# kalj/dealii-cuda

Measured on AMD Instinct MI355X. Metric: DoFs/s on 1305x Laplace vmult (bmop), p=4 3D uniform, higher is better.
Workload: dtype f64; 1 GPU; bmop: DEGREE_FE=4, DIMENSION=3, MATRIX_FREE_UNIFORM_MESH, hyper_cube(-1,1), 54^3 cells, 10218313 DoFs, 1 z-slab(s); cells_per_dir=54, n_dofs=10218313, n_cells=157464, parallelism=slab1, dof_numbering=caller's (lexicographic), finite=True, clock_ramp_steps=2000

## Files before the change

### dealii-cuda_amd/csrc/mfgpu_api.hip

```cpp
#include <hip/hip_runtime.h>

#include <type_traits>

#include <algorithm>
#include <cmath>
#include <cstdlib>
#include <cstring>
#include <memory>
#include <string>
#include <vector>

#include "mfgpu_kernels.h"

using namespace mfgpu;

struct EventTimer {
  std::vector<Event> ev;
  size_t used = 0;
  double ms = 0.0;
  int begin(hipStream_t st) {
    if (used + 2 > ev.size()) {
      Event e0, e1;
      int rc;
      if ((rc = e0.create(hipEventDefault)) || (rc = e1.create(hipEventDefault))) return rc;
      ev.push_back(std::move(e0));
      ev.push_back(std::move(e1));
    }
    HIP_TRY(hipEventRecord(ev[used].get(), st));
    return 0;
  }
  int end(hipStream_t st) {
    HIP_TRY(hipEventRecord(ev[used + 1].get(), st));
    used += 2;
    return 0;
  }
  int drain(double *total) {
    for (size_t i = 0; i + 1 < used; i += 2) {
      float t = 0.f;
      HIP_TRY(hipEventElapsedTime(&t, ev[i].get(), ev[i + 1].get()));
      ms += t;
    }
    used = 0;
    *total = ms;
    return 0;
  }
  void reset() {
    used = 0;
    ms = 0.0;
  }
};

struct mfgpu_handle {
  Plan plan;
  int dim = 0, n = 0, nd = 0, number_type = MFGPU_F64;
  bool hn = false;
  std::vector<double> S, Dt;
  std::vector<double> sv, sg;
  DeviceArray<uint32_t> d_batch_cell_off, d_batch_dof_off, d_bdofs;
  DeviceArray<uint8_t> d_bflags;
  DeviceArray<uint16_t> d_lmap;
  DeviceArray<uint16_t> d_lmapx;
  DeviceArray<uint16_t> d_perm;
  DeviceArray<uint32_t> d_bdofsp, d_idxp;
  DeviceArray<uint32_t> d_shtab;
  bool shared_records = false;
  size_t record_bytes = 0;
  DeviceArray<uint32_t> d_hnrec;
  DeviceArray<uint32_t> d_hn_slot;
  DeviceArray<void> d_coefp;
  DeviceArray<void> d_coef;
  DeviceArray<void> d_mass, d_massp;
  bool updatable = false;
  FoldGeometry geo;
  DeviceArray<uint32_t> d_cell_batch, d_cell_pos;
  size_t n_plane_cells = 0;
  DeviceArray<uint32_t> d_cmask, d_orphans;
  DeviceArray<void> d_hnw;
  DeviceArray<uint32_t> d_constrained;
  uint32_t n_constrained = 0;
  DeviceArray<void> d_tabsd;
  DeviceArray<void> d_tab2;
  bool twopass = true;
  DeviceArray<uint32_t> d_batch_nint, d_halo_off;
  std::vector<uint32_t> seg_end;
  std::vector<DeviceArray<uint32_t>> d_p2arr, d_p2tiles;
  std::vector<uint32_t> n_p2tiles;
  DeviceArray<uint32_t> d_p2rec, d_p2tab;
  bool p2_shared = false, p2_reverse = false, no_shared_records = false;
  Stream side;
  std::vector<Event> ev_seg;
  Event ev_side;
  bool side_pending = false;
  DeviceArray<void> d_halo;
  DeviceArray<unsigned long long> d_stamps;
  size_t lds = 0, device_bytes = 0;
  PlaneKernel planes = PlaneKernel::none;
  BatchKernel batches = BatchKernel::none;
  enum { kPlain, kMasked, kBatch };
  CellKernel<double> kernels_f64[3];
  CellKernel<float> kernels_f32[3];
  template <typename T>
  CellKernel<T> &kernel(int which) {
    if constexpr (std::is_same<T, double>::value) return kernels_f64[which];
    else return kernels_f32[which];
  }
  MultiKernel<double> multi_f64[kMaxFusedWidth - 1];
  MultiKernel<float> multi_f32[kMaxFusedWidth - 1];
  template <typename T>
  MultiKernel<T> &multi(int width) {
    if constexpr (std::is_same<T, double>::value) return multi_f64[width - 2];
    else return multi_f32[width - 2];
  }
  int multi_width = 1;
  DeviceArray<void> d_halo_multi;
  size_t halo_bytes = 0;
  uint32_t n_cus = 0, max_workgroups = 0;
  bool prof = false;
  EventTimer t_cells;
  EventTimer t_pass2;
  uint64_t prof_vmults = 0;
};

namespace {

template <typename T>
hipError_t bind_kernel(const mfgpu_handle *h, PlaneKernel pk, BatchKernel bk, bool hn, bool sh, CellKernel<T> *k) {
  const Plan &P = h->plan;
  const auto bind = pk == PlaneKernel::planes3 ? p_bind<T> : pk == PlaneKernel::planes4 ? q_bind<T>
                    : bk == BatchKernel::batches ? apply_bind<T> : bk == BatchKernel::x ? x_bind<T>
                    : bk == BatchKernel::g ? g_bind<T> : bk == BatchKernel::g2 ? g2_bind<T> : nullptr;
  if (!bind) return hipErrorInvalidValue;
  return bind(P.dim, P.n, hn, h->twopass, sh, h->d_mass.get() != nullptr, P.max_batch_dofs, k);
}

template <typename T, typename Args>
int launch_bound(mfgpu_handle *h, const CellKernel<T, Args> &k, const Args &a, uint32_t nbat, hipStream_t st) {
  if (!k.launch[0]) {
    set_error("cell-loop kernel not bound");
    return MFGPU_EINVAL;
  }
  uint32_t grid = (uint32_t)(k.per_cu < 1 ? 1 : k.per_cu) * h->n_cus;
  if (h->max_workgroups && h->max_workgroups < grid) grid = h->max_workgroups;
  HIP_TRY(k.launch[a.add != 0](a, h->S.data(), h->Dt.data(), k.lds, nbat < grid ? nbat : grid, st));
  return 0;
}

int check_symmetrize(int n, std::vector<double> &S, std::vector<double> &Dt) {
  const int p = n - 1;
  double err = 0, mag = 0;
  for (int r = 0; r < n; ++r)
    for (int c = 0; c < n; ++c) {
      const double s1 = S[r * n + c], s2 = S[(p - r) * n + (p - c)];
      const double d1 = Dt[r * n + c], d2 = -Dt[(p - r) * n + (p - c)];
      err = std::fmax(err, std::fmax(std::fabs(s1 - s2), std::fabs(d1 - d2)));
      mag = std::fmax(mag, std::fmax(std::fabs(s1), std::fabs(d1)));
    }
  if (err > 1e-10 * mag) {
    set_error("shape tables are not symmetric about the cell midpoint (unsupported)");
    return MFGPU_EUNSUPPORTED;
  }
  for (int r = 0; r < n; ++r)
    for (int c = 0; c < n; ++c) {
      const int r2 = p - r, c2 = p - c;
      if (r * n + c < r2 * n + c2) {
        const double s = 0.5 * (S[r * n + c] + S[r2 * n + c2]);
        S[r * n + c] = S[r2 * n + c2] = s;
        const double d = 0.5 * (Dt[r * n + c] - Dt[r2 * n + c2]);
        Dt[r * n + c] = d;
        Dt[r2 * n + c2] = -d;
      } else if (r == r2 && c == c2) {
        Dt[r * n + c] = 0.0;
      }
    }
  return 0;
}

int upload_pass2(mfgpu_handle *h, const uint32_t *priority, uint32_t n_priority) {
  const Plan &P = h->plan;
  const size_t ng = 1 + h->seg_end.size();
  const bool shared = P.sh_p2_use && !h->no_shared_records && n_priority == 0 && ng == 2;
  std::vector<Pass2Group> groups;
  int rc;
  if ((rc = pass2_groups(P, h->seg_end, priority, n_priority, shared, groups))) return rc;
  std::vector<DeviceArray<uint32_t>> d_arr(ng), d_tiles(ng);
  std::vector<uint32_t> n_tiles(ng, 0u);
  const bool reverse = (size_t)P.halo_off.back() * esize(h->number_type) <= ((size_t)256 << 20);
  DeviceArray<uint32_t> d_rec, d_tab;
  if (shared) {
    if ((rc = d_rec.upload(P.sh_p2rec.data(), P.sh_p2rec.size()))) return rc;
    if ((rc = d_tab.upload(P.sh_p2tab.data(), P.sh_p2tab.size()))) return rc;
  }
  for (size_t g = 0; g < ng; ++g) {
    std::vector<uint32_t> arr, tiles;
    build_pass2_classes(groups[g].dofs, groups[g].offsets, groups[g].slots, arr, tiles);
    n_tiles[g] = (uint32_t)(tiles.size() / 4);
    if (reverse) {
      const size_t nt = tiles.size() / 4;
      for (size_t a = 0, b = nt ? nt - 1 : 0; a < b; ++a, --b)
        for (int w = 0; w < 4; ++w) std::swap(tiles[4 * a + w], tiles[4 * b + w]);
    }
    if ((rc = d_arr[g].upload(arr.data(), arr.size()))) return rc;
    if ((rc = d_tiles[g].upload(tiles.data(), tiles.size()))) return rc;
  }
  h->d_p2arr = std::move(d_arr);
  h->d_p2tiles = std::move(d_tiles);
  h->n_p2tiles = std::move(n_tiles);
  h->d_p2rec = std::move(d_rec);
  h->d_p2tab = std::move(d_tab);
  h->p2_shared = shared;
  h->p2_reverse = reverse;
  return 0;
}

template <typename T>
int relayout_planes(mfgpu_handle *h, const uint32_t *cell_batch, const uint32_t *cell_pos, bool coef, bool mass,
                    hipStream_t st) {
  const size_t total = h->n_plane_cells * (size_t)h->nd;
  if (coef)
    HIP_TRY(relayout_coef_launch<T>(h->d_coefp.as<T>(), h->d_coef.as<const T>(), cell_batch, cell_pos, total, h->n, st));
  if (mass)
    HIP_TRY(relayout_coef_launch<T>(h->d_massp.as<T>(), h->d_mass.as<const T>(), cell_batch, cell_pos, total, h->n, st));
  return 0;
}

template <typename T>
int update_typed(mfgpu_handle *h, const void *coef, const void *mass, hipStream_t st) {
  const FoldInputs<T> in = h->geo.inputs<T>();
  if (coef) HIP_TRY(fold_coefficient_launch<T>(h->d_coef.as<T>(), (const T *)coef, in, st));
  if (mass) HIP_TRY(fold_mass_launch<T>(h->d_mass.as<T>(), (const T *)mass, in, st));
  if (h->planes == PlaneKernel::none) return 0;
  return relayout_planes<T>(h, h->d_cell_batch.get(), h->d_cell_pos.get(), coef != nullptr, mass != nullptr, st);
}

template <typename T>
int create_arrays(mfgpu_handle *h, const mfgpu_desc &d) {
  const Plan &P = h->plan;
  const size_t ncell = P.n_cells, nd = (size_t)P.nd;
  size_t &acct = h->device_bytes;
  auto up = [&](auto &arr, const void *src, size_t n) {
    const int rc = arr.upload(src, n);
    acct += arr.bytes();
    return rc;
  };
  int rc;
  if ((rc = up(h->d_batch_cell_off, P.batch_cell_off.data(), P.batch_cell_off.size()))) return rc;
  if ((rc = up(h->d_batch_dof_off, P.batch_dof_off.data(), P.batch_dof_off.size()))) return rc;
  if ((rc = up(h->d_bdofs, P.bdofs.data(), P.bdofs.size()))) return rc;
  if ((rc = up(h->d_bflags, P.bflags.data(), P.bflags.size()))) return rc;
  if ((rc = up(h->d_lmap, P.lmap.data(), P.lmap.size()))) return rc;
  const bool general = h->batches == BatchKernel::g || h->batches == BatchKernel::g2;
  if (h->batches == BatchKernel::x && !h->hn) {
    const std::vector<uint16_t> perm = x_lane_permutation(P.n);
    if ((rc = up(h->d_perm, perm.data(), perm.size()))) return rc;
  }
  if (h->batches == BatchKernel::x || general) {
    const std::vector<uint16_t> lx = x_pencil_runs(P.lmap, P.n);
    if ((rc = up(h->d_lmapx, lx.data(), lx.size()))) return rc;
  }
  if (h->batches == BatchKernel::g2) {
    std::vector<T> sd(2 * (size_t)P.n * P.n);
    for (int i = 0; i < P.n * P.n; ++i) {
      sd[i] = (T)h->S[i];
      sd[P.n * P.n + i] = (T)h->Dt[i];
    }
    if ((rc = up(h->d_tabsd, sd.data(), sd.size() * sizeof(T)))) return rc;
  }
  if (h->planes != PlaneKernel::none) {
    if ((rc = build_plane_records(h->plan, d.constraint_mask))) return rc;
    if (!P.pr_hn.empty()) {
      if ((rc = up(h->d_hnrec, P.pr_hn.data(), P.pr_hn.size()))) return rc;
      if ((rc = up(h->d_hn_slot, P.pr_hn_slot.data(), P.pr_hn_slot.size()))) return rc;
    }
    h->shared_records = P.sh_use && !(d.flags & MFGPU_NO_SHARED_RECORDS) &&
                        kernel_exists(h->planes, P.n, d.number_type, false, true, d.mass_coefficient != nullptr);
    const std::vector<uint32_t> &rd = h->shared_records ? P.sh_dofs : P.pr_dofs;
    const std::vector<uint32_t> &rx = h->shared_records ? P.sh_idx : P.pr_idx;
    if ((rc = up(h->d_bdofsp, rd.data(), rd.size()))) return rc;
    if ((rc = up(h->d_idxp, rx.data(), rx.size()))) return rc;
    if (h->shared_records && (rc = up(h->d_shtab, P.sh_batch.data(), P.sh_batch.size()))) return rc;
    h->record_bytes = h->d_bdofsp.bytes() + h->d_idxp.bytes() + h->d_shtab.bytes();
  }
  if ((rc = up(h->d_orphans, P.orphans.data(), P.orphans.size()))) return rc;
  if (h->twopass) {
    if ((rc = up(h->d_batch_nint, P.batch_nint.data(), P.batch_nint.size()))) return rc;
    if ((rc = up(h->d_halo_off, P.halo_off.data(), P.halo_off.size()))) return rc;
    if (h->planes != PlaneKernel::none && (uint64_t)P.halo_off.back() >= (1ull << 29)) {
      set_error("halo buffer too large for 32-bit byte offsets");
      return MFGPU_EUNSUPPORTED;
    }
    const size_t hb = ((size_t)P.halo_off.back() + 1) * sizeof(T);
    if ((rc = h->d_halo.alloc(hb, true))) return rc;
    acct += hb;
    h->halo_bytes = hb;
  }
  if (h->hn) {
    std::vector<uint32_t> cm(ncell);
    for (size_t i = 0; i < ncell; ++i) cm[i] = d.constraint_mask[P.cell_order[i]];
    if ((rc = up(h->d_cmask, cm.data(), ncell))) return rc;
    std::vector<T> w((size_t)h->n * h->n);
    for (size_t i = 0; i < w.size(); ++i) w[i] = (T)d.constraint_weights[i];
    if ((rc = up(h->d_hnw, w.data(), w.size() * sizeof(T)))) return rc;
  }
  FoldGeometry geo;
  if ((rc = geo.upload(d.JxW, d.inv_jac, P.cell_order.data(), P.dim, (uint32_t)ncell, (uint32_t)nd, general,
                       d.number_type)))
    return rc;
  DeviceArray<T> metric;
  if ((rc = fold_coefficient<T>(metric, d.coefficient, d.quadrature_points, geo.inputs<T>()))) return rc;
  h->d_coef = std::move(metric);
  acct += h->d_coef.bytes();
  if (d.mass_coefficient) {
    DeviceArray<T> mass;
    if ((rc = fold_mass<T>(mass, d.mass_coefficient, geo.inputs<T>()))) return rc;
    h->d_mass = std::move(mass);
    acct += h->d_mass.bytes();
  }
  if (h->updatable) {
    acct += geo.bytes();
    h->geo = std::move(geo);
  }
  if (h->planes != PlaneKernel::none) {
    const int n = P.n, NT = p_cells_per_wave(n) * n;
    const size_t nbat = P.n_plane_batches, total = nbat * (size_t)(n * n) * NT;
    const size_t ncell_p = P.batch_cell_off[nbat];
    std::vector<uint32_t> cb(ncell_p), cp(ncell_p);
    for (size_t b = 0; b < nbat; ++b)
      for (uint32_t c = P.batch_cell_off[b]; c < P.batch_cell_off[b + 1]; ++c) {
        cb[c] = (uint32_t)b;
        cp[c] = c - P.batch_cell_off[b];
      }
    DeviceArray<uint32_t> t_cb, t_cp;
    if ((rc = t_cb.upload(cb.data(), ncell_p))) return rc;
    if ((rc = t_cp.upload(cp.data(), ncell_p))) return rc;
    if ((rc = h->d_coefp.alloc(total * sizeof(T), true))) return rc;
    acct += h->d_coefp.bytes();
    h->n_plane_cells = ncell_p;
    if (d.mass_coefficient) {
      if ((rc = h->d_massp.alloc(total * sizeof(T), true))) return rc;
      acct += h->d_massp.bytes();
    }
    if ((rc = relayout_planes<T>(h, t_cb.get(), t_cp.get(), true, d.mass_coefficient != nullptr, nullptr))) return rc;
    HIP_TRY(hipDeviceSynchronize());
    if (h->updatable) {
      acct += t_cb.bytes() + t_cp.bytes();
      h->d_cell_batch = std::move(t_cb);
      h->d_cell_pos = std::move(t_cp);
    }
  }
  int dev = 0;
  hipDeviceProp_t prop;
  HIP_TRY(hipGetDevice(&dev));
  HIP_TRY(hipGetDeviceProperties(&prop, dev));
  h->n_cus = (uint32_t)prop.multiProcessorCount;
  h->max_workgroups = d.max_workgroups;
  if (h->planes != PlaneKernel::none) {
    CellKernel<T> &plain = h->kernel<T>(mfgpu_handle::kPlain), &masked = h->kernel<T>(mfgpu_handle::kMasked);
    HIP_TRY(bind_kernel<T>(h, h->planes, BatchKernel::none, false, h->shared_records, &plain));
    h->lds = plain.lds;
    if (P.n_plain_plane_batches < P.n_plane_batches) {
      HIP_TRY(bind_kernel<T>(h, h->planes, BatchKernel::none, true, false, &masked));
      h->lds = std::max(h->lds, masked.lds);
    }
  }
  if (h->batches == BatchKernel::none) return 0;
  CellKernel<T> &batch = h->kernel<T>(mfgpu_handle::kBatch);
  const hipError_t bind_batch_family = bind_kernel<T>(h, PlaneKernel::none, h->batches, h->hn, false, &batch);
  h->lds = batch.lds;
  if (h->lds > 160 * 1024) {
    set_error("batch needs more than 160 KiB of LDS; lower max_dofs_per_batch");
    return MFGPU_EINVAL;
  }
  HIP_TRY(bind_batch_family);
  if (h->twopass && h->planes == PlaneKernel::none)
    for (const int w : kFusedWidths) {
      if (!fused_kernel_exists(h->batches, P.n, d.number_type, h->hn, h->d_mass.get() != nullptr, w)) continue;
      MultiKernel<T> &mk = h->multi<T>(w);
      if (g_bind_width<T>(P.n, h->hn, false, h->d_mass.get() != nullptr, w, P.max_batch_dofs, &mk) != hipSuccess) {
        (void)hipGetLastError();
        mk = MultiKernel<T>();
      } else
        h->multi_width = std::max(h->multi_width, w);
    }
  return 0;
}

void choose_segments(mfgpu_handle *h, uint32_t request) {
  const Plan &P = h->plan;
  const uint32_t nb = (uint32_t)(P.batch_cell_off.size() - 1);
  h->seg_end.assign(1, nb);
  if (!h->twopass || nb < 2 || request == 1) return;
  const uint32_t npl = P.n_plane_batches, nplain = P.n_plain_plane_batches;
  std::vector<uint32_t> cuts;
  if (npl > 0 && npl < nb) cuts.push_back(npl);
  if (nplain > 0 && nplain < npl) cuts.push_back(nplain);
  if (request > 1) {
    for (uint32_t i = 1; i < request; ++i) cuts.push_back((uint32_t)((uint64_t)nb * i / request));
  }
  if (request == 0 && !P.pr_hn.empty() && nplain == 0 && P.n == 5) cuts.push_back(nb / 2);
  std::sort(cuts.begin(), cuts.end());
  h->seg_end.clear();
  for (uint32_t c : cuts)
    if (c > 0 && c < nb && (h->seg_end.empty() || h->seg_end.back() != c)) h->seg_end.push_back(c);
  h->seg_end.push_back(nb);
}

template <typename T>
int create_typed(mfgpu_handle *h, const mfgpu_desc &d) {
  int rc = create_arrays<T>(h, d);
  if (rc) return rc;
  choose_segments(h, d.cell_loop_segments);
  if (!h->twopass) return 0;
  if (h->seg_end.size() > 1) {
    int prio_least = 0, prio_greatest = 0;
    HIP_TRY(hipDeviceGetStreamPriorityRange(&prio_least, &prio_greatest));
    if ((rc = h->side.create(hipStreamNonBlocking, prio_least))) return rc;
    if ((rc = h->ev_side.create(hipEventDisableTiming))) return rc;
    h->ev_seg.resize(h->seg_end.size() - 1);
    for (Event &e : h->ev_seg)
      if ((rc = e.create(hipEventDisableTiming))) return rc;
  }
  return upload_pass2(h, nullptr, 0);
}

template <typename T>
int launch_pass2_group(mfgpu_handle *h, size_t group, void *dst, const void *src, hipStream_t st, int add) {
  if (h->p2_shared && group == 1)
    HIP_TRY(reduce_owner_batches_launch<T>((T *)dst, (const T *)src, h->d_halo.as<const T>(), h->d_p2rec.get(),
                                           h->d_p2tab.get(), (uint32_t)(h->plan.batch_cell_off.size() - 1),
                                           (uint32_t)p_hs(h->plan.n) * 64u, h->p2_reverse ? 1 : 0, add, st));
  HIP_TRY(reduce_classes_launch<T>((T *)dst, (const T *)src, h->d_halo.as<const T>(), h->d_p2arr[group].get(),
                                   h->d_p2tiles[group].get(), h->n_p2tiles[group], add, st));
  return 0;
}

template <typename T>
int vmult_pass2(mfgpu_handle *h, int phase, void *dst, const void *src, hipStream_t st, int add) {
  if (!h->twopass) return 0;
  if (phase == 0) return launch_pass2_group<T>(h, 0, dst, src, st, add);
  int rc = launch_pass2_group<T>(h, h->seg_end.size(), dst, src, st, add);
  if (!rc && h->side_pending) {
    HIP_TRY(hipStreamWaitEvent(st, h->ev_side.get(), 0));
    h->side_pending = false;
  }
  return rc;
}

template <typename T>
int launch_cells(mfgpu_handle *h, ApplyArgs<T> a, uint32_t b0, uint32_t b1, hipStream_t st) {
  const Plan &P = h->plan;
// ... 395 lines not shown
    set_error("null argument");
    return MFGPU_EINVAL;
  }
  const size_t nd = h->plan.n_dofs;
  if (n_vectors == 0 || (n_vectors > 1 && stride < nd)) {
    set_error("mfgpu_vmult_multi: n_vectors must be >= 1 and stride >= n_dofs");
    return MFGPU_EINVAL;
  }
  if ((flags & ~(MFGPU_MULTI_ADD | MFGPU_MULTI_LOOP | MFGPU_MULTI_FUSED)) ||
      ((flags & MFGPU_MULTI_LOOP) && (flags & MFGPU_MULTI_FUSED))) {
    set_error("mfgpu_vmult_multi: bad flags (MFGPU_MULTI_LOOP and MFGPU_MULTI_FUSED exclude each other)");
    return MFGPU_EINVAL;
  }
  const size_t bytes = ((size_t)(n_vectors - 1) * stride + nd) * esize(h->number_type);
  const char *d0 = (const char *)dst, *s0 = (const char *)src;
  if (d0 < s0 + bytes && s0 < d0 + bytes) {
    set_error("mfgpu_vmult_multi: the dst range overlaps the src range");
    return MFGPU_EINVAL;
  }
  return h->number_type == MFGPU_F64 ? vmult_multi_typed<double>(h, dst, src, n_vectors, stride, flags, (hipStream_t)stream)
                                     : vmult_multi_typed<float>(h, dst, src, n_vectors, stride, flags, (hipStream_t)stream);
}

int mfgpu_multi_width(const mfgpu_handle *h) { return h ? h->multi_width : 0; }

int mfgpu_update_coefficients(mfgpu_handle *h, const void *coefficient_dev, const void *mass_coefficient_dev,
                              void *stream) {
  if (!h) {
    set_error("null argument");
    return MFGPU_EINVAL;
  }
  if (!h->updatable) {
    set_error("mfgpu_update_coefficients: the handle was created without MFGPU_UPDATABLE_COEFFICIENTS");
    return MFGPU_EINVAL;
  }
  if (!coefficient_dev && !mass_coefficient_dev) {
    set_error("mfgpu_update_coefficients: coefficient_dev and mass_coefficient_dev are both NULL");
    return MFGPU_EINVAL;
  }
  if (mass_coefficient_dev && !h->d_mass.get()) {
    set_error("mfgpu_update_coefficients: the handle was created without a mass term (its kernels have no mass "
              "instantiation bound); create it with mass_coefficient");
    return MFGPU_EINVAL;
  }
  return h->number_type == MFGPU_F64 ? update_typed<double>(h, coefficient_dev, mass_coefficient_dev, (hipStream_t)stream)
                                     : update_typed<float>(h, coefficient_dev, mass_coefficient_dev, (hipStream_t)stream);
}

uint32_t mfgpu_n_dofs(const mfgpu_handle *h) { return h ? h->plan.n_dofs : 0; }

size_t mfgpu_memory_consumption(const mfgpu_handle *h) { return h ? h->device_bytes : 0; }

int mfgpu_plan_stats(const mfgpu_handle *h, uint64_t s[8]) {
  if (!h || !s) return MFGPU_EINVAL;
  const Plan &P = h->plan;
  s[0] = P.batch_cell_off.size() - 1;
  s[1] = P.color_batch_off.size() - 1;
  s[2] = P.bdofs.size();
  s[3] = P.max_batch_dofs;
  s[4] = P.max_batch_cells;
  s[5] = P.orphans.size();
  s[6] = P.n_first;
  s[7] = P.n_add;
  if (h->twopass) {
    const uint32_t nb = (uint32_t)s[0], npl = P.n_plane_batches, nplain = P.n_plain_plane_batches;
    const uint32_t edge[4] = {0u, nplain, npl, nb};
    s[1] = 0;
    for (size_t g = 0; g < h->seg_end.size(); ++g) {
      const uint32_t s0 = g ? h->seg_end[g - 1] : 0u, s1 = h->seg_end[g];
      for (int f = 0; f < 3; ++f)
        if (std::max(s0, edge[f]) < std::min(s1, edge[f + 1])) ++s[1];
    }
    s[6] = P.sdofs.size();
    s[7] = P.halo_off.back();
  }
  return 0;
}

int mfgpu_record_stats(const mfgpu_handle *h, uint64_t s[4]) {
  if (!h || !s) return MFGPU_EINVAL;
  const Plan &P = h->plan;
  const size_t n = (size_t)P.n, nb = (size_t)p_kgu((int)n) * 64, nx = ((n * n + 1) / 2) * (p_cells_per_wave((int)n) * n);
  const bool planes = h->planes != PlaneKernel::none;
  s[0] = (h->shared_records ? 1 : 0) | (h->p2_shared ? 2 : 0);
  s[1] = planes ? P.sh_dofs.size() / nb : 0;
  s[2] = planes ? P.sh_idx.size() / nx : 0;
  s[3] = h->record_bytes;
  return 0;
}

const char *mfgpu_kernel_name(const mfgpu_handle *h) {
  if (!h) return "";
  const bool x = h->batches == BatchKernel::x;
  switch (h->planes) {
    case PlaneKernel::planes3: return x ? "apply_planes3+apply_batches_x" : "apply_planes3";
    case PlaneKernel::planes4: return x ? "apply_planes4+apply_batches_x" : "apply_planes4";
    default: break;
  }
  switch (h->batches) {
    case BatchKernel::x: return "apply_batches_x";
    case BatchKernel::g: return "apply_batches_g";
    case BatchKernel::g2: return "apply_batches_g2";
    default: return "apply_batches";
  }
}

int mfgpu_profile_enable(mfgpu_handle *h, int on) {
  if (!h) return MFGPU_EINVAL;
  h->prof = on != 0;
  h->t_cells.reset();
  h->t_pass2.reset();
  h->prof_vmults = 0;
  return 0;
}

int mfgpu_profile_read_pass2(mfgpu_handle *h, double *ms) {
  if (!h || !ms) return MFGPU_EINVAL;
  HIP_TRY(hipDeviceSynchronize());
  return h->t_pass2.drain(ms);
}

int mfgpu_profile_read(mfgpu_handle *h, double *ms, uint64_t *nv) {
  if (!h || !ms || !nv) return MFGPU_EINVAL;
  HIP_TRY(hipDeviceSynchronize());
  if (const int rc = h->t_cells.drain(ms)) return rc;
  *nv = h->prof_vmults;
  return 0;
}

#ifdef MFGPU_STAMPS
int mfgpu_debug_stamps(mfgpu_handle *h, unsigned long long *out, size_t n_batches) {
  if (!h) return MFGPU_EINVAL;
  const size_t nbt = h->plan.batch_cell_off.size() - 1;
  if (!h->d_stamps.get()) return h->d_stamps.alloc(2 * nbt * 16, true);
  if (out && n_batches == nbt) {
    HIP_TRY(hipDeviceSynchronize());
    HIP_TRY(hipMemcpy(out, h->d_stamps.get(), 2 * nbt * 16 * sizeof(unsigned long long), hipMemcpyDeviceToHost));
  }
  return 0;
}
#endif


int mfgpu_compute_inverse_diagonal(mfgpu_handle *h, void *inv_diag, void *stream) {
  if (!h || !inv_diag) {
    set_error("null argument");
    return MFGPU_EINVAL;
  }
  return h->number_type == MFGPU_F64 ? inverse_diagonal_typed<double>(h, inv_diag, (hipStream_t)stream)
                                     : inverse_diagonal_typed<float>(h, inv_diag, (hipStream_t)stream);
}

int mfgpu_set_constrained_values(mfgpu_handle *h, void *vec, double value, void *stream) {
  if (!h || !vec) {
    set_error("null argument");
    return MFGPU_EINVAL;
  }
  if (h->number_type == MFGPU_F64)
    HIP_TRY(set_values_launch<double>((double *)vec, h->d_constrained.get(), h->n_constrained, value, (hipStream_t)stream));
  else
    HIP_TRY(set_values_launch<float>((float *)vec, h->d_constrained.get(), h->n_constrained, (float)value,
                                     (hipStream_t)stream));
  return 0;
}

int mfgpu_vec_sadd(void *v, double s, double a, const void *w, size_t n, int nt, void *stream) {
  return vec_map(0, v, w, s, a, n, nt, stream);
// ... 75 lines not shown
```

### dealii-cuda_amd/csrc/mfgpu_internal.h

```cpp
#ifndef MFGPU_INTERNAL_H
#define MFGPU_INTERNAL_H

#include <cstdint>
#include <string>
#include <vector>

#include "../../include/mfgpu.h"

namespace mfgpu {

void set_error(const std::string &msg);

inline int ipow(int a, int e) {
  int r = 1;
  for (int i = 0; i < e; ++i) r *= a;
  return r;
}

constexpr int p_cells_per_wave(int n) { return 64 / n; }
constexpr int p_ji(int n) { return n == 3 ? 2 : n == 4 ? 5 : n == 5 ? 9 : n == 6 ? 14 : 23; }
constexpr int p_hs(int n) { return n == 3 ? 3 : n == 4 ? 6 : n == 5 ? 9 : n == 6 ? 14 : 18; }
constexpr int p_kgu(int n) { return p_ji(n) + p_hs(n); }
constexpr int p_cell_stride(int n) {
  int s = n * n * n;
  while ((s & 31) != (n & 31)) ++s;
  return s;
}

constexpr int q_plane_stride(int n) { return n >= 6 ? 65 : n == 5 ? 33 : n == 4 ? 17 : 33; }
constexpr int q_cell_stride(int n) { return n * q_plane_stride(n); }
constexpr int p_priv_max(int n) { return n >= 5 ? 384 : n == 4 ? 256 : 192; }
constexpr int kHnOpRounds = 2;
constexpr int p_hn_rows(int n) { return p_priv_max(n) / 64 + 3 * kHnOpRounds * 3 + 2; }

template <typename T>
constexpr size_t q_region_doubles(int n) {
  const size_t t = ((size_t)(p_cells_per_wave(n) + 1) * q_cell_stride(n) * sizeof(T) + 7) / 8;
  const size_t u = (size_t)p_kgu(n) * 64 + p_priv_max(n);
  return t > u ? t : u;
}
template <typename T>
constexpr size_t q_lds_bytes(int n, bool hn) {
  return (q_region_doubles<T>(n) + (hn ? (size_t)n * n : 0)) * 8;
}

constexpr uint8_t kFlagConstrained = 1;
constexpr uint8_t kFlagAdd = 2;

struct Plan {
  int dim = 0, degree = 0, n = 0, nd = 0;
  uint32_t n_dofs = 0, n_cells = 0;
  std::vector<uint32_t> cell_order;
  std::vector<uint32_t> batch_cell_off;
  std::vector<uint32_t> batch_dof_off;
  std::vector<uint32_t> color_batch_off;
  std::vector<uint32_t> bdofs;
  std::vector<uint8_t> bflags;
  std::vector<uint16_t> lmap;
  std::vector<uint32_t> orphans;
  std::vector<uint32_t> batch_nint;
  std::vector<uint32_t> halo_off;
  std::vector<uint32_t> sdofs;
  std::vector<uint32_t> s_off;
  std::vector<uint32_t> s_idx;
  std::vector<uint32_t> chunks;
  std::vector<uint32_t> gstarts;
  uint32_t max_batch_dofs = 0, max_batch_cells = 0;
  uint32_t n_plane_batches = 0;
  uint32_t n_plain_plane_batches = 0;
  std::vector<uint32_t> pr_dofs, pr_idx, pr_hn, pr_hn_slot;
  std::vector<uint32_t> sh_dofs, sh_idx, sh_batch;
  bool sh_use = false;
  std::vector<uint32_t> sh_p2rec, sh_p2tab;
  bool sh_p2_use = false;
  uint64_t n_first = 0, n_add = 0;
};

struct PlanLimits {
  uint32_t max_cells = 0, max_dofs = 0;
  uint32_t interior_max = 0, shared_max = 0, halo_stride = 0;
  bool segregate_masked = false;
  bool masked_planes = false;
  uint32_t private_max = 0;
};

int build_plan(const mfgpu_desc &d, Plan &plan, uint32_t max_chunks = 3, const PlanLimits *limits = nullptr);

struct HnLine {
  uint16_t node[8];
};
void hn_cell_lines(unsigned mask, int n, std::vector<HnLine> (&lines)[3], std::vector<uint16_t> &nodes);

enum class PlaneKernel : uint8_t { none, planes3, planes4 };
enum class BatchKernel : uint8_t { none, batches, x, g, g2 };
int choose_kernel_and_plan(const mfgpu_desc &d, PlaneKernel &pk, BatchKernel &bk, Plan &plan);

constexpr bool planes4_wide(int n) { return n >= 6; }
constexpr bool kernel_exists(PlaneKernel k, int n, int number_type, bool hn, bool sh, bool mass) {
  switch (k) {
    case PlaneKernel::planes3: return n >= 3 && n <= 5 && !(sh && hn);
    case PlaneKernel::planes4:
      return planes4_wide(n) ? n <= 7 && !hn && !sh && !mass
                             : n >= 3 && !sh && !(mass && n == 5 && number_type == MFGPU_F64);
    default: return false;
  }
}
constexpr bool kernel_exists(BatchKernel k, int n, int , bool , bool sh, bool ) {
  return k != BatchKernel::none && n >= 2 && n <= 7 && !sh;
}
constexpr int kFusedWidths[] = {3, 2};
constexpr bool fused_kernel_exists(BatchKernel k, int n, int number_type, bool hn, bool , int nv) {
  return k == BatchKernel::g && n >= 2 && n <= 7 && (nv == 2 || nv == 3) &&
         !(hn && number_type == MFGPU_F64 && n >= (nv == 3 ? 6 : 7));
}
std::vector<uint32_t> multi_groups(uint32_t n_vectors, const std::vector<uint32_t> &widths);
int build_plane_records(Plan &plan, const uint32_t *constraint_mask);
constexpr int kShBatchWords = 4;
constexpr double kShareMaxFraction = 0.5;
void share_plane_records(Plan &plan);
constexpr int kP2Header = 16, kP2MaxK = 12, kP2SlotBits = 12;
void share_pass2_records(Plan &plan);

std::vector<uint16_t> x_lane_permutation(int n);
std::vector<uint16_t> x_pencil_runs(const std::vector<uint16_t> &lmap, int n);
struct Pass2Group {
  std::vector<uint32_t> dofs, offsets = std::vector<uint32_t>(1, 0u), slots;
};
int pass2_groups(const Plan &plan, const std::vector<uint32_t> &seg_end, const uint32_t *priority, uint32_t n_priority,
                 bool shared, std::vector<Pass2Group> &groups);

int derive_tables(int n, const double *shape_values, const double *shape_gradients,
                  std::vector<double> &S, std::vector<double> &Dt);

int handle_number_type(const mfgpu_handle *h);
int handle_set_priority_dofs(mfgpu_handle *h, const uint32_t *ids, uint32_t n);
int handle_vmult_phase(mfgpu_handle *h, int phase, void *dst, const void *src, void *stream, int add);
int handle_n_batches(const mfgpu_handle *h);
bool handle_ranged_ok(const mfgpu_handle *h);
int handle_batches_touching(const mfgpu_handle *h, const uint32_t *ids, uint32_t n, std::vector<uint8_t> &flags);
int handle_cells_range(mfgpu_handle *h, uint32_t b0, uint32_t b1, void *dst, const void *src, void *stream, int add);
int handle_cells_two_ranges(mfgpu_handle *h, uint32_t b0, uint32_t b1, uint32_t c0, uint32_t c1, void *dst,
                            const void *src, void *stream, int add);
int handle_pass2_group(mfgpu_handle *h, int group, void *dst, const void *src, void *stream, int add);

void transfer_sizes(const mfgpu_transfer *t, uint32_t *n_coarse_dofs, uint32_t *n_fine_dofs, int *number_type);
void vcycle_active(const mfgpu_vcycle *v, int *active_type, uint32_t *n_active);

}

struct mfgpu_plan {
  mfgpu::Plan plan;
};

#endif
```

### dealii-cuda_amd/csrc/mfgpu_kernels.h

```cpp
#ifndef MFGPU_KERNELS_H
#define MFGPU_KERNELS_H

#include <hip/hip_runtime.h>

#include <type_traits>

#include "mfgpu_device.h"
#include "mfgpu_internal.h"

namespace mfgpu {

template <typename T>
struct ApplyArgs {
  const uint32_t *batch_cell_off;
  const uint32_t *batch_dof_off;
  const uint32_t *bdofs;
  const uint8_t *bflags;
  const uint16_t *lmap;
  const uint16_t *lmapx;
  const uint16_t *perm;
  const uint32_t *bdofsp;
  const uint32_t *idxp;
  const T *coefp;
  const uint32_t *hnrec;
// ... 16 lines not shown
  int dbg;
  const uint32_t *shtab = nullptr;
  const T *mass = nullptr;
  const T *massp = nullptr;
};

constexpr int kMaxFusedWidth = 3;
template <typename T>
struct MultiArgs : ApplyArgs<T> {
  size_t stride = 0;
  T *halos[kMaxFusedWidth];
};
constexpr size_t kMaxLdsBytes = 160 * 1024;

template <typename T, int n>
struct Tables {
  T S[((n + 1) / 2) * n];
  T Dt[((n + 1) / 2) * n];
};

template <typename T, int n>
inline Tables<T, n> make_tables(const double *S, const double *Dt) {
  Tables<T, n> tab;
  for (int i = 0; i < ((n + 1) / 2) * n; ++i) {
    tab.S[i] = (T)S[i];
    tab.Dt[i] = (T)Dt[i];
  }
  return tab;
}

template <typename T, typename Args = ApplyArgs<T>>
struct CellKernel {
  size_t lds = 0;
  int per_cu = 0;
  hipError_t (*launch[2])(const Args &a, const double *S, const double *Dt, size_t lds, uint32_t grid,
                          hipStream_t st) = {nullptr, nullptr};
};

template <typename T, int Block, auto K, auto MakeTab, typename Args = ApplyArgs<T>>
hipError_t launch_cell_kernel(const Args &a, const double *S, const double *Dt, size_t lds, uint32_t grid,
                              hipStream_t st) {
  if constexpr (std::is_null_pointer_v<decltype(MakeTab)>)
    hipLaunchKernelGGL(K, dim3(grid), dim3(Block), lds, st, a);
  else
    hipLaunchKernelGGL(K, dim3(grid), dim3(Block), lds, st, a, MakeTab(S, Dt));
  return hipGetLastError();
}

template <typename T, int Block, auto K0, auto K1, auto MakeTab, typename Args = ApplyArgs<T>>
hipError_t bind_cell_kernel(size_t lds, CellKernel<T, Args> *k) {
  k->lds = lds;
  for (const void *f : {(const void *)K1, (const void *)K0})
    if (const hipError_t e = hipFuncSetAttribute(f, hipFuncAttributeMaxDynamicSharedMemorySize, (int)lds)) return e;
  k->launch[0] = launch_cell_kernel<T, Block, K0, MakeTab, Args>;
  k->launch[1] = launch_cell_kernel<T, Block, K1, MakeTab, Args>;
  return hipOccupancyMaxActiveBlocksPerMultiprocessor(&k->per_cu, (const void *)K0, Block, lds);
}

template <typename F>
hipError_t dispatch_flags(F &&f) { return f(); }
template <typename F, typename... B>
hipError_t dispatch_flags(F &&f, bool flag, B... rest) {
  return dispatch_flags(
      [&](auto... c) { return flag ? f(std::true_type{}, c...) : f(std::false_type{}, c...); }, rest...);
}
template <typename F, typename... B>
hipError_t dispatch_instantiation(int n, F &&f, B... flags) {
  auto at = [&](auto N) { return dispatch_flags([&](auto... c) { return f(N, c...); }, flags...); };
  switch (n) {
    case 2: return at(std::integral_constant<int, 2>{});
    case 3: return at(std::integral_constant<int, 3>{});
    case 4: return at(std::integral_constant<int, 4>{});
    case 5: return at(std::integral_constant<int, 5>{});
    case 6: return at(std::integral_constant<int, 6>{});
    case 7: return at(std::integral_constant<int, 7>{});
    default: return hipErrorInvalidValue;
  }
}
template <typename T>
constexpr int number_type_of = sizeof(T) == 8 ? MFGPU_F64 : MFGPU_F32;

#define MFGPU_CELL_LOOP_FAMILY(F)                                                                              \
  template <typename T>                                                                                        \
  hipError_t F##_bind(int dim, int n, bool hn, bool twopass, bool sh, bool mass, uint32_t nb_max, CellKernel<T> *k);
MFGPU_CELL_LOOP_FAMILY(apply)
MFGPU_CELL_LOOP_FAMILY(x)
MFGPU_CELL_LOOP_FAMILY(g)
MFGPU_CELL_LOOP_FAMILY(g2)
MFGPU_CELL_LOOP_FAMILY(p)
MFGPU_CELL_LOOP_FAMILY(q)
#undef MFGPU_CELL_LOOP_FAMILY
template <typename T>
using MultiKernel = CellKernel<T, MultiArgs<T>>;
template <typename T, typename Args>
hipError_t g_bind_width(int n, bool hn, bool sh, bool mass, int nv, uint32_t nb_max, CellKernel<T, Args> *k);

void build_pass2_classes(const std::vector<uint32_t> &sdofs, const std::vector<uint32_t> &s_off,
                         const std::vector<uint32_t> &s_idx, std::vector<uint32_t> &arr, std::vector<uint32_t> &tiles);
template <typename T>
hipError_t reduce_classes_launch(T *dst, const T *src, const T *halo, const uint32_t *arr, const uint32_t *tiles,
                                 uint32_t n_tiles, int add, hipStream_t st);
template <typename T>
hipError_t reduce_classes_multi_launch(int nv, T *dst, const T *src, size_t stride, T *const *halos, const uint32_t *arr,
                                       const uint32_t *tiles, uint32_t n_tiles, int add, hipStream_t st);
template <typename T>
hipError_t reduce_owner_batches_launch(T *dst, const T *src, const T *halo, const uint32_t *rec, const uint32_t *tab,
                                       uint32_t n_batches, uint32_t hstride, int reverse, int add, hipStream_t st);
template <typename T>
hipError_t relayout_coef_launch(T *out, const T *in, const uint32_t *cell_batch, const uint32_t *cell_pos,
                                size_t total, int n, hipStream_t st);
template <typename T>
hipError_t fold_general_launch(T *M, const T *coef, const T *jxw, const T *jinv, const uint32_t *order,
                               uint32_t n_cells, uint32_t nd, hipStream_t st);
template <typename T>
hipError_t fold_general2_launch(T *M, const T *coef, const T *jxw, const T *jinv, const uint32_t *order,
                                uint32_t n_cells, uint32_t nd, hipStream_t st);
template <typename T>
hipError_t orphan_launch(T *dst, const T *src, const uint32_t *orph, uint32_t n, int add, hipStream_t st);
template <typename T>
hipError_t coefficient_launch(T *coef, const T *qpts, size_t nq, int dim, hipStream_t st);
template <typename T>
hipError_t fold_launch(T *c, const T *coef, const T *jxw, const T *j0, const uint32_t *order,
                       uint32_t n_cells, uint32_t nd, hipStream_t st);
template <typename T>
hipError_t fill_launch(T *v, size_t n, T a, hipStream_t st);
template <typename T>
struct FoldInputs {
  const T *jxw = nullptr, *jinv = nullptr;
  const uint32_t *order = nullptr;
  int dim = 0;
  uint32_t n_cells = 0, nd = 0;
  bool general = false;
  size_t metric_entries() const { return (size_t)n_cells * nd * (general ? (dim == 3 ? 6 : 3) : 1); }
};
template <typename T>
hipError_t fold_coefficient_launch(T *out, const T *coef, const FoldInputs<T> &in, hipStream_t st);
template <typename T>
hipError_t fold_mass_launch(T *out, const T *c, const FoldInputs<T> &in, hipStream_t st);
struct FoldGeometry {
  DeviceArray<void> jxw, jinv;
  DeviceArray<uint32_t> order;
  int dim = 0;
  uint32_t n_cells = 0, nd = 0;
  bool general = false;
  int upload(const void *JxW, const void *inv_jac, const uint32_t *cell_order, int dim_, uint32_t n_cells_, uint32_t nd_,
             bool general_, int number_type);
  size_t bytes() const { return jxw.bytes() + jinv.bytes() + order.bytes(); }
  template <typename T>
  FoldInputs<T> inputs(const T *jxw_resident = nullptr) const {
    FoldInputs<T> in;
    in.jxw = jxw_resident ? jxw_resident : jxw.as<const T>();
    in.jinv = jinv.as<const T>();
    in.order = order.get();
    in.dim = dim, in.n_cells = n_cells, in.nd = nd, in.general = general;
    return in;
  }
};
template <typename T>
int fold_mass(DeviceArray<T> &out, const void *mass_coefficient, const FoldInputs<T> &in);
template <typename T>
int fold_coefficient(DeviceArray<T> &out, const void *coefficient, const void *quadrature_points,
                     const FoldInputs<T> &in);

template <typename T>
hipError_t diag_launch(int dim, int n, T *diag, uint32_t n_batches, const uint32_t *batch_cell_off,
                       const uint32_t *batch_dof_off, const uint32_t *bdofs, const uint16_t *lmap, const T *coef,
                       const uint32_t *cmask, const T *hn_weights, const T *tab2, hipStream_t st);
// ... 24 lines not shown
```

### dealii-cuda_amd/csrc/mfgpu_kernels.hip

```cpp
#include <hip/hip_runtime.h>

#include "mfgpu_cell.h"
#include "mfgpu_kernels.h"

namespace mfgpu {

template <int n>
constexpr int min_waves_per_simd() { return n <= 5 ? 2 : 1; }

template <int dim, int n, typename T, bool HN, bool TWOPASS, bool MASS = false>
__global__ void __launch_bounds__(256) __attribute__((amdgpu_waves_per_eu(min_waves_per_simd<n>())))
apply_batches(const ApplyArgs<T> A, const Tables<T, n> tab) {
  constexpr int kBlock = 256;
  constexpr int kGU = (max_batch_dofs(kBlock) + kBlock - 1) / kBlock;
  constexpr int nd = (dim == 3) ? n * n * n : n * n;
  constexpr int P = nd / n;
  constexpr int NG = 1;
  constexpr int GT = kBlock / NG;
  constexpr int CH = GT / P;
  constexpr int n2 = n * n;
  constexpr int CHND = CH * nd;
  static_assert(CH >= 1, "a cell's pencils must fit into one thread group");
  extern __shared__ __attribute__((aligned(16))) unsigned char smem_raw[];
  double *acc = reinterpret_cast<double *>(smem_raw);
// ... 178 lines not shown
          }
        }
      }
    } else if (!DBG(4)) {
      T old[kGU];
#pragma unroll
      for (int j = 0; j < kGU; ++j) old[j] = A.dst[G[j] & 0x7fffffffu];
#pragma unroll
      for (int j = 0; j < kGU; ++j) {
        const int t = tid + j * kBlock;
        if (t < nb && !(G[j] >> 31)) A.dst[G[j]] = ((F[j] & kFlagAdd) || A.add) ? old[j] + (T)acc[t] : (T)acc[t];
      }
    }
    STAMP(15);
    if (!has_nb) break;
    __syncthreads();
    b = bn;
    c0 = c0n;
    ncell = ncelln;
    d0 = d0n;
    nb = nbn;
    nint = nintn;
    hoff = hoffn;
#pragma unroll
    for (int j = 0; j < kGU; ++j) {
      G[j] = Gn[j];
      F[j] = Fn[j];
      SV[j] = SVn[j];
    }
  }
}

template <typename T>
__global__ void orphan_kernel(T *dst, const T *src, const uint32_t *orph, uint32_t n, int add) {
  const uint32_t i = blockIdx.x * blockDim.x + threadIdx.x;
  if (i >= n) return;
  const uint32_t o = orph[i];
  const uint32_t g = o & 0x7fffffffu;
  const T s = (o >> 31) ? src[g] : T(0);
  dst[g] = add ? dst[g] + s : s;
}

template <typename T, int dim>
__global__ void coefficient_kernel(T *coef, const T *qpts, size_t nq) {
  const size_t i = (size_t)blockIdx.x * blockDim.x + threadIdx.x;
  if (i >= nq) return;
  T s = 0;
#pragma unroll
  for (int d = 0; d < dim; ++d) {
    const T x = qpts[i * dim + d];
    s += x * x;
  }
  coef[i] = T(1) / (T(0.05) + T(2) * s);
}

template <typename T>
__global__ void fold_kernel(T *c, const T *coef, const T *jxw, const T *j0, const uint32_t *order,
                            uint32_t n_cells, uint32_t nd) {
  const size_t i = (size_t)blockIdx.x * blockDim.x + threadIdx.x;
  if (i >= (size_t)n_cells * nd) return;
  const uint32_t pos = (uint32_t)(i / nd), q = (uint32_t)(i - (size_t)pos * nd);
  const uint32_t cell = order[pos];
  const T j = j0[cell];
  c[i] = coef[(size_t)cell * nd + q] * j * j * jxw[(size_t)cell * nd + q];
}

template <typename T>
__global__ void fill_kernel(T *v, size_t n, T a) {
  size_t i = (size_t)blockIdx.x * blockDim.x + threadIdx.x;
  const size_t stride = (size_t)gridDim.x * blockDim.x;
  for (; i < n; i += stride) v[i] = a;
}


template <int dim, int n, typename T>
static size_t lds_bytes_t(uint32_t nb_max) {
  constexpr int nd = (dim == 3) ? n * n * n : n * n;
  const int CH = 256 / (nd / n);
  return (size_t)nb_max * sizeof(double) + (size_t)(nb_max + 3 * CH * nd + n * n) * sizeof(T) +
         (size_t)CH * nd * sizeof(uint16_t);
}

template <typename T>
hipError_t apply_bind(int dim, int n, bool hn, bool twopass, bool sh, bool mass, uint32_t nb_max, CellKernel<T> *k) {
  if (dim != 2 && dim != 3) return hipErrorInvalidValue;
  return dispatch_instantiation(n, [&](auto N, auto D3, auto HN, auto TP, auto SH, auto MASS) {
    constexpr int n_ = N, dim_ = D3 ? 3 : 2;
    if constexpr (kernel_exists(BatchKernel::batches, n_, number_type_of<T>, HN, SH, MASS)) {
      constexpr auto K = apply_batches<dim_, n_, T, HN, TP, MASS>;
      return bind_cell_kernel<T, 256, K, K, make_tables<T, n_>>(lds_bytes_t<dim_, n_, T>(nb_max), k);
    } else
      return hipErrorInvalidValue;
  }, dim == 3, hn, twopass, sh, mass);
}

template <typename T>
hipError_t orphan_launch(T *dst, const T *src, const uint32_t *orph, uint32_t n, int add,
                         hipStream_t st) {
  if (n == 0) return hipSuccess;
  hipLaunchKernelGGL(orphan_kernel<T>, dim3((n + 255) / 256), dim3(256), 0, st, dst, src, orph, n, add);
  return hipGetLastError();
}

template <typename T>
hipError_t coefficient_launch(T *coef, const T *qpts, size_t nq, int dim, hipStream_t st) {
  const unsigned grid = (unsigned)((nq + 255) / 256);
  if (dim == 2)
    hipLaunchKernelGGL((coefficient_kernel<T, 2>), dim3(grid), dim3(256), 0, st, coef, qpts, nq);
  else
    hipLaunchKernelGGL((coefficient_kernel<T, 3>), dim3(grid), dim3(256), 0, st, coef, qpts, nq);
  return hipGetLastError();
}

template <typename T>
hipError_t fold_launch(T *c, const T *coef, const T *jxw, const T *j0, const uint32_t *order,
                       uint32_t n_cells, uint32_t nd, hipStream_t st) {
  const size_t tot = (size_t)n_cells * nd;
  hipLaunchKernelGGL(fold_kernel<T>, dim3((unsigned)((tot + 255) / 256)), dim3(256), 0, st, c, coef, jxw,
                     j0, order, n_cells, nd);
  return hipGetLastError();
}

int FoldGeometry::upload(const void *JxW, const void *inv_jac, const uint32_t *cell_order, int dim_, uint32_t n_cells_,
                         uint32_t nd_, bool general_, int number_type) {
  dim = dim_, n_cells = n_cells_, nd = nd_, general = general_;
  const size_t np = (size_t)n_cells * nd, es = esize(number_type);
  int rc;
  if (JxW && (rc = jxw.upload(JxW, np * es))) return rc;
  if ((rc = jinv.upload(inv_jac, (general ? np * (size_t)(dim * dim) : n_cells) * es))) return rc;
  return order.upload(cell_order, n_cells);
}

template <typename T>
hipError_t fold_coefficient_launch(T *out, const T *coef, const FoldInputs<T> &in, hipStream_t st) {
  if ((size_t)in.n_cells * in.nd == 0) return hipSuccess;
  const auto fold = !in.general ? fold_launch<T> : in.dim == 3 ? fold_general_launch<T> : fold_general2_launch<T>;
  return fold(out, coef, in.jxw, in.jinv, in.order, in.n_cells, in.nd, st);
}

template <typename T>
int fold_coefficient(DeviceArray<T> &out, const void *coefficient, const void *quadrature_points,
                     const FoldInputs<T> &in) {
  const size_t np = (size_t)in.n_cells * in.nd;
  DeviceArray<T> coef, qpts;
  int rc;
  if (coefficient) {
    if ((rc = coef.upload(coefficient, np))) return rc;
  } else {
    if ((rc = qpts.upload(quadrature_points, np * in.dim))) return rc;
    if ((rc = coef.alloc(np))) return rc;
    if ((rc = hip_check(coefficient_launch<T>(coef.get(), qpts.get(), np, in.dim, nullptr), "coefficient evaluation")))
      return rc;
  }
  if ((rc = out.alloc(in.metric_entries()))) return rc;
  if ((rc = hip_check(fold_coefficient_launch<T>(out.get(), coef.get(), in, nullptr), "coefficient fold"))) return rc;
  return hip_check(hipDeviceSynchronize(), "coefficient fold");
}

template <typename T>
__global__ void fold_mass_kernel(T *m, const T *c, const T *jxw, const uint32_t *order, uint32_t n_cells, uint32_t nd) {
  const size_t i = (size_t)blockIdx.x * blockDim.x + threadIdx.x;
  if (i >= (size_t)n_cells * nd) return;
  const uint32_t pos = (uint32_t)(i / nd), q = (uint32_t)(i - (size_t)pos * nd);
  const size_t s = (size_t)order[pos] * nd + q;
  m[i] = c[s] * jxw[s];
}

template <typename T>
hipError_t fold_mass_launch(T *out, const T *c, const FoldInputs<T> &in, hipStream_t st) {
  const size_t np = (size_t)in.n_cells * in.nd;
  if (np == 0) return hipSuccess;
  hipLaunchKernelGGL(fold_mass_kernel<T>, dim3((unsigned)((np + 255) / 256)), dim3(256), 0, st, out, c, in.jxw,
                     in.order, in.n_cells, in.nd);
  return hipGetLastError();
}

template <typename T>
int fold_mass(DeviceArray<T> &out, const void *mass_coefficient, const FoldInputs<T> &in) {
  const size_t np = (size_t)in.n_cells * in.nd;
  DeviceArray<T> c;
  int rc;
  if ((rc = c.upload(mass_coefficient, np)) || (rc = out.alloc(np))) return rc;
  if ((rc = hip_check(fold_mass_launch<T>(out.get(), c.get(), in, nullptr), "mass fold"))) return rc;
  return hip_check(hipDeviceSynchronize(), "mass fold");
}

template <typename T>
hipError_t fill_launch(T *v, size_t n, T a, hipStream_t st) {
  if (n == 0) return hipSuccess;
  size_t blocks = (n + 255) / 256;
  if (blocks > 2048) blocks = 2048;
  hipLaunchKernelGGL(fill_kernel<T>, dim3((unsigned)blocks), dim3(256), 0, st, v, n, a);
  return hipGetLastError();
}

#define INST(T)                                                                                         \
  template hipError_t apply_bind<T>(int, int, bool, bool, bool, bool, uint32_t, CellKernel<T> *);      \
  template hipError_t orphan_launch<T>(T *, const T *, const uint32_t *, uint32_t, int, hipStream_t);   \
  template hipError_t coefficient_launch<T>(T *, const T *, size_t, int, hipStream_t);                  \
  template hipError_t fold_launch<T>(T *, const T *, const T *, const T *, const uint32_t *, uint32_t,  \
                                     uint32_t, hipStream_t);                                            \
  template hipError_t fold_coefficient_launch<T>(T *, const T *, const FoldInputs<T> &, hipStream_t);   \
  template hipError_t fold_mass_launch<T>(T *, const T *, const FoldInputs<T> &, hipStream_t);          \
  template int fold_coefficient<T>(DeviceArray<T> &, const void *, const void *, const FoldInputs<T> &); \
  template int fold_mass<T>(DeviceArray<T> &, const void *, const FoldInputs<T> &);                    \
  template hipError_t fill_launch<T>(T *, size_t, T, hipStream_t);
INST(double)
INST(float)

}
```

### dealii-cuda_amd/csrc/mfgpu_kernels_g.hip

```cpp
#include <hip/hip_runtime.h>

#include "mfgpu_cell.h"
#include "mfgpu_kernels.h"

namespace mfgpu {

template <typename T, int NV>
using GArgs = std::conditional_t<NV == 1, ApplyArgs<T>, MultiArgs<T>>;
template <typename T, typename P>
__device__ __forceinline__ P *vec_at(const ApplyArgs<T> &, P *p, int) { return p; }
template <typename T, typename P>
__device__ __forceinline__ P *vec_at(const MultiArgs<T> &A, P *p, int v) { return p + (size_t)v * A.stride; }
template <typename T>
__device__ __forceinline__ T *vec_halo(const ApplyArgs<T> &A, int) { return A.halo; }
template <typename T>
__device__ __forceinline__ T *vec_halo(const MultiArgs<T> &A, int v) { return A.halos[v]; }

template <int n, typename T, bool HN, int NV>
constexpr int g_waves_per_simd() {
  if (NV == 1) return 2;
  if (NV != 2) return 1;
  if (sizeof(T) == 8) return n <= (HN ? 2 : 3) ? 2 : 1;
  return n <= (HN ? 4 : 6) ? 2 : 1;
}
// ... 341 lines not shown
        T *hl = vec_halo(A, v) + hoff + l - nint;
        T old[kGU];
        if (A.add) {
#pragma unroll
          for (int j = 0; j < kGU; ++j) old[j] = vec_at(A, A.dst, v)[G[j] & 0x7fffffffu];
        }
#pragma unroll
        for (int j = 0; j < kGU; ++j) {
          if (l < nint - j * kBlock) {
            if (!(G[j] >> 31)) vec_at(A, A.dst, v)[G[j]] = A.add ? old[j] + (T)ul[j * kBlock] : (T)ul[j * kBlock];
          } else if (l < nb - j * kBlock) {
            hl[j * kBlock] = (T)ul[j * kBlock];
          }
        }
        if (NV == 1) break;
      }
    }
    if (!has_nb) break;
    b = bn;
    c0 = c0n;
    ncell = ncelln;
    d0 = d0n;
    nb = nbn;
    nint = nintn;
    hoff = hoffn;
#pragma unroll
    for (int j = 0; j < kGU; ++j) {
      G[j] = Gn[j];
#pragma unroll
      for (int iv = 0; iv < NV; ++iv) {
        const int v = NV == 1 ? 0 : iv;
        SV[v][j] = SVn[v][j];
        if (NV == 1) break;
      }
    }
#pragma unroll
    for (int k = 0; k < kMaxChunks; ++k)
#pragma unroll
      for (int q = 0; q < NW; ++q) IX[k][q] = IXn[k][q];
  }
}

template <typename T>
__global__ void fold_general_kernel(T *M, const T *coef, const T *jxw, const T *jinv, const uint32_t *order,
                                    uint32_t n_cells, uint32_t nd) {
  const size_t i = (size_t)blockIdx.x * blockDim.x + threadIdx.x;
  if (i >= (size_t)n_cells * nd) return;
  const uint32_t cell = (uint32_t)(i / nd), q = (uint32_t)(i - (size_t)cell * nd);
  const size_t s = (size_t)order[cell] * nd + q;
  const T *J = jinv + s * 9;
  const T a = coef[s] * jxw[s];
  T *m = M + (size_t)cell * (6 * nd) + q;
  int e = 0;
  for (int d1 = 0; d1 < 3; ++d1)
    for (int d2 = d1; d2 < 3; ++d2)
      m[(e++) * nd] = a * (J[3 * d1] * J[3 * d2] + J[3 * d1 + 1] * J[3 * d2 + 1] + J[3 * d1 + 2] * J[3 * d2 + 2]);
}

template <int n, typename T>
static size_t g_lds_bytes(uint32_t nb_max, int nv) {
  constexpr int nd = n * n * n;
  constexpr int CH = 256 / (n * n);
  return (size_t)nv * nb_max * sizeof(double) + (size_t)(4 * CH * nd + n * n) * sizeof(T);
}

template <typename T, typename Args>
hipError_t g_bind_width(int n, bool hn, bool sh, bool mass, int nv, uint32_t nb_max, CellKernel<T, Args> *k) {
  return dispatch_instantiation(n, [&](auto N, auto W3, auto HN, auto SH, auto MASS) {
    constexpr int n_ = N;
    constexpr int NV = std::is_same_v<Args, ApplyArgs<T>> ? 1 : W3 ? 3 : 2;
    if constexpr (NV == 1 ? kernel_exists(BatchKernel::g, n_, number_type_of<T>, HN, SH, MASS)
                          : !SH && fused_kernel_exists(BatchKernel::g, n_, number_type_of<T>, HN, MASS, NV)) {
      constexpr auto K = apply_batches_g<n_, T, HN, MASS, NV>;
      const size_t lds = g_lds_bytes<n_, T>(nb_max, NV);
      k->lds = lds;
      if (NV > 1 && lds > kMaxLdsBytes) return hipErrorInvalidValue;
      return bind_cell_kernel<T, 256, K, K, make_tables<T, n_>>(lds, k);
    } else
      return hipErrorInvalidValue;
  }, nv == 3, hn, sh, mass);
}

template <typename T>
hipError_t g_bind(int, int n, bool hn, bool, bool sh, bool mass, uint32_t nb_max, CellKernel<T> *k) {
  return g_bind_width(n, hn, sh, mass, 1, nb_max, k);
}

template <typename T>
hipError_t fold_general_launch(T *M, const T *coef, const T *jxw, const T *jinv, const uint32_t *order,
                               uint32_t n_cells, uint32_t nd, hipStream_t st) {
  const size_t tot = (size_t)n_cells * nd;
  hipLaunchKernelGGL(fold_general_kernel<T>, dim3((unsigned)((tot + 255) / 256)), dim3(256), 0, st, M, coef, jxw, jinv,
                     order, n_cells, nd);
  return hipGetLastError();
}

#define INST(T)                                                                                                  \
  template hipError_t g_bind<T>(int, int, bool, bool, bool, bool, uint32_t, CellKernel<T> *);                    \
  template hipError_t g_bind_width<T>(int, bool, bool, bool, int, uint32_t, MultiKernel<T> *);                   \
  template hipError_t fold_general_launch<T>(T *, const T *, const T *, const T *, const uint32_t *, uint32_t, \
                                             uint32_t, hipStream_t);
INST(double)
INST(float)

}
```

### dealii-cuda_amd/csrc/mfgpu_kernels_g2.hip

```cpp
#include <hip/hip_runtime.h>

#include "mfgpu_kernels.h"

namespace mfgpu {

namespace {

constexpr unsigned kTypeX = 1u << 0, kTypeY = 1u << 1, kFaceX = 1u << 3, kFaceY = 1u << 4;

template <int n, typename T, bool HN, bool MASS = false>
__global__ void __launch_bounds__(256)
apply_batches_g2(const ApplyArgs<T> A) {
  constexpr int nd = n * n, CH = 256 / nd, p = n - 1;
  extern __shared__ __attribute__((aligned(16))) unsigned char smem_raw[];
  double *acc = reinterpret_cast<double *>(smem_raw);
  T *usrc = reinterpret_cast<T *>(acc + A.nb_max);
  T *X = usrc + A.nb_max;
  T *Y = X + CH * nd;
  T *FX = Y + CH * nd;
  T *FY = FX + CH * nd;
  T *St = FY + CH * nd;
  T *Dt = St + nd;
  T *Wt = Dt + nd;
  const int tid = threadIdx.x;
// ... 67 lines not shown
      if (act) {
        T gx = T(0), gy = T(0);
        if (MASS) mv = A.mass[cell * nd + q] * x[q];
        for (int t = 0; t < n; ++t) {
          gx += Dt[i * n + t] * x[t + n * j];
          gy += Dt[j * n + t] * x[i + n * t];
        }
        const T *m = A.coef + cell * (3 * nd) + q;
        const T mxx = m[0], mxy = m[nd], myy = m[2 * nd];
        fx[q] = mxx * gx + mxy * gy;
        fy[q] = mxy * gx + myy * gy;
      }
      __syncthreads();
      if (act) {
        T s = T(0);
        for (int t = 0; t < n; ++t) s += Dt[t * n + i] * fx[t + n * j] + Dt[t * n + j] * fy[i + n * t];
        y[q] = MASS ? s + mv : s;
      }
      __syncthreads();
      if (act) {
        T s = T(0);
        for (int k = 0; k < n; ++k) s += St[j * n + k] * y[i + n * k];
        x[q] = s;
      }
      __syncthreads();
      T out = T(0);
      if (act) {
        for (int k = 0; k < n; ++k) out += St[i * n + k] * x[k + n * j];
      }
      if (HN) {
        __syncthreads();
        if (act) y[q] = out;
        __syncthreads();
        if (act) x[q] = hn_pass(y, 1, true);
        __syncthreads();
        if (act) out = hn_pass(x, 0, true);
      }
      if (MASS) {
        for (int w = 0; w < 4; ++w) {
          if (act && (tid >> 6) == w) atomicAdd(&acc[lm], (double)out);
          __syncthreads();
        }
      } else {
        if (act) atomicAdd(&acc[lm], (double)out);
        __syncthreads();
      }
    }
    T *halo = A.halo + A.halo_off[b];
    for (uint32_t t = tid; t < nb; t += 256) {
      const uint32_t g = A.bdofs[d0 + t];
      if (t < nint) {
        if (!(g >> 31)) A.dst[g] = A.add ? A.dst[g] + (T)acc[t] : (T)acc[t];
      } else {
        halo[t - nint] = (T)acc[t];
      }
    }
  }
}

template <typename T>
__global__ void fold_general2_kernel(T *M, const T *coef, const T *jxw, const T *jinv, const uint32_t *order,
                                     uint32_t n_cells, uint32_t nd) {
  const size_t i = (size_t)blockIdx.x * blockDim.x + threadIdx.x;
  if (i >= (size_t)n_cells * nd) return;
  const uint32_t cell = (uint32_t)(i / nd), q = (uint32_t)(i - (size_t)cell * nd);
  const size_t s = (size_t)order[cell] * nd + q;
  const T *J = jinv + s * 4;
  const T a = coef[s] * jxw[s];
  T *m = M + (size_t)cell * (3 * nd) + q;
  m[0] = a * (J[0] * J[0] + J[1] * J[1]);
  m[nd] = a * (J[0] * J[2] + J[1] * J[3]);
  m[2 * nd] = a * (J[2] * J[2] + J[3] * J[3]);
}

template <int n, typename T>
size_t g2_lds_bytes(uint32_t nb_max) {
  constexpr int nd = n * n, CH = 256 / nd;
  return (size_t)nb_max * sizeof(double) + ((size_t)nb_max + 4 * CH * nd + 3 * nd) * sizeof(T);
}

}

template <typename T>
hipError_t g2_bind(int, int n, bool hn, bool, bool sh, bool mass, uint32_t nb_max, CellKernel<T> *k) {
  return dispatch_instantiation(n, [&](auto N, auto HN, auto SH, auto MASS) {
    constexpr int n_ = N;
    if constexpr (kernel_exists(BatchKernel::g2, n_, number_type_of<T>, HN, SH, MASS)) {
      constexpr auto K = apply_batches_g2<n_, T, HN, MASS>;
      return bind_cell_kernel<T, 256, K, K, nullptr>(g2_lds_bytes<n_, T>(nb_max), k);
    } else
      return hipErrorInvalidValue;
  }, hn, sh, mass);
}
template hipError_t g2_bind<double>(int, int, bool, bool, bool, bool, uint32_t, CellKernel<double> *);
template hipError_t g2_bind<float>(int, int, bool, bool, bool, bool, uint32_t, CellKernel<float> *);

template <typename T>
hipError_t fold_general2_launch(T *M, const T *coef, const T *jxw, const T *jinv, const uint32_t *order,
                                uint32_t n_cells, uint32_t nd, hipStream_t st) {
  const size_t tot = (size_t)n_cells * nd;
  hipLaunchKernelGGL(fold_general2_kernel<T>, dim3((unsigned)((tot + 255) / 256)), dim3(256), 0, st, M, coef, jxw, jinv,
                     order, n_cells, nd);
  return hipGetLastError();
}
template hipError_t fold_general2_launch<double>(double *, const double *, const double *, const double *,
                                                 const uint32_t *, uint32_t, uint32_t, hipStream_t);
template hipError_t fold_general2_launch<float>(float *, const float *, const float *, const float *, const uint32_t *,
                                                uint32_t, uint32_t, hipStream_t);

}
```

### dealii-cuda_amd/csrc/mfgpu_kernels_p.hip

```cpp
#include <hip/hip_runtime.h>

#include "mfgpu_cell.h"
#include "mfgpu_kernels.h"
#include "mfgpu_planes.h"

namespace mfgpu {

#define MFGPU_PIN_VMEM() __builtin_amdgcn_sched_barrier(0x380)

template <int n, typename T, bool ADD, bool HN, bool SH = false, bool MASS = false>
__global__ void __launch_bounds__(64) __attribute__((amdgpu_waves_per_eu(1, 1)))
apply_planes3(const ApplyArgs<T> A, const TablesEO<T, n> tab) {
  constexpr int n2 = n * n;
  constexpr int CW = p_cells_per_wave(n);
  constexpr int NT = CW * n;
  constexpr int KGU = p_kgu(n);
  constexpr int JI = p_ji(n);
  constexpr int HS = KGU - JI;
  constexpr int SA = p_cell_stride(n);
  constexpr int NIW = (n2 + 1) / 2;
  extern __shared__ __attribute__((aligned(16))) unsigned char smem_raw[];
  constexpr int PRIV = HN ? p_priv_max(n) : 0;
  double *ua = reinterpret_cast<double *>(smem_raw);
  T *Aw = reinterpret_cast<T *>(ua + KGU * 64 + PRIV + (HN ? n2 : 0));
  T *Bw = Aw + (CW + 1) * SA;
  double *Wl = ua + KGU * 64 + PRIV;

  const int lane = threadIdx.x;
  if (HN) {
    if (lane < n2) Wl[lane] = (double)A.hn_weights[lane];
  }
  const int lc = lane / n, k = lane - lc * n;
  const bool lane_on = lane < NT;
  const int tk = lane_on ? lane : NT - 1;

  uint32_t b, bstride, bend;
  {
    const uint32_t nbt = A.batch_end - A.batch0 - A.hole_len, G = gridDim.x;
    if (G >= 8 && nbt >= G) {
      const uint32_t xcd = blockIdx.x & 7u, slot = blockIdx.x >> 3;
      const uint32_t q = G >> 3, rem = G & 7u;
      const uint32_t wlo = xcd * q + (xcd < rem ? xcd : rem);
      const uint32_t w = q + (xcd < rem ? 1u : 0u);
      b = A.batch0 + (uint32_t)((uint64_t)nbt * wlo / G) + slot;
      bend = A.batch0 + (uint32_t)((uint64_t)nbt * (wlo + w) / G);
      bstride = w;
    } else {
      b = A.batch0 + blockIdx.x;
      bend = A.batch_end - A.hole_len;
      bstride = G;
    }
  }
  if (b >= bend) return;
  const uint32_t hole0 = A.hole0, hole_len = A.hole_len;
  auto next_of = [&](uint32_t x) {
    const uint32_t l = (x >= hole0 ? x - hole_len : x) + bstride;
    return l < bend ? (l >= hole0 ? l + hole_len : l) : x;
  };
  if (b >= hole0) b += hole_len;
  static_assert(kernel_exists(PlaneKernel::planes3, n, number_type_of<T>, HN, SH, MASS), "no such instantiation");
  struct Meta {
    uint32_t base, drec, irec;
  };
  auto meta_request = [&](uint32_t bb) -> uint32_t {
    return A.shtab[(size_t)bb * kShBatchWords + (lane & (kShBatchWords - 1))];
  };
  auto meta_of = [&](uint32_t v) -> Meta {
    return Meta{(uint32_t)__builtin_amdgcn_readlane((int)v, 0), (uint32_t)__builtin_amdgcn_readlane((int)v, 1),
                (uint32_t)__builtin_amdgcn_readlane((int)v, 2)};
  };

  auto load_dofs = [&](uint32_t rec, uint32_t (&g)[KGU]) {
    const uint32_t *p = A.bdofsp + (size_t)rec * (KGU * 64) + lane;
#pragma unroll
    for (int j = 0; j < KGU; ++j) g[j] = SH ? p[j * 64] : nt_load(p + j * 64);
  };
  auto src_at = [&](uint32_t base, uint32_t g) -> T {
    const T *const sp = SH ? A.src + base : A.src;
    return *reinterpret_cast<const T *>(reinterpret_cast<const char *>(sp) + (uint32_t)(g * (uint32_t)sizeof(T)));
  };
  auto dst_at = [&](uint32_t base, uint32_t g) -> T * {
    T *const dp = SH ? A.dst + base : A.dst;
    return reinterpret_cast<T *>(reinterpret_cast<char *>(dp) + (uint32_t)(g * (uint32_t)sizeof(T)));
  };
  auto load_ix = [&](uint32_t rec, uint32_t (&ix)[NIW]) {
    const uint32_t *p = A.idxp + (size_t)rec * (NIW * NT) + tk;
#pragma unroll
    for (int w = 0; w < NIW; ++w) ix[w] = SH ? p[w * NT] : nt_load(p + w * NT);
  };
  auto stage_src = [&](const uint32_t (&g)[KGU], const T (&sv)[KGU]) {
#pragma unroll
    for (int j = 0; j < KGU; ++j) {
      double v = (double)sv[j];
      if (j >= JI) {
        const unsigned long long keep = (unsigned long long)(long long)~((int)g[j] >> 31);
        v = __longlong_as_double((long long)((unsigned long long)__double_as_longlong(v) & keep));
      }
      ua[lane + j * 64] = v;
    }
  };
  auto ixb = [&](const uint32_t (&ix)[NIW], int i) -> uint32_t {
    return (i & 1) ? (ix[i >> 1] >> 16) : (ix[i >> 1] & 0xffffu);
  };
  auto scatter_slot = [&](int j, uint32_t bb, uint32_t base, uint32_t g, T r, T oldv) {
    if (j < JI) {
      *dst_at(base, g) = ADD ? oldv + r : r;
    } else {
      T *const hp = A.halo + (size_t)bb * (HS * 64) + lane;
      hp[(j - JI) * 64] = r;
    }
  };

  uint32_t b1 = next_of(b), b2 = next_of(b1);
  uint32_t Gp[KGU], Gc[KGU], Gn[KGU], Gnn[KGU];
  uint32_t IXc[NIW], IXn[NIW];
  constexpr int CR = PRIV / 64, HROWS = HN ? p_hn_rows(n) : 1;
  uint32_t Hc[HROWS], Hn[HROWS];
  auto load_hn = [&](uint32_t bb, uint32_t (&H)[HROWS]) {
    const uint32_t slot = A.hn_slot[bb];
    if (slot != 0xffffffffu) {
      const uint32_t *p = A.hnrec + (size_t)slot * (HROWS * 64) + lane;
#pragma unroll
      for (int w = 0; w < HROWS; ++w) H[w] = nt_load(p + w * 64);
    } else {
#pragma unroll
      for (int w = 0; w < HROWS; ++w) H[w] = 0u;
    }
  };
  T Cc[n2];
  T Mm[MASS ? n2 : 1];
  T SVn[KGU], R[KGU], old[KGU];
  Meta Mp{0u, 0u, 0u}, Mc = Mp, M1 = Mp, M2 = Mp;
  uint32_t Mv = 0u;
  if (SH) {
    Mc = meta_of(meta_request(b));
    M1 = meta_of(meta_request(b1));
    M2 = meta_of(meta_request(b2));
    Mp = Mc;
  }
  load_dofs(SH ? Mc.drec : b, Gc);
  load_dofs(SH ? M1.drec : b1, Gn);
  load_ix(SH ? Mc.irec : b, IXc);
  if (HN) load_hn(b, Hc);
  constexpr uint32_t kDummyIx = 8u * (uint32_t)(KGU * 64 - 1) * 0x10001u;
#pragma unroll
  for (int w = 0; w < NIW; ++w) IXc[w] = lane_on ? IXc[w] : kDummyIx;
  {
    const T *p = A.coefp + (size_t)b * (n2 * NT) + tk;
#pragma unroll
    for (int r = 0; r < n2; ++r) Cc[r] = nt_load(p + r * NT);
  }
  if (MASS) {
    const T *p = A.massp + (size_t)b * (n2 * NT) + tk;
#pragma unroll
    for (int r = 0; r < n2; ++r) Mm[r] = nt_load(p + r * NT);
  }
#pragma unroll
  for (int j = 0; j < KGU; ++j) {
    SVn[j] = src_at(Mc.base, Gc[j]);
    Gp[j] = Gc[j];
    R[j] = T(0);
    old[j] = T(0);
  }
  stage_src(Gc, SVn);
  WaveSync::sync();

  const int pxy = lc * SA + n2 * k;
  const int pyz = lc * SA + k;
  uint32_t bp = b;

  while (true) {
    const bool has_next = b1 != b;
    constexpr int kH2 = HN ? HROWS - 2 : 0, kH1 = HN ? HROWS - 1 : 0;
    const uint32_t hn_ncopy = HN ? (uint32_t)__builtin_amdgcn_readfirstlane(Hc[kH2] & 0xffffu) : 0u;
    auto hn_count = [&](int dir) -> uint32_t {
      const uint32_t w = dir == 0 ? Hc[kH2] >> 16 : dir == 1 ? Hc[kH1] & 0xffffu : Hc[kH1] >> 16;
      return (uint32_t)__builtin_amdgcn_readfirstlane(w);
    };
    auto hn_pass = [&](int dir, bool transposed, const double (&Wr)[n2]) {
      const uint32_t count = hn_count(dir);
#pragma unroll
      for (int r = 0; r < kHnOpRounds; ++r) {
        if ((uint32_t)(r * 64) >= count) break;
        const bool on = (uint32_t)(r * 64 + lane) < count;
        const uint32_t *ww = &Hc[CR + (dir * kHnOpRounds + r) * 3];
        double v[n], o[n];
        uint32_t pos[n];
#pragma unroll
        for (int t = 0; t < n; ++t) {
          pos[t] = on ? (ww[t >> 1] >> (16 * (t & 1))) & 0xffffu : (uint32_t)(KGU * 64 + PRIV - 1);
          v[t] = ua[pos[t]];
        }
#pragma unroll
        for (int i = 0; i < n; ++i) {
          double acc = 0.0;
#pragma unroll
          for (int k2 = 0; k2 < n; ++k2) acc = fma(transposed ? Wr[k2 * n + i] : Wr[i * n + k2], v[k2], acc);
          o[i] = acc;
        }
        if (on) {
#pragma unroll
          for (int i = 0; i < n; ++i) ua[pos[i]] = o[i];
        }
      }
    };
    if (HN && hn_ncopy) {
      double Wr[n2];
#pragma unroll
      for (int i = 0; i < n2; ++i) Wr[i] = Wl[i];
      double cv[CR > 0 ? CR : 1];
#pragma unroll
      for (int r = 0; r < CR; ++r) cv[r] = (uint32_t)(r * 64 + lane) < hn_ncopy ? ua[Hc[r] & 0xffffu] : 0.0;
#pragma unroll
      for (int r = 0; r < CR; ++r)
        if ((uint32_t)(r * 64 + lane) < hn_ncopy) ua[Hc[r] >> 16] = cv[r];
      WaveSync::sync();
      hn_pass(0, false, Wr);
      WaveSync::sync();
      hn_pass(1, false, Wr);
      WaveSync::sync();
      hn_pass(2, false, Wr);
      WaveSync::sync();
    }
    STAMP(0);
    RSTAMP(8);
    WGSTAMP(10);
    load_dofs(SH ? M2.drec : b2, Gnn);
    load_ix(SH ? M1.irec : b1, IXn);
    if (SH) Mv = meta_request(next_of(b2));
    if (HN) load_hn(b1, Hn);
    if (ADD) {
#pragma unroll
      for (int j = 0; j < JI; ++j) old[j] = *dst_at(Mp.base, Gp[j]);
    }
    STAMP(1);
    auto hookA = [&](int) {};
    auto hookB = [&](int s) {
      MFGPU_PIN_VMEM();
#pragma unroll
      for (int j = (KGU * s) / (5 * n); j < (KGU * (s + 1)) / (5 * n); ++j)
        scatter_slot(j, bp, Mp.base, Gp[j], R[j], old[j]);
#pragma unroll
      for (int j = (KGU * s) / (5 * n); j < (KGU * (s + 1)) / (5 * n); ++j)
        SVn[j] = src_at(M1.base, Gn[j]);
      MFGPU_PIN_VMEM();
    };
    const T *const cnext = A.coefp + (size_t)b1 * (n2 * NT) + tk;
    const T *const mnext = MASS ? A.massp + (size_t)b1 * (n2 * NT) + tk : nullptr;
    auto hookC = [&](int s) {
      MFGPU_PIN_VMEM();
#pragma unroll
      for (int r = (n2 * s) / (2 * n); r < (n2 * (s + 1)) / (2 * n); ++r)
        Cc[r] = nt_load(cnext + r * NT);
      if (MASS) {
#pragma unroll
        for (int r = (n2 * s) / (2 * n); r < (n2 * (s + 1)) / (2 * n); ++r)
          Mm[r] = nt_load(mnext + r * NT);
      }
      MFGPU_PIN_VMEM();
    };

    {
      T u[n2];
#pragma unroll
      for (int x = 0; x < n; ++x)
#pragma unroll
        for (int y = 0; y < n; ++y)
          u[x + n * y] = (T) * reinterpret_cast<const double *>(reinterpret_cast<const char *>(ua) + ixb(IXc, x + n * y));
#pragma unroll
      for (int x = 0; x < n; ++x) {
        T in[n], out[n];
        get_line<n, 1>(u, x, in);
        eo_apply<n, 0>(tab, in, out);
        set_line<n, 1>(u, x, out);
        hookA(x);
      }
#pragma unroll
      for (int y = 0; y < n; ++y) {
        T in[n], a[n], bb[n];
        get_line<n, 0>(u, y, in);
        eo_apply<n, 0>(tab, in, a);
        eo_apply<n, 2>(tab, a, bb);
#pragma unroll
        for (int x = 0; x < n; ++x) {
          Aw[pxy + x + n * y] = a[x];
          Bw[pxy + x + n * y] = bb[x];
        }
        hookA(n + y);
      }
    }
    WaveSync::sync();
    STAMP(2);
#pragma unroll
    for (int j = 0; j < KGU + PRIV / 64; ++j) ua[lane + j * 64] = 0.0;

    {
      T nx[n];
#pragma unroll
      for (int z = 0; z < n; ++z) nx[z] = Bw[pyz + n2 * z];
#pragma unroll
      for (int y = 0; y < n; ++y) {
        T in[n], g[n], o[n];
#pragma unroll
        for (int z = 0; z < n; ++z) in[z] = nx[z];
#pragma unroll
        for (int z = 0; z < n; ++z) nx[z] = y + 1 < n ? Bw[pyz + n * (y + 1) + n2 * z] : Aw[pyz + n2 * z];
        eo_apply<n, 0>(tab, in, g);
#pragma unroll
        for (int z = 0; z < n; ++z) g[z] *= Cc[y + n * z];
        eo_apply<n, 1>(tab, g, o);
#pragma unroll
        for (int z = 0; z < n; ++z) Bw[pyz + n * y + n2 * z] = o[z];
        hookB(y);
      }
      T v[n2], r[n2];
#pragma unroll
      for (int y = 0; y < n; ++y) {
        T in[n], o[n];
#pragma unroll
        for (int z = 0; z < n; ++z) in[z] = nx[z];
        if (y + 1 < n) {
#pragma unroll
          for (int z = 0; z < n; ++z) nx[z] = Aw[pyz + n * (y + 1) + n2 * z];
        }
        eo_apply<n, 0>(tab, in, o);
        set_line<n, 1>(v, y, o);
        hookB(n + y);
// ... 16 lines not shown
        eo_apply<n, 2>(tab, in, g);
#pragma unroll
        for (int y = 0; y < n; ++y) g[y] *= Cc[y + n * z];
        eo_apply<n, 3>(tab, g, o);
#pragma unroll
        for (int y = 0; y < n; ++y) r[y + n * z] += MASS ? fma(Mm[y + n * z], in[y], o[y]) : o[y];
        hookB(3 * n + z);
      }
#pragma unroll
      for (int y = 0; y < n; ++y) {
        T in[n], o[n];
        get_line<n, 1>(r, y, in);
        eo_apply<n, 1>(tab, in, o);
#pragma unroll
        for (int z = 0; z < n; ++z) Aw[pyz + n * y + n2 * z] = o[z];
        hookB(4 * n + y);
      }
    }
    WaveSync::sync();
    STAMP(3);

    {
      T o[n2];
      T nr[n], nt[n];
#pragma unroll
      for (int x = 0; x < n; ++x) {
        nr[x] = Aw[pxy + x];
        nt[x] = Bw[pxy + x];
      }
#pragma unroll
      for (int y = 0; y < n; ++y) {
        T rp[n], tp[n], w[n], ol[n];
#pragma unroll
        for (int x = 0; x < n; ++x) {
          rp[x] = nr[x];
          tp[x] = nt[x];
        }
        if (y + 1 < n) {
#pragma unroll
          for (int x = 0; x < n; ++x) {
            nr[x] = Aw[pxy + x + n * (y + 1)];
            nt[x] = Bw[pxy + x + n * (y + 1)];
          }
        }
        eo_apply<n, 3>(tab, tp, w);
#pragma unroll
        for (int x = 0; x < n; ++x) w[x] += rp[x];
        eo_apply<n, 1>(tab, w, ol);
        set_line<n, 0>(o, y, ol);
        hookC(y);
      }
#pragma unroll
      for (int x = 0; x < n; ++x) {
        T in[n], out[n];
        get_line<n, 1>(o, x, in);
        eo_apply<n, 1>(tab, in, out);
#pragma unroll
        for (int y = 0; y < n; ++y)
          lds_add(reinterpret_cast<double *>(reinterpret_cast<char *>(ua) + ixb(IXc, x + n * y)), (double)out[y]);
        hookC(n + x);
      }
    }
    WaveSync::sync();
    STAMP(4);

    if (HN && hn_ncopy) {
      double Wr[n2];
#pragma unroll
      for (int i = 0; i < n2; ++i) Wr[i] = Wl[i];
      hn_pass(2, true, Wr);
      WaveSync::sync();
      hn_pass(1, true, Wr);
      WaveSync::sync();
      hn_pass(0, true, Wr);
      WaveSync::sync();
      double cv[CR > 0 ? CR : 1];
#pragma unroll
      for (int r = 0; r < CR; ++r) cv[r] = (uint32_t)(r * 64 + lane) < hn_ncopy ? ua[Hc[r] >> 16] : 0.0;
#pragma unroll
      for (int r = 0; r < CR; ++r)
        if ((uint32_t)(r * 64 + lane) < hn_ncopy) lds_add(ua + (Hc[r] & 0xffffu), cv[r]);
      WaveSync::sync();
    }
#pragma unroll
    for (int j = 0; j < KGU; ++j) R[j] = (T)ua[lane + j * 64];
    WaveSync::sync();
    STAMP(5);
    stage_src(Gn, SVn);
    STAMP(6);
    bp = b;
    if (SH) Mp = Mc;
#pragma unroll
    for (int j = 0; j < KGU; ++j) Gp[j] = Gc[j];
    STAMP(7);
    RSTAMP(9);
    if (!has_next) break;
    WaveSync::sync();
    b = b1;
    b1 = b2;
    b2 = next_of(b2);
    if (SH) {
      Mc = M1;
      M1 = M2;
      M2 = meta_of(Mv);
    }
#pragma unroll
    for (int j = 0; j < KGU; ++j) {
      Gc[j] = Gn[j];
      Gn[j] = Gnn[j];
    }
#pragma unroll
    for (int w = 0; w < NIW; ++w) IXc[w] = lane_on ? IXn[w] : kDummyIx;
    if (HN) {
#pragma unroll
      for (int w = 0; w < HROWS; ++w) Hc[w] = Hn[w];
    }
  }
  if (ADD) {
#pragma unroll
    for (int j = 0; j < JI; ++j) old[j] = *dst_at(Mp.base, Gp[j]);
  }
#pragma unroll
  for (int j = 0; j < KGU; ++j) scatter_slot(j, bp, Mp.base, Gp[j], R[j], old[j]);
}

template <int n, typename T>
static size_t p_lds_bytes(bool hn) {
  return ((size_t)p_kgu(n) * 64 + (hn ? (size_t)p_priv_max(n) + n * n : 0)) * sizeof(double) +
         (size_t)2 * (p_cells_per_wave(n) + 1) * p_cell_stride(n) * sizeof(T);
}

template <typename T>
hipError_t p_bind(int, int n, bool hn, bool, bool sh, bool mass, uint32_t, CellKernel<T> *k) {
  return dispatch_instantiation(n, [&](auto N, auto HN, auto SH, auto MASS) {
    constexpr int n_ = N;
    if constexpr (kernel_exists(PlaneKernel::planes3, n_, number_type_of<T>, HN, SH, MASS))
      return bind_cell_kernel<T, 64, apply_planes3<n_, T, false, HN, SH, MASS>, apply_planes3<n_, T, true, HN, SH, MASS>,
                              make_tables_eo<T, n_>>(p_lds_bytes<n_, T>(HN), k);
    else
      return hipErrorInvalidValue;
  }, hn, sh, mass);
}
template hipError_t p_bind<double>(int, int, bool, bool, bool, bool, uint32_t, CellKernel<double> *);
template hipError_t p_bind<float>(int, int, bool, bool, bool, bool, uint32_t, CellKernel<float> *);

template <typename T>
__global__ void relayout_coef_kernel(T *out, const T *in, const uint32_t *cell_batch, const uint32_t *cell_pos,
                                     size_t total, int n) {
  const size_t i = (size_t)blockIdx.x * blockDim.x + threadIdx.x;
  if (i >= total) return;
  const int n2 = n * n, nd = n2 * n, NT = (64 / n) * n;
  const size_t cell = i / nd;
  const int q = (int)(i - cell * nd);
  const int x = q % n, r = q / n;
  out[((size_t)cell_batch[cell] * n2 + r) * NT + cell_pos[cell] * n + x] = in[i];
}

template <typename T>
hipError_t relayout_coef_launch(T *out, const T *in, const uint32_t *cell_batch, const uint32_t *cell_pos,
                                size_t total, int n, hipStream_t st) {
  if (total == 0) return hipSuccess;
  hipLaunchKernelGGL(relayout_coef_kernel<T>, dim3((unsigned)((total + 255) / 256)), dim3(256), 0, st, out, in,
                     cell_batch, cell_pos, total, n);
  return hipGetLastError();
}
template hipError_t relayout_coef_launch<double>(double *, const double *, const uint32_t *, const uint32_t *, size_t,
                                                 int, hipStream_t);
template hipError_t relayout_coef_launch<float>(float *, const float *, const uint32_t *, const uint32_t *, size_t, int,
                                                hipStream_t);

}
```

### dealii-cuda_amd/csrc/mfgpu_kernels_q.hip

```cpp
#include <hip/hip_runtime.h>

#include "mfgpu_cell.h"
#include "mfgpu_kernels.h"
#include "mfgpu_planes.h"

namespace mfgpu {

#define MFGPU_PIN_VMEM() __builtin_amdgcn_sched_barrier(0x380)

template <int n, typename T, bool ADD, bool HN, bool MASS = false>
__device__ __forceinline__ void planes4_body(const ApplyArgs<T> &A, const TablesEO<T, n> &tab) {
  constexpr int n2 = n * n;
  constexpr int CW = p_cells_per_wave(n);
  constexpr int NT = CW * n;
  constexpr int KGU = p_kgu(n);
  constexpr int JI = p_ji(n);
  constexpr int HS = KGU - JI;
  constexpr int SA = q_cell_stride(n);
  constexpr int ZS = q_plane_stride(n);
  constexpr int NIW = (n2 + 1) / 2;
  constexpr int PRIV = HN ? p_priv_max(n) : 0;
  constexpr int NUA = KGU * 64 + PRIV;
  extern __shared__ __attribute__((aligned(16))) unsigned char smem_raw[];
  double *ua = reinterpret_cast<double *>(smem_raw);
// ... 306 lines not shown
      for (int x = 0; x < n; ++x) rp[x] = Tw[pxy + x + n * y];
#pragma unroll
      for (int x = 0; x < n; ++x) s2[x] = w[x + n * y] + rp[x];
      eo_apply<n, 1>(tab, s2, ol);
      set_line<n, 0>(w, y, ol);
      hook(y);
    }
    WaveSync::sync();
#pragma unroll
    for (int j = 0; j < (NUA + 63) / 64; ++j) ua[lane + j * 64] = 0.0;
#pragma unroll
    for (int x = 0; x < n; ++x) {
      T in[n], out[n];
      get_line<n, 1>(w, x, in);
      eo_apply<n, 1>(tab, in, out);
      set_line<n, 1>(w, x, out);
      hook(n + x);
    }
    WaveSync::sync();
#pragma unroll
    for (int i = 0; i < n2; ++i)
      lds_add(reinterpret_cast<double *>(reinterpret_cast<char *>(ua) + ixb(IXc, i)), (double)w[i]);
    WaveSync::sync();

    if (HN && hn_ncopy) {
      double Wr[n2];
#pragma unroll
      for (int i = 0; i < n2; ++i) Wr[i] = Wl[i];
      hn_pass(2, true, Wr);
      WaveSync::sync();
      hn_pass(1, true, Wr);
      WaveSync::sync();
      hn_pass(0, true, Wr);
      WaveSync::sync();
      double cv[CR > 0 ? CR : 1];
#pragma unroll
      for (int r = 0; r < CR; ++r) cv[r] = (uint32_t)(r * 64 + lane) < hn_ncopy ? ua[Hc[r] >> 16] : 0.0;
#pragma unroll
      for (int r = 0; r < CR; ++r)
        if ((uint32_t)(r * 64 + lane) < hn_ncopy) lds_add(ua + (Hc[r] & 0xffffu), cv[r]);
      WaveSync::sync();
    }

    {
      T *const hp = A.halo + (size_t)b * (HS * 64) + lane;
#pragma unroll
      for (int j = 0; j < KGU; ++j) {
        const T r = (T)ua[lane + j * 64];
        if (j < JI) {
          T *const p = dst_at(Gc[j]);
          *p = ADD ? *p + r : r;
        } else {
          hp[(j - JI) * 64] = r;
        }
      }
    }
    WaveSync::sync();
    if (!has_next) break;
    b = b1;
    b1 = next_of(b1);
#pragma unroll
    for (int j = 0; j < KGU; ++j) Gc[j] = Gn[j];
#pragma unroll
    for (int w2 = 0; w2 < NIW; ++w2) IXc[w2] = lane_on ? IXn[w2] : kDummyIx;
    if (HN) {
#pragma unroll
      for (int w2 = 0; w2 < HROWS; ++w2) Hc[w2] = Hn[w2];
    }
  }
}

template <int n, typename T, bool ADD, bool HN, bool MASS = false>
__global__ void __launch_bounds__(64) __attribute__((amdgpu_waves_per_eu(2, 2)))
apply_planes4(const ApplyArgs<T> A, const TablesEO<T, n> tab) {
  planes4_body<n, T, ADD, HN, MASS>(A, tab);
}
template <int n, typename T, bool ADD>
__global__ void __launch_bounds__(64) __attribute__((amdgpu_waves_per_eu(1, 1)))
apply_planes4w(const ApplyArgs<T> A, const TablesEO<T, n> tab) {
  planes4_body<n, T, ADD, false>(A, tab);
}

template <typename T>
hipError_t q_bind(int, int n, bool hn, bool, bool sh, bool mass, uint32_t, CellKernel<T> *k) {
  return dispatch_instantiation(n, [&](auto N, auto HN, auto SH, auto MASS) {
    constexpr int n_ = N;
    if constexpr (!kernel_exists(PlaneKernel::planes4, n_, number_type_of<T>, HN, SH, MASS))
      return hipErrorInvalidValue;
    else if constexpr (planes4_wide(n_))
      return bind_cell_kernel<T, 64, apply_planes4w<n_, T, false>, apply_planes4w<n_, T, true>, make_tables_eo<T, n_>>(
          q_lds_bytes<T>(n_, false), k);
    else
      return bind_cell_kernel<T, 64, apply_planes4<n_, T, false, HN, MASS>, apply_planes4<n_, T, true, HN, MASS>,
                              make_tables_eo<T, n_>>(q_lds_bytes<T>(n_, HN), k);
  }, hn, sh, mass);
}
template hipError_t q_bind<double>(int, int, bool, bool, bool, bool, uint32_t, CellKernel<double> *);
template hipError_t q_bind<float>(int, int, bool, bool, bool, bool, uint32_t, CellKernel<float> *);

}
```

### dealii-cuda_amd/csrc/mfgpu_kernels_x.hip

```cpp
#include <hip/hip_runtime.h>

#include "mfgpu_cell.h"
#include "mfgpu_kernels.h"

namespace mfgpu {

template <int n, typename T, bool HN, bool MASS = false, typename StageNext>
__device__ __forceinline__ void cell_pipeline_x(const bool act, const bool acty, const bool actz, const int pa, const int pb,
                                                const unsigned mask, const bool any_mask, T (&u)[n],
                                                const uint32_t (&ixw)[(n + 1) / 2], double *acc, T *Wc, T *Rc, const T *cf,
                                                T *Wy, T *Ry, const T *Cy, T *Wz, T *Rz, const T *Cz, const T *Wl,
                                                const Tables<T, n> &tab, StageNext &&stage_next,
                                                const T *mz = nullptr) {

  constexpr int n2 = n * n;
  const int bx = n * pa + n2 * pb;
  T v[n], w[n], g[n], r[n];
  T mm[MASS ? n : 1];
  if (MASS && actz) {
#pragma unroll
    for (int s = 0; s < n; ++s) mm[s] = stream_load(mz + s * n2);
  }
  if (HN && any_mask) {
    bool type;
// ... 288 lines not shown
      const int base = k * CH;
      if (base >= ncell) continue;
      const bool act = lane_on && (base + lc < ncell);
      const int nxt = base + CH;
      int cnt_next = 0;
      if (nxt < ncell) {
        cnt_next = chunk_count(ncell, nxt);
        prefetch(c0 + nxt, cnt_next);
      } else if (has_nb) {
        cnt_next = chunk_count(ncelln, 0);
        prefetch(c0n, cnt_next);
      }
      if (k == KC - 1 && has_nb) load_src(Gn, SVn);
      if (k == 1 && has_nb) load_ix(c0n, ncelln, IXn);
      unsigned mask = 0;
      bool any_mask = false;
      if (HN) {
        if (act) mask = A.cmask[(size_t)c0 + base + lc];
        any_mask = __syncthreads_or(mask != 0) != 0;
      }
      const bool acty = oy >= 0 && base + cy < ncell, actz = oz >= 0 && base + cz < ncell;
      cell_pipeline_x<n, T, HN, MASS>(
          act, acty, actz, pa, pb, mask, any_mask, U[k], IX[k], ua, Wc, Rc, cf, Wb + oy, Rb + oy, Cb + oy, Wb + oz,
          Rb + oz, Cb + oz, Wl, tab,
          [&]() {
            if (cnt_next > 0) stage(cnt_next);
          },
          MASS && actz ? A.mass + ((size_t)c0 + base) * nd + oz : nullptr);
    }
    if (has_nb && ncell <= (KC - 1) * CH) {
      load_src(Gn, SVn);
      if (ncell <= CH) load_ix(c0n, ncelln, IXn);
    }
    __syncthreads();

    {
      const int l = lane();
      const double *ul = ua + l;
      T *hl = A.halo + hoff + l - nint;
#pragma unroll
      for (int j = 0; j < kPark; ++j) G[kGU - kPark + j] = Gp[j * kBlock + tid];
      T old[kGU];
      if (A.add) {
#pragma unroll
        for (int j = 0; j < kGU; ++j) old[j] = A.dst[G[j] & 0x7fffffffu];
      }
#pragma unroll
      for (int j = 0; j < kGU; ++j) {
        if (l < nint - j * kBlock) {
          if (!(G[j] >> 31)) A.dst[G[j]] = A.add ? old[j] + (T)ul[j * kBlock] : (T)ul[j * kBlock];
        } else if (l < nb - j * kBlock) {
          hl[j * kBlock] = (T)ul[j * kBlock];
        }
      }
    }
    if (!has_nb) break;
    b = bn;
    c0 = c0n;
    ncell = ncelln;
    d0 = d0n;
    nb = nbn;
    nint = nintn;
    hoff = hoffn;
#pragma unroll
    for (int j = 0; j < kGU; ++j) {
      G[j] = Gn[j];
      SV[j] = SVn[j];
    }
#pragma unroll
    for (int k = 0; k < KC; ++k)
#pragma unroll
      for (int q = 0; q < NW; ++q) IX[k][q] = IXn[k][q];
  }
}

template <int n, typename T>
static size_t x_lds_bytes(uint32_t nb_max) {
  constexpr int nd = n * n * n;
  constexpr int CH = 256 / (n * n);
  return (size_t)nb_max * sizeof(double) + (size_t)(3 * CH * nd + n * n) * sizeof(T) + 4 * 256 * sizeof(uint32_t);
}

template <typename T>
hipError_t x_bind(int, int n, bool hn, bool, bool sh, bool mass, uint32_t nb_max, CellKernel<T> *k) {
  return dispatch_instantiation(n, [&](auto N, auto HN, auto SH, auto MASS) {
    constexpr int n_ = N;
    if constexpr (kernel_exists(BatchKernel::x, n_, number_type_of<T>, HN, SH, MASS)) {
      constexpr auto K = apply_batches_x<n_, T, HN, MASS>;
      return bind_cell_kernel<T, 256, K, K, make_tables<T, n_>>(x_lds_bytes<n_, T>(nb_max), k);
    } else
      return hipErrorInvalidValue;
  }, hn, sh, mass);
}

#define INST(T) template hipError_t x_bind<T>(int, int, bool, bool, bool, bool, uint32_t, CellKernel<T> *);
INST(double)
INST(float)

}
```

### dealii-cuda_amd/csrc/mfgpu_plan.cpp

```cpp
#include <algorithm>
#include <cassert>
#include <cmath>
#include <cstring>
#include <numeric>
#include <unordered_map>

#include "mfgpu_internal.h"

namespace mfgpu {

static thread_local std::string g_err;
void set_error(const std::string &msg) { g_err = msg; }
const char *last_error() { return g_err.c_str(); }

int derive_tables(int n, const double *sv, const double *sg, std::vector<double> &S,
                  std::vector<double> &Dt) {
  std::vector<long double> A(n * n), B(n * n);
  for (int i = 0; i < n * n; ++i) {
    A[i] = sv[i];
    B[i] = sg[i];
  }
  for (int c = 0; c < n; ++c) {
    int piv = c;
    for (int r = c + 1; r < n; ++r)
// ... 730 lines not shown
  ix.assign((size_t)NIW * NT * nbat, dummy | (dummy << 16));
  std::vector<uint32_t> slot_of;
  const int HROWS = p_hn_rows(n), CR = p_priv_max(n) / 64;
  std::vector<uint32_t> &hnrec = P.pr_hn;
  hnrec.clear();
  P.pr_hn_slot.assign(nbat, 0xffffffffu);
  std::vector<HnLine> lines[3];
  std::vector<uint16_t> pnodes;
  std::vector<uint32_t> priv_pos((size_t)P.nd);
  for (size_t b = 0; b < nbat; ++b) {
    const uint32_t c0 = P.batch_cell_off[b], nc = P.batch_cell_off[b + 1] - c0;
    const uint32_t d0 = P.batch_dof_off[b], nbd = P.batch_dof_off[b + 1] - d0, ni = P.batch_nint[b];
    if ((int)nc * n > NT || (int)ni > JI || (int)(nbd - ni) >= NB - JI || nbd == ni) {
      set_error("internal: batch does not fit the plane kernel's dof-list slots");
      return MFGPU_EINVAL;
    }
    slot_of.assign(nbd, 0u);
    for (uint32_t t = 0; t < nbd; ++t) slot_of[t] = t < ni ? t : (uint32_t)JI + (t - ni);
    for (int t = 0; t < NB; ++t) {
      uint32_t src_t;
      if (t < JI) src_t = (uint32_t)t < ni ? (uint32_t)t : ni;
      else src_t = std::min<uint32_t>(ni + (uint32_t)(t - JI), nbd - 1);
      bd[b * NB + t] = P.bdofs[d0 + src_t];
    }
    bool hnb = false;
    if (constraint_mask && b >= P.n_plain_plane_batches)
      for (uint32_t c = 0; c < nc; ++c) hnb = hnb || constraint_mask[P.cell_order[c0 + c]] != 0;
    uint32_t next_priv = (uint32_t)NB;
    std::vector<uint32_t> copies, ops_d[3];
    for (uint32_t c = 0; c < nc; ++c) {
      const unsigned mask = hnb ? constraint_mask[P.cell_order[c0 + c]] : 0u;
      std::fill(priv_pos.begin(), priv_pos.end(), 0xffffffffu);
      if (mask) {
        hn_cell_lines(mask, n, lines, pnodes);
        for (uint16_t node : pnodes) {
          if (next_priv >= (uint32_t)NB + (uint32_t)p_priv_max(n)) {
            set_error("internal: batch exceeds the plane kernel's private hanging-node entries");
            return MFGPU_EINVAL;
          }
          priv_pos[node] = next_priv;
          copies.push_back((next_priv << 16) | slot_of[P.lmap[(size_t)(c0 + c) * P.nd + node]]);
          ++next_priv;
        }
        for (int dir = 0; dir < 3; ++dir)
          for (const HnLine &L : lines[dir]) {
            uint32_t w[3] = {0u, 0u, 0u};
            for (int t = 0; t < n; ++t) w[t >> 1] |= priv_pos[L.node[t]] << (16 * (t & 1));
            ops_d[dir].insert(ops_d[dir].end(), w, w + 3);
          }
      }
      for (int k = 0; k < n; ++k)
        for (int i = 0; i < n2; ++i) {
          const int node = i + n2 * k;
          const uint32_t pos = priv_pos[node] != 0xffffffffu ? priv_pos[node] : slot_of[P.lmap[(size_t)(c0 + c) * P.nd + node]];
          const uint32_t off = 8u * pos;
          uint32_t &w = ix[(b * NIW + i / 2) * NT + c * n + k];
          w = (i & 1) ? ((w & 0xffffu) | (off << 16)) : ((w & 0xffff0000u) | off);
        }
    }
    if (hnb) {
      P.pr_hn_slot[b] = (uint32_t)(hnrec.size() / ((size_t)HROWS * 64));
      hnrec.resize(hnrec.size() + (size_t)HROWS * 64, 0u);
      uint32_t *rec = hnrec.data() + (size_t)P.pr_hn_slot[b] * HROWS * 64;
      for (size_t e = 0; e < copies.size(); ++e) rec[e] = copies[e];
      for (int dir = 0; dir < 3; ++dir) {
        const size_t nops = ops_d[dir].size() / 3;
        if (nops > (size_t)kHnOpRounds * 64) {
          set_error("internal: more hanging-node lines in a batch than the plane kernel's record holds");
          return MFGPU_EINVAL;
        }
        for (size_t e = 0; e < nops; ++e)
          for (int w = 0; w < 3; ++w)
            rec[(size_t)(CR + (dir * kHnOpRounds + (int)(e / 64)) * 3 + w) * 64 + e % 64] = ops_d[dir][e * 3 + w];
      }
      const uint32_t h0 = (uint32_t)copies.size() | ((uint32_t)(ops_d[0].size() / 3) << 16);
      const uint32_t h1 = (uint32_t)(ops_d[1].size() / 3) | ((uint32_t)(ops_d[2].size() / 3) << 16);
      for (int l = 0; l < 64; ++l) {
        rec[(size_t)(HROWS - 2) * 64 + l] = h0;
        rec[(size_t)(HROWS - 1) * 64 + l] = h1;
      }
    }
  }
  share_plane_records(P);
  share_pass2_records(P);
  return 0;
}

namespace {
uint64_t hash_words(const uint32_t *w, size_t n) {
  uint64_t h = 1469598103934665603ull;
  for (size_t i = 0; i < n; ++i) h = (h ^ w[i]) * 1099511628211ull;
  return h;
}

using SeenRecords = std::unordered_multimap<uint64_t, std::pair<size_t, size_t>>;
size_t intern_record(std::vector<uint32_t> &table, SeenRecords &seen, const uint32_t *rec, size_t len) {
  const uint64_t h = hash_words(rec, len);
  const auto range = seen.equal_range(h);
  for (auto it = range.first; it != range.second; ++it)
    if (it->second.second == len && !std::memcmp(table.data() + it->second.first, rec, len * sizeof(uint32_t)))
      return it->second.first;
  const size_t off = table.size();
  table.insert(table.end(), rec, rec + len);
  seen.emplace(h, std::make_pair(off, len));
  return off;
}
}

void share_plane_records(Plan &P) {
  const int n = P.n, NT = p_cells_per_wave(n) * n, NIW = (n * n + 1) / 2;
  const size_t NB = (size_t)p_kgu(n) * 64, NX = (size_t)NIW * NT, nbat = P.n_plane_batches;
  P.sh_dofs.clear();
  P.sh_idx.clear();
  P.sh_batch.assign(nbat * kShBatchWords, 0u);
  SeenRecords seen_d, seen_x;
  std::vector<uint32_t> rel(NB);
  for (size_t b = 0; b < nbat; ++b) {
    const uint32_t *g = P.pr_dofs.data() + b * NB;
    uint32_t base = 0x7fffffffu;
    for (size_t t = 0; t < NB; ++t) base = std::min(base, g[t] & 0x7fffffffu);
    for (size_t t = 0; t < NB; ++t) rel[t] = g[t] - base;
    uint32_t *e = P.sh_batch.data() + b * kShBatchWords;
    e[0] = base;
    e[1] = (uint32_t)(intern_record(P.sh_dofs, seen_d, rel.data(), NB) / NB);
    e[2] = (uint32_t)(intern_record(P.sh_idx, seen_x, P.pr_idx.data() + b * NX, NX) / NX);
  }
  const size_t shared = P.sh_dofs.size() + P.sh_idx.size() + P.sh_batch.size();
  const size_t expanded = P.pr_dofs.size() + P.pr_idx.size();
  P.sh_use = nbat > 0 && P.pr_hn.empty() && (double)shared <= kShareMaxFraction * (double)expanded;
}

void share_pass2_records(Plan &P) {
  P.sh_p2rec.clear();
  P.sh_p2tab.clear();
  P.sh_p2_use = false;
  const size_t nb = P.batch_cell_off.size() - 1;
  const uint32_t hs = (uint32_t)p_hs(P.n) * 64u;
  if (nb == 0 || P.n_plane_batches != nb || P.halo_off.size() != nb + 1 || hs > (1u << kP2SlotBits)) return;
  for (size_t b = 0; b <= nb; ++b)
    if (P.halo_off[b] != (uint64_t)b * hs) return;
  std::vector<std::vector<uint32_t>> owned(nb);
  size_t expanded = 0;
  for (size_t i = 0; i < P.sdofs.size(); ++i) {
    const uint32_t k = P.s_off[i + 1] - P.s_off[i];
    expanded += 1 + (k ? k : 1);
    if (k == 0) continue;
    if (k > (uint32_t)kP2MaxK) return;
    const uint32_t owner = P.s_idx[P.s_off[i]] / hs;
    for (uint32_t t = 0; t < k; ++t) {
      const uint32_t tb = P.s_idx[P.s_off[i] + t] / hs;
      if (tb >= nb || tb < owner || tb - owner >= (1u << (32 - kP2SlotBits))) return;
    }
    owned[owner].push_back((uint32_t)i);
  }
  P.sh_p2tab.assign(2 * nb, 0u);
  SeenRecords seen;
  std::vector<uint32_t> rec;
  for (size_t b = 0; b < nb; ++b) {
    std::vector<uint32_t> &m = owned[b];
    auto k_of = [&](uint32_t i) { return P.s_off[i + 1] - P.s_off[i]; };
    std::stable_sort(m.begin(), m.end(), [&](uint32_t x, uint32_t y) { return k_of(x) > k_of(y); });
    const uint32_t base = P.sh_batch[b * kShBatchWords], ne = (uint32_t)m.size(), kmax = ne ? k_of(m[0]) : 0u;
    auto pad = [](uint32_t x) { return (x + 63u) & ~63u; };
    const uint32_t e0 = pad(ne);
    rec.assign(kP2Header, 0u);
    rec[0] = ne;
    rec[1] = e0;
    rec[2] = kmax;
    rec.resize(kP2Header + 2 * (size_t)e0, 0u);
    for (uint32_t e = 0; e < e0; ++e) rec[kP2Header + e] = e < ne ? P.sdofs[m[e]] - base : 0xffffffffu;
    for (uint32_t e = 0; e < ne; ++e) rec[kP2Header + e0 + e] = k_of(m[e]);
    for (uint32_t t = 0; t < kmax; ++t) {
      uint32_t cnt = 0;
      while (cnt < ne && k_of(m[cnt]) > t) ++cnt;
      rec[3 + t] = (uint32_t)rec.size();
      rec.resize(rec.size() + pad(cnt), 0u);
      for (uint32_t e = 0; e < cnt; ++e) {
        const uint32_t slot = P.s_idx[P.s_off[m[e]] + t], tb = slot / hs;
        rec[rec[3 + t] + e] = ((tb - (uint32_t)b) << kP2SlotBits) | (slot - tb * hs);
      }
    }
    P.sh_p2tab[2 * b] = base;
    P.sh_p2tab[2 * b + 1] = (uint32_t)intern_record(P.sh_p2rec, seen, rec.data(), rec.size());
  }
  const size_t shared = P.sh_p2rec.size() + P.sh_p2tab.size();
  P.sh_p2_use = (double)shared <= kShareMaxFraction * (double)expanded;
}

int choose_kernel_and_plan(const mfgpu_desc &d, PlaneKernel &pk, BatchKernel &bk, Plan &plan) {
  const bool general = !(d.flags & MFGPU_UNIFORM_J0), hn = (d.flags & MFGPU_HANGING_NODES) != 0;
  const bool colored = (d.flags & MFGPU_COLORED_SCATTER) != 0;
  if (d.kernel > MFGPU_KERNEL_PLANES_2W) {
    set_error("unknown mfgpu_desc.kernel");
    return MFGPU_EINVAL;
  }
  const bool pk_ok = d.dim == 3 && !general && !colored && d.degree >= 2 && d.degree <= 6 &&
                     d.n_dofs < (1u << 29);
  const bool xk_ok = d.dim == 3 && !general && !colored;
  const bool want_planes = d.kernel == MFGPU_KERNEL_PLANES || d.kernel == MFGPU_KERNEL_PLANES_2W;
  if ((want_planes && !pk_ok) || (d.kernel == MFGPU_KERNEL_PENCILS_X && !xk_ok) ||
      (d.kernel == MFGPU_KERNEL_PENCILS && general)) {
    set_error("mfgpu_desc.kernel: this kernel family does not cover the description (see include/mfgpu.h)");
    return MFGPU_EUNSUPPORTED;
  }
  const bool planes4 = d.kernel == MFGPU_KERNEL_PLANES_2W || d.degree >= 5 ||
                       (d.kernel == MFGPU_KERNEL_AUTO && d.degree == 3 && d.number_type == MFGPU_F64);
  const PlaneKernel plane_kind = planes4 ? PlaneKernel::planes4 : PlaneKernel::planes3;
  const bool mass = d.mass_coefficient != nullptr;
  auto plane_kernel_exists = [&](bool with_hn) {
    return kernel_exists(plane_kind, d.degree + 1, d.number_type, with_hn, false, mass);
  };
  const bool mass_without_planes = mass && pk_ok && !plane_kernel_exists(false);
// ... 140 lines not shown
size_t mfgpu_desc_size(void) { return sizeof(mfgpu_desc); }

int mfgpu_suggest_renumbering(const mfgpu_desc *desc, uint32_t *new_index) {
  if (!desc || !new_index) {
    mfgpu::set_error("null argument");
    return MFGPU_EINVAL;
  }
  mfgpu::Plan P;
  mfgpu::PlaneKernel pk;
  mfgpu::BatchKernel bk;
  mfgpu_desc d = *desc;
  d.mass_coefficient = nullptr;
  int rc = mfgpu::choose_kernel_and_plan(d, pk, bk, P);
  if (rc) return rc;
  const uint32_t NONE = 0xffffffffu;
  std::fill(new_index, new_index + desc->n_dofs, NONE);
  uint32_t next = 0;
  const size_t nb = P.batch_cell_off.size() - 1;
  for (size_t b = 0; b < nb; ++b) {
    const uint32_t d0 = P.batch_dof_off[b];
    const uint32_t ni = P.batch_nint.empty() ? P.batch_dof_off[b + 1] - d0 : P.batch_nint[b];
    for (uint32_t t = 0; t < ni; ++t) {
      const uint32_t g = P.bdofs[d0 + t] & 0x7fffffffu;
      if (new_index[g] == NONE) new_index[g] = next++;
    }
  }
  for (uint32_t e : P.sdofs) {
    const uint32_t g = e & 0x7fffffffu;
    if (new_index[g] == NONE) new_index[g] = next++;
  }
  for (uint32_t g = 0; g < desc->n_dofs; ++g)
    if (new_index[g] == NONE) new_index[g] = next++;
  if (next != desc->n_dofs) {
    mfgpu::set_error("internal: renumbering is not a permutation");
    return MFGPU_EINVAL;
  }
  return 0;
}

int64_t mfgpu_plan_array_u32(const mfgpu_plan *p, int what, const uint32_t **ptr) {
  if (!p || !ptr) return MFGPU_EINVAL;
  const std::vector<uint32_t> *v = nullptr;
  switch (what) {
    case 0: v = &p->plan.batch_cell_off; break;
    case 1: v = &p->plan.batch_dof_off; break;
    case 2: v = &p->plan.color_batch_off; break;
    case 3: v = &p->plan.cell_order; break;
    case 4: v = &p->plan.bdofs; break;
    case 5: v = &p->plan.orphans; break;
    case 6: v = &p->plan.batch_nint; break;
    case 7: v = &p->plan.halo_off; break;
    case 8: v = &p->plan.sdofs; break;
    case 9: v = &p->plan.s_off; break;
    case 10: v = &p->plan.s_idx; break;
    case 11: v = &p->plan.chunks; break;
    case 12: v = &p->plan.gstarts; break;
    case 13: v = &p->plan.pr_dofs; break;
    case 14: v = &p->plan.pr_idx; break;
    case 15: v = &p->plan.pr_hn; break;
    case 16: v = &p->plan.pr_hn_slot; break;
    case 17: v = &p->plan.sh_dofs; break;
    case 18: v = &p->plan.sh_idx; break;
    case 19: v = &p->plan.sh_batch; break;
    case 20: v = &p->plan.sh_p2rec; break;
    case 21: v = &p->plan.sh_p2tab; break;
    default: mfgpu::set_error("bad array id"); return MFGPU_EINVAL;
  }
  *ptr = v->data();
  return (int64_t)v->size();
}

int mfgpu_plan_multi_groups(uint32_t n_vectors, const uint32_t *widths, uint32_t n_widths, uint32_t *groups,
                            uint32_t capacity) {
  if ((!widths && n_widths) || (!groups && capacity)) return MFGPU_EINVAL;
  const std::vector<uint32_t> g = mfgpu::multi_groups(n_vectors, std::vector<uint32_t>(widths, widths + n_widths));
  for (size_t i = 0; i < g.size() && i < capacity; ++i) groups[i] = g[i];
  return (int)g.size();
}

int mfgpu_plan_shares_records(const mfgpu_plan *p) {
  return p ? (p->plan.sh_use ? 1 : 0) | (p->plan.sh_p2_use ? 2 : 0) : 0;
}

int64_t mfgpu_plan_lmap(const mfgpu_plan *p, const uint16_t **ptr) {
  if (!p || !ptr) return MFGPU_EINVAL;
  *ptr = p->plan.lmap.data();
  return (int64_t)p->plan.lmap.size();
}

int64_t mfgpu_plan_bflags(const mfgpu_plan *p, const uint8_t **ptr) {
  if (!p || !ptr) return MFGPU_EINVAL;
  *ptr = p->plan.bflags.data();
  return (int64_t)p->plan.bflags.size();
}

}
```

### dealii-cuda_amd/pymfgpu/__init__.py

```python
from __future__ import annotations

import ctypes as C
import os

import numpy as np

_HERE = os.path.dirname(os.path.abspath(__file__))
LIB_PATH = os.environ.get("MFGPU_LIB") or os.path.join(os.path.dirname(_HERE), "lib", "libmfgpu.so")

F64, F32 = 0, 1
OK, EINVAL = 0, -1
EUNSUPPORTED = -4
MULTI_ADD, MULTI_LOOP, MULTI_FUSED = 1, 2, 4
UNIFORM_J0, HANGING_NODES, COLORED_SCATTER, NO_SHARED_RECORDS = 1, 2, 1 << 8, 1 << 9
UPDATABLE_COEFFICIENTS = 1 << 10
KERNEL_AUTO, KERNEL_PENCILS, KERNEL_PENCILS_X, KERNEL_PLANES, KERNEL_PLANES_2W = 0, 1, 2, 3, 4


class MfgpuError(RuntimeError):
    pass


class Desc(C.Structure):
    _fields_ = [
        ("dim", C.c_int32), ("degree", C.c_int32), ("number_type", C.c_int32), ("flags", C.c_uint32),
        ("n_dofs", C.c_uint32), ("n_cells", C.c_uint32),
        ("loc2glob", C.c_void_p), ("constraint_mask", C.c_void_p),
        ("JxW", C.c_void_p), ("inv_jac", C.c_void_p), ("coefficient", C.c_void_p),
        ("quadrature_points", C.c_void_p), ("shape_values", C.c_void_p), ("shape_gradients", C.c_void_p),
        ("constraint_weights", C.c_void_p), ("constrained_dofs", C.c_void_p),
        ("n_constrained", C.c_uint32), ("max_cells_per_batch", C.c_uint32), ("max_dofs_per_batch", C.c_uint32),
        ("kernel", C.c_uint32), ("cell_loop_segments", C.c_uint32), ("max_workgroups", C.c_uint32),
        ("mass_coefficient", C.c_void_p),
    ]


CG_NONE, CG_JACOBI, CG_CHEBYSHEV, CG_CALLBACK = 0, 1, 2, 3
CG_STATE_BYTES, CG_PARTIAL_BYTES = 128, 3 * 2048 * 8


class CGInfo(C.Structure):
    _fields_ = [("iterations", C.c_uint32), ("status", C.c_uint32), ("residual", C.c_double),
                ("initial_residual", C.c_double)]

    def as_tuple(self):
        return int(self.iterations), int(self.status), float(self.residual), float(self.initial_residual)


VCYCLE_COARSE_AUTO, VCYCLE_COARSE_DENSE, VCYCLE_COARSE_CG = 0, 1, 2
VCYCLE_DENSE_MAX = 2048
SPD_INVERSE_DEVICE_MAX = 512
EIG_STATE_BYTES, EIG_PARTIAL_BYTES = 64, 2 * 2048 * 8


class EigResult(C.Structure):
    _fields_ = [("lambda_max", C.c_double), ("estimate", C.c_double), ("steps", C.c_uint32), ("status", C.c_uint32)]


class VCycleRefreshInfo(C.Structure):
    _fields_ = [("coarse_status", C.c_uint32), ("eig_status_max", C.c_uint32), ("eig_steps_max", C.c_uint32),
                ("reserved", C.c_uint32)]


class VCycleLevelDesc(C.Structure):
    _fields_ = [("op", C.c_void_p), ("edges", C.c_void_p), ("from_coarser", C.c_void_p), ("to_mg", C.c_void_p),
                ("from_mg", C.c_void_p)]


class VCycleDesc(C.Structure):
    _fields_ = [("n_levels", C.c_uint32), ("levels", C.POINTER(VCycleLevelDesc)), ("active_type", C.c_int32),
                ("n_active", C.c_uint32), ("smoother_degree", C.c_uint32), ("smoothing_range", C.c_double),
                ("eig_iterations", C.c_uint32), ("lambda_max", C.POINTER(C.c_double)), ("coarse", C.c_uint32),
                ("coarse_tolerance", C.c_double), ("coarse_max_iterations", C.c_uint32)]


CG_CALLBACK_TYPE = C.CFUNCTYPE(C.c_int, C.c_void_p, C.c_void_p, C.c_void_p, C.c_void_p)


SYMBOLS = [
    "mfgpu_vmult_multi", "mfgpu_multi_width", "mfgpu_plan_multi_groups",
    "mfgpu_create", "mfgpu_vmult", "mfgpu_vmult_add", "mfgpu_n_dofs", "mfgpu_memory_consumption",
    "mfgpu_destroy", "mfgpu_last_error", "mfgpu_plan_stats", "mfgpu_kernel_name", "mfgpu_compute_inverse_diagonal", "mfgpu_set_constrained_values",
    "mfgpu_vec_sadd", "mfgpu_vec_equ", "mfgpu_vec_scale", "mfgpu_vec_divide", "mfgpu_vec_invert", "mfgpu_vec_mul",
    "mfgpu_vec_dot", "mfgpu_vec_l2_norm", "mfgpu_vec_add_and_dot", "mfgpu_vec_all_zero", "mfgpu_profile_enable", "mfgpu_profile_read", "mfgpu_profile_read_pass2",
    "mfgpu_plan_create", "mfgpu_plan_destroy", "mfgpu_plan_array_u32", "mfgpu_plan_lmap", "mfgpu_plan_bflags",
    "mfgpu_plan_shares_records", "mfgpu_record_stats",
    "mfgpu_vec_alloc", "mfgpu_vec_free", "mfgpu_vec_fill", "mfgpu_vec_from_host", "mfgpu_vec_to_host",
    "mfgpu_device_synchronize", "mfgpu_device_memory_info", "mfgpu_mesh_create_uniform", "mfgpu_mesh_create_adaptive", "mfgpu_mesh_create_ball", "mfgpu_mesh_create_from_leaves",
    "mfgpu_mesh_cell_levels", "mfgpu_mesh_destroy",
    "mfgpu_mesh_desc", "mfgpu_mesh_dof_coords", "mfgpu_mesh_interface_dofs",
    "mfgpu_dist_unique_id", "mfgpu_dist_create", "mfgpu_dist_connect_local", "mfgpu_dist_attach", "mfgpu_dist_schedule",
    "mfgpu_vmult_dist_begin", "mfgpu_vmult_dist_end", "mfgpu_vmult_dist", "mfgpu_dist_destroy",
    "mfgpu_transfer_create", "mfgpu_transfer_create_from_meshes", "mfgpu_transfer_prolongate",
    "mfgpu_transfer_restrict_and_add", "mfgpu_transfer_memory_consumption", "mfgpu_transfer_destroy",
    "mfgpu_mesh_transfer_patches", "mfgpu_suggest_renumbering", "mfgpu_mesh_renumber",
    "mfgpu_level_create", "mfgpu_level_operator", "mfgpu_level_vmult_interface_down", "mfgpu_level_vmult_interface_up",
    "mfgpu_level_destroy", "mfgpu_index_pairs_create", "mfgpu_vec_copy_pairs", "mfgpu_index_pairs_destroy",
    "mfgpu_mesh_create_adaptive_mg", "mfgpu_mg_hierarchy_create", "mfgpu_mg_n_levels", "mfgpu_mg_level_mesh",
    "mfgpu_mg_edge_dofs", "mfgpu_mg_copy_pairs", "mfgpu_mg_transfer_arrays", "mfgpu_mg_hierarchy_destroy",
    "mfgpu_integrator_create", "mfgpu_integrator_rhs", "mfgpu_integrator_l2_error", "mfgpu_integrator_error_points",
    "mfgpu_integrator_destroy",
    "mfgpu_vec_convert", "mfgpu_vec_copy_pairs_convert", "mfgpu_vec_chebyshev_start", "mfgpu_vec_chebyshev_update",
    "mfgpu_desc_size",
    "mfgpu_update_coefficients", "mfgpu_level_update_coefficients", "mfgpu_integrator_update_coefficients",
    "mfgpu_integrator_evaluate",
    "mfgpu_cg_create", "mfgpu_cg_set_callback", "mfgpu_cg_begin", "mfgpu_cg_iterate", "mfgpu_cg_status", "mfgpu_cg_solve",
    "mfgpu_cg_memory_consumption", "mfgpu_cg_destroy", "mfgpu_cg_chebyshev_scalars",
    "mfgpu_cg_begin_relative", "mfgpu_cg_set_vcycle", "mfgpu_transfer_prolongate_add", "mfgpu_vec_residual",
    "mfgpu_vcycle_create", "mfgpu_vcycle_apply", "mfgpu_vcycle_lambda_max", "mfgpu_vcycle_memory_consumption",
    "mfgpu_vcycle_destroy", "mfgpu_estimate_lambda_max", "mfgpu_spd_inverse",
    "mfgpu_vec_chebyshev_start_dev", "mfgpu_vec_chebyshev_update_dev", "mfgpu_cg_chebyshev_scalars_dev",
    "mfgpu_eig_workspace_bytes", "mfgpu_estimate_lambda_max_enqueue", "mfgpu_spd_inverse_workspace_bytes",
    "mfgpu_spd_inverse_enqueue", "mfgpu_vcycle_refresh", "mfgpu_vcycle_refresh_status", "mfgpu_estimate_lambda_max_steps",
    "mfgpu_transfer_create_p", "mfgpu_transfer_create_p_from_meshes", "mfgpu_transfer_p_prolongation_1d",
    "mfgpu_transfer_create_p_hn", "mfgpu_transfer_create_p_hn_from_meshes", "mfgpu_transfer_p_owner_list",
    "mfgpu_mesh_coarsen_leaves", "mfgpu_mesh_coarsening_map", "mfgpu_transfer_create_h_hn",
    "mfgpu_transfer_create_h_hn_from_meshes",
    "mfgpu_integrator_recovery_indicator", "mfgpu_mesh_refine_leaves",
    "mfgpu_mesh_adapt_leaves", "mfgpu_transfer_create_h_hn_interp", "mfgpu_transfer_create_h_hn_interp_from_meshes",
    "mfgpu_transfer_interpolate",
    "mfgpu_locate_points", "mfgpu_points_create", "mfgpu_points_create_in_cells", "mfgpu_points_cells",
    "mfgpu_points_n_not_found", "mfgpu_points_evaluate", "mfgpu_points_integrate", "mfgpu_points_memory_consumption",
    "mfgpu_points_destroy",
    "mfgpu_locator_create", "mfgpu_locator_locate", "mfgpu_locator_memory_consumption", "mfgpu_locator_destroy",
    "mfgpu_points_create_located",
]

_lib = None


def lib():
    global _lib
    if _lib is None:
        if not os.path.exists(LIB_PATH):
            raise MfgpuError(f"{LIB_PATH} not found: build it with __graft_entry__.build() "
                             "(make -C dealii-cuda_amd); there is no fallback path")
        L = C.CDLL(LIB_PATH)
        L.mfgpu_last_error.restype = C.c_char_p
        L.mfgpu_create.argtypes = [C.POINTER(Desc), C.POINTER(C.c_void_p)]
        L.mfgpu_desc_size.argtypes = []
        L.mfgpu_desc_size.restype = C.c_size_t
        L.mfgpu_vmult.argtypes = [C.c_void_p, C.c_void_p, C.c_void_p, C.c_void_p]
        L.mfgpu_vmult_add.argtypes = [C.c_void_p, C.c_void_p, C.c_void_p, C.c_void_p]
        L.mfgpu_n_dofs.argtypes = [C.c_void_p]
        L.mfgpu_n_dofs.restype = C.c_uint32
        L.mfgpu_memory_consumption.argtypes = [C.c_void_p]
        L.mfgpu_memory_consumption.restype = C.c_size_t
        L.mfgpu_destroy.argtypes = [C.c_void_p]
        L.mfgpu_destroy.restype = None
        L.mfgpu_plan_stats.argtypes = [C.c_void_p, C.POINTER(C.c_uint64)]
        L.mfgpu_device_memory_info.argtypes = [C.POINTER(C.c_size_t), C.POINTER(C.c_size_t)]
        L.mfgpu_kernel_name.argtypes = [C.c_void_p]
        L.mfgpu_kernel_name.restype = C.c_char_p
        L.mfgpu_compute_inverse_diagonal.argtypes = [C.c_void_p, C.c_void_p, C.c_void_p]
        L.mfgpu_set_constrained_values.argtypes = [C.c_void_p, C.c_void_p, C.c_double, C.c_void_p]
        vp, d, z, i = C.c_void_p, C.c_double, C.c_size_t, C.c_int
        L.mfgpu_vec_sadd.argtypes = [vp, d, d, vp, z, i, vp]
        L.mfgpu_vec_equ.argtypes = [vp, d, vp, z, i, vp]
        L.mfgpu_vec_scale.argtypes = [vp, vp, z, i, vp]
        L.mfgpu_vec_divide.argtypes = [vp, vp, z, i, vp]
        L.mfgpu_vec_invert.argtypes = [vp, z, i, vp]
        L.mfgpu_vec_mul.argtypes = [vp, d, z, i, vp]
        L.mfgpu_vec_dot.argtypes = [vp, vp, z, i, vp, C.POINTER(d)]
        L.mfgpu_vec_l2_norm.argtypes = [vp, z, i, vp, C.POINTER(d)]
        L.mfgpu_vec_add_and_dot.argtypes = [vp, d, vp, vp, z, i, vp, C.POINTER(d)]
        L.mfgpu_vec_all_zero.argtypes = [vp, z, i, vp, C.POINTER(i)]
        L.mfgpu_profile_enable.argtypes = [C.c_void_p, C.c_int]
        L.mfgpu_profile_read.argtypes = [C.c_void_p, C.POINTER(C.c_double), C.POINTER(C.c_uint64)]
        L.mfgpu_profile_read_pass2.argtypes = [C.c_void_p, C.POINTER(C.c_double)]
        L.mfgpu_plan_create.argtypes = [C.POINTER(Desc), C.POINTER(C.c_void_p)]
        L.mfgpu_plan_destroy.argtypes = [C.c_void_p]
        L.mfgpu_plan_destroy.restype = None
        L.mfgpu_plan_array_u32.argtypes = [C.c_void_p, C.c_int, C.POINTER(C.c_void_p)]
        L.mfgpu_plan_array_u32.restype = C.c_int64
        L.mfgpu_plan_lmap.argtypes = [C.c_void_p, C.POINTER(C.c_void_p)]
        L.mfgpu_plan_lmap.restype = C.c_int64
        L.mfgpu_plan_bflags.argtypes = [C.c_void_p, C.POINTER(C.c_void_p)]
        L.mfgpu_plan_bflags.restype = C.c_int64
        L.mfgpu_plan_shares_records.argtypes = [C.c_void_p]
        L.mfgpu_record_stats.argtypes = [C.c_void_p, C.POINTER(C.c_uint64)]
        L.mfgpu_vec_alloc.argtypes = [C.POINTER(C.c_void_p), C.c_size_t, C.c_int]
        L.mfgpu_vec_free.argtypes = [C.c_void_p]
        L.mfgpu_vec_fill.argtypes = [C.c_void_p, C.c_size_t, C.c_int, C.c_double, C.c_void_p]
        L.mfgpu_vec_from_host.argtypes = [C.c_void_p, C.c_void_p, C.c_size_t, C.c_int]
        L.mfgpu_vec_to_host.argtypes = [C.c_void_p, C.c_void_p, C.c_size_t, C.c_int]
        L.mfgpu_mesh_create_uniform.argtypes = [C.c_int, C.c_int, C.POINTER(C.c_uint32), C.c_double, C.c_double,
                                                C.c_uint32, C.c_uint32, C.c_int, C.POINTER(C.c_void_p)]
        L.mfgpu_mesh_create_adaptive.argtypes = [C.c_int, C.c_int, C.c_int, C.c_int, C.POINTER(C.c_void_p)]
        L.mfgpu_mesh_create_ball.argtypes = [C.c_int, C.c_int, C.c_int, C.c_int, C.POINTER(C.c_void_p)]
        L.mfgpu_mesh_create_from_leaves.argtypes = [C.c_int, C.c_int, C.c_void_p, C.c_uint32, C.c_int, C.POINTER(C.c_void_p)]
        L.mfgpu_mesh_cell_levels.argtypes = [C.c_void_p, C.POINTER(C.c_void_p)]
        L.mfgpu_mesh_cell_levels.restype = C.c_int64
        L.mfgpu_mesh_destroy.argtypes = [C.c_void_p]
        L.mfgpu_mesh_destroy.restype = None
        L.mfgpu_mesh_desc.argtypes = [C.c_void_p, C.POINTER(Desc)]
        L.mfgpu_mesh_dof_coords.argtypes = [C.c_void_p, C.POINTER(C.c_void_p)]
        L.mfgpu_mesh_dof_coords.restype = C.c_int64
        L.mfgpu_mesh_interface_dofs.argtypes = [C.c_void_p, C.c_int, C.POINTER(C.c_void_p)]
        L.mfgpu_mesh_interface_dofs.restype = C.c_int64
        L.mfgpu_transfer_create.argtypes = [C.c_int, C.c_int, C.c_int, C.c_uint32, C.c_void_p, C.c_void_p, C.c_uint32,
                                            C.c_uint32, C.c_void_p, C.c_uint32, C.c_void_p, C.POINTER(C.c_void_p)]
        L.mfgpu_transfer_create_from_meshes.argtypes = [C.c_void_p, C.c_void_p, C.POINTER(C.c_void_p)]
        L.mfgpu_transfer_prolongate.argtypes = [C.c_void_p, C.c_void_p, C.c_void_p, C.c_void_p]
        L.mfgpu_transfer_restrict_and_add.argtypes = [C.c_void_p, C.c_void_p, C.c_void_p, C.c_void_p]
        L.mfgpu_transfer_memory_consumption.argtypes = [C.c_void_p]
        L.mfgpu_transfer_memory_consumption.restype = C.c_size_t
        L.mfgpu_mesh_transfer_patches.argtypes = [C.c_void_p, C.c_void_p, C.c_void_p, C.c_void_p]
        L.mfgpu_mesh_transfer_patches.restype = C.c_int64
        L.mfgpu_suggest_renumbering.argtypes = [C.POINTER(Desc), C.c_void_p]
        L.mfgpu_mesh_renumber.argtypes = [C.c_void_p, C.c_void_p]
        L.mfgpu_level_create.argtypes = [C.POINTER(Desc), C.c_void_p, C.c_uint32, C.POINTER(C.c_void_p)]
        L.mfgpu_level_operator.argtypes = [C.c_void_p]
        L.mfgpu_level_operator.restype = C.c_void_p
        L.mfgpu_level_vmult_interface_down.argtypes = [C.c_void_p, C.c_void_p, C.c_void_p, C.c_void_p]
        L.mfgpu_level_vmult_interface_up.argtypes = [C.c_void_p, C.c_void_p, C.c_void_p, C.c_void_p]
        L.mfgpu_mesh_create_adaptive_mg.argtypes = [C.c_int, C.c_int, C.c_int, C.c_int, C.POINTER(C.c_void_p)]
        L.mfgpu_mg_hierarchy_create.argtypes = [C.c_void_p, C.POINTER(C.c_void_p)]
        L.mfgpu_mg_n_levels.argtypes = [C.c_void_p]
        L.mfgpu_mg_level_mesh.argtypes = [C.c_void_p, C.c_int]
        L.mfgpu_mg_level_mesh.restype = C.c_void_p
        L.mfgpu_mg_edge_dofs.argtypes = [C.c_void_p, C.c_int, C.POINTER(C.c_void_p)]
        L.mfgpu_mg_edge_dofs.restype = C.c_int64
        L.mfgpu_mg_copy_pairs.argtypes = [C.c_void_p, C.c_int, C.POINTER(C.c_void_p), C.POINTER(C.c_void_p)]
        L.mfgpu_mg_copy_pairs.restype = C.c_int64
        L.mfgpu_mg_transfer_arrays.argtypes = [C.c_void_p, C.c_int, C.POINTER(C.c_void_p), C.POINTER(C.c_void_p)]
        L.mfgpu_mg_transfer_arrays.restype = C.c_int64
        L.mfgpu_mg_hierarchy_destroy.argtypes = [C.c_void_p]
        L.mfgpu_mg_hierarchy_destroy.restype = None
        L.mfgpu_index_pairs_create.argtypes = [C.c_void_p, C.c_void_p, C.c_uint32, C.POINTER(C.c_void_p)]
        L.mfgpu_vec_copy_pairs.argtypes = [C.c_void_p, C.c_void_p, C.c_void_p, C.c_int, C.c_void_p]
        L.mfgpu_index_pairs_destroy.argtypes = [C.c_void_p]
        L.mfgpu_index_pairs_destroy.restype = None
        L.mfgpu_level_destroy.argtypes = [C.c_void_p]
        L.mfgpu_level_destroy.restype = None
        L.mfgpu_transfer_destroy.argtypes = [C.c_void_p]
        L.mfgpu_transfer_destroy.restype = None
        L.mfgpu_integrator_create.argtypes = [C.POINTER(Desc), C.POINTER(C.c_void_p)]
        L.mfgpu_integrator_rhs.argtypes = [C.c_void_p, C.c_void_p, C.c_void_p, C.c_void_p, C.c_void_p]
        L.mfgpu_integrator_l2_error.argtypes = [C.c_void_p, C.c_void_p, C.c_void_p, C.c_void_p, C.c_void_p,
                                                C.POINTER(C.c_double)]
        L.mfgpu_integrator_error_points.argtypes = [C.c_void_p, C.c_void_p, C.c_void_p]
        L.mfgpu_integrator_destroy.argtypes = [C.c_void_p]
        L.mfgpu_integrator_destroy.restype = None
        L.mfgpu_vec_convert.argtypes = [vp, i, vp, i, z, vp]
        L.mfgpu_update_coefficients.argtypes = [vp, vp, vp, vp]
        L.mfgpu_level_update_coefficients.argtypes = [vp, vp, vp, vp]
        L.mfgpu_integrator_update_coefficients.argtypes = [vp, vp, vp, vp]
        L.mfgpu_integrator_evaluate.argtypes = [vp, vp, vp, vp, vp]
        L.mfgpu_vec_copy_pairs_convert.argtypes = [vp, vp, i, vp, i, vp]
        L.mfgpu_vec_chebyshev_start.argtypes = [vp, vp, vp, vp, vp, vp, d, i, z, i, vp]
        L.mfgpu_vec_chebyshev_update.argtypes = [vp, vp, vp, vp, vp, d, d, z, i, vp]
        L.mfgpu_vmult_multi.argtypes = [vp, vp, vp, C.c_uint32, z, C.c_uint32, vp]
        L.mfgpu_multi_width.argtypes = [vp]
        L.mfgpu_plan_multi_groups.argtypes = [C.c_uint32, C.POINTER(C.c_uint32), C.c_uint32, C.POINTER(C.c_uint32),
                                              C.c_uint32]
        u32 = C.c_uint32
        L.mfgpu_cg_create.argtypes = [vp, i, vp, u32, d, d, C.POINTER(vp)]
        L.mfgpu_cg_set_callback.argtypes = [vp, CG_CALLBACK_TYPE, vp]
        L.mfgpu_cg_begin.argtypes = [vp, vp, vp, d, u32, vp]
        L.mfgpu_cg_iterate.argtypes = [vp, u32, vp]
        L.mfgpu_cg_status.argtypes = [vp, vp, C.POINTER(CGInfo)]
        L.mfgpu_cg_solve.argtypes = [vp, vp, vp, d, u32, u32, vp, C.POINTER(CGInfo)]
        L.mfgpu_cg_memory_consumption.argtypes = [vp]
        L.mfgpu_cg_memory_consumption.restype = C.c_size_t
        L.mfgpu_cg_destroy.argtypes = [vp]
        L.mfgpu_cg_destroy.restype = None
        L.mfgpu_cg_chebyshev_scalars.argtypes = [u32, d, d, C.POINTER(d)]
        L.mfgpu_cg_begin_relative.argtypes = [vp, vp, vp, d, u32, vp]
        L.mfgpu_cg_set_vcycle.argtypes = [vp, vp]
        L.mfgpu_transfer_prolongate_add.argtypes = [vp, vp, vp, vp]
        L.mfgpu_vec_residual.argtypes = [vp, vp, vp, z, i, vp]
        L.mfgpu_vcycle_create.argtypes = [C.POINTER(VCycleDesc), C.POINTER(vp)]
        L.mfgpu_vcycle_apply.argtypes = [vp, vp, vp, vp]
        L.mfgpu_vcycle_lambda_max.argtypes = [vp, C.POINTER(d)]
        L.mfgpu_vcycle_memory_consumption.argtypes = [vp]
        L.mfgpu_vcycle_memory_consumption.restype = C.c_size_t
        L.mfgpu_vcycle_destroy.argtypes = [vp]
        L.mfgpu_vcycle_destroy.restype = None
        L.mfgpu_estimate_lambda_max.argtypes = [vp, vp, u32, C.POINTER(d)]
        L.mfgpu_spd_inverse.argtypes = [u32, vp, vp]
        L.mfgpu_vec_chebyshev_start_dev.argtypes = [vp, vp, vp, vp, vp, vp, vp, i, z, i, vp]
        L.mfgpu_vec_chebyshev_update_dev.argtypes = [vp, vp, vp, vp, vp, vp, z, i, vp]
        L.mfgpu_cg_chebyshev_scalars_dev.argtypes = [u32, vp, d, vp, vp]
        L.mfgpu_eig_workspace_bytes.argtypes = [u32, i]
        L.mfgpu_eig_workspace_bytes.restype = C.c_size_t
        L.mfgpu_estimate_lambda_max_enqueue.argtypes = [vp, vp, u32, u32, vp, vp]
        L.mfgpu_spd_inverse_workspace_bytes.argtypes = [u32]
        L.mfgpu_spd_inverse_workspace_bytes.restype = C.c_size_t
        L.mfgpu_spd_inverse_enqueue.argtypes = [u32, vp, u32, vp, u32, vp, vp, vp]
        L.mfgpu_vcycle_refresh.argtypes = [vp, u32, vp]
        L.mfgpu_estimate_lambda_max_steps.argtypes = [vp, vp, u32, C.POINTER(d), C.POINTER(u32)]
        L.mfgpu_vcycle_refresh_status.argtypes = [vp, vp, C.POINTER(VCycleRefreshInfo)]
        L.mfgpu_transfer_create_p.argtypes = [i, i, i, i, u32, vp, vp, u32, u32, vp, u32, vp, C.POINTER(vp)]
        L.mfgpu_transfer_create_p_from_meshes.argtypes = [vp, vp, C.POINTER(vp)]
        L.mfgpu_transfer_p_prolongation_1d.argtypes = [i, i, vp]
        L.mfgpu_transfer_create_p_hn.argtypes = [i, i, i, i, u32, vp, vp, u32, u32, vp, u32, vp, vp, vp, C.POINTER(vp)]
        L.mfgpu_transfer_create_p_hn_from_meshes.argtypes = [vp, vp, C.POINTER(vp)]
        L.mfgpu_transfer_p_owner_list.argtypes = [i, i, u32, vp, vp, u32, vp]
        L.mfgpu_mesh_coarsen_leaves.argtypes = [i, vp, u32, vp]
        L.mfgpu_mesh_coarsen_leaves.restype = C.c_int64
        L.mfgpu_mesh_coarsening_map.argtypes = [vp, vp, vp, vp]
        L.mfgpu_transfer_create_h_hn.argtypes = [i, i, i, u32, u32, vp, vp, vp, vp, u32, u32, vp, u32, vp, vp, vp, vp,
                                                 C.POINTER(vp)]
        L.mfgpu_transfer_create_h_hn_from_meshes.argtypes = [vp, vp, C.POINTER(vp)]
        L.mfgpu_integrator_recovery_indicator.argtypes = [vp, vp, vp, vp, vp]
        L.mfgpu_mesh_refine_leaves.argtypes = [i, vp, u32, vp, u32, vp, C.c_uint64]
        L.mfgpu_mesh_refine_leaves.restype = C.c_int64
        L.mfgpu_mesh_adapt_leaves.argtypes = [i, vp, u32, vp, vp, u32, vp, C.c_uint64, vp, C.POINTER(u32)]
        L.mfgpu_mesh_adapt_leaves.restype = C.c_int64
        L.mfgpu_transfer_create_h_hn_interp.argtypes = [i, i, i, u32, u32, vp, vp, vp, vp, u32, u32, vp, u32, vp, vp, vp, vp,
                                                        vp, C.POINTER(vp)]
        L.mfgpu_transfer_create_h_hn_interp_from_meshes.argtypes = [vp, vp, C.POINTER(vp)]
        L.mfgpu_transfer_interpolate.argtypes = [vp, vp, vp, vp]
        L.mfgpu_locate_points.argtypes = [C.POINTER(Desc), vp, u32, vp, vp, C.POINTER(u32)]
        L.mfgpu_points_create.argtypes = [vp, C.POINTER(Desc), vp, u32, C.POINTER(vp)]
        L.mfgpu_points_create_in_cells.argtypes = [vp, vp, vp, u32, C.POINTER(vp)]
        L.mfgpu_points_cells.argtypes = [vp, C.POINTER(vp)]
        L.mfgpu_points_cells.restype = C.c_int64
        L.mfgpu_points_n_not_found.argtypes = [vp]
        L.mfgpu_points_n_not_found.restype = u32
        L.mfgpu_points_evaluate.argtypes = [vp, vp, vp, vp, vp]
        L.mfgpu_points_integrate.argtypes = [vp, vp, vp, vp]
        L.mfgpu_points_memory_consumption.argtypes = [vp]
        L.mfgpu_points_memory_consumption.restype = C.c_size_t
        L.mfgpu_points_destroy.argtypes = [vp]
        L.mfgpu_points_destroy.restype = None
        L.mfgpu_locator_create.argtypes = [vp, C.POINTER(Desc), C.POINTER(vp)]
        L.mfgpu_locator_locate.argtypes = [vp, vp, u32, vp, vp, vp, vp, vp]
        L.mfgpu_locator_memory_consumption.argtypes = [vp]
        L.mfgpu_locator_memory_consumption.restype = C.c_size_t
        L.mfgpu_locator_destroy.argtypes = [vp]
        L.mfgpu_locator_destroy.restype = None
        L.mfgpu_points_create_located.argtypes = [vp, vp, vp, u32, vp, C.POINTER(vp)]
        _lib = L
    return _lib


def _check(rc):
    if rc != 0:
        err = MfgpuError(f"mfgpu error {rc}: {lib().mfgpu_last_error().decode()}")
        err.code = rc
        raise err


def np_dtype(number_type):
    return np.float64 if number_type == F64 else np.float32


def _view(ptr, count, dtype):
    if count <= 0 or not ptr:
        return np.zeros(0, dtype=dtype)
    buf = (C.c_char * (count * np.dtype(dtype).itemsize)).from_address(ptr)
    return np.frombuffer(buf, dtype=dtype, count=count)


class Mesh:

    def __init__(self, handle, keep=None):
        self._h = handle
        self._keep = keep
        self.desc = Desc()
        _check(lib().mfgpu_mesh_desc(self._h, C.byref(self.desc)))

    @classmethod
    def uniform(cls, dim, degree, n_per_dir, lo=-1.0, hi=1.0, slab=(0, 0), number_type=F64):
        if np.isscalar(n_per_dir):
            n_per_dir = [int(n_per_dir)] * dim
        arr = (C.c_uint32 * 3)(*(list(n_per_dir) + [1] * (3 - len(n_per_dir))))
        h = C.c_void_p()
        _check(lib().mfgpu_mesh_create_uniform(dim, degree, arr, lo, hi, slab[0], slab[1], number_type, C.byref(h)))
        return cls(h)

    @classmethod
    def adaptive(cls, dim, degree, n_ref, number_type=F64):
        h = C.c_void_p()
        _check(lib().mfgpu_mesh_create_adaptive(dim, degree, n_ref, number_type, C.byref(h)))
        return cls(h)

    @classmethod
    def adaptive_mg(cls, dim, degree, n_ref, number_type=F64):
        h = C.c_void_p()
        _check(lib().mfgpu_mesh_create_adaptive_mg(dim, degree, n_ref, number_type, C.byref(h)))
        return cls(h)

    @classmethod
    def ball(cls, dim, degree, n_ref, number_type=F64):
        h = C.c_void_p()
        _check(lib().mfgpu_mesh_create_ball(dim, degree, n_ref, number_type, C.byref(h)))
        return cls(h)

    @classmethod
    def from_leaves(cls, dim, degree, leaves, number_type=F64):
        lv = np.ascontiguousarray(leaves, dtype=np.uint32).reshape(-1, 4)
        h = C.c_void_p()
        _check(lib().mfgpu_mesh_create_from_leaves(dim, degree, lv.ctypes.data, len(lv), number_type, C.byref(h)))
        return cls(h)

    @staticmethod
    def coarsen_leaves(dim, leaves):
        lv = np.ascontiguousarray(leaves, dtype=np.uint32).reshape(-1, 4)
        out = np.zeros((max(len(lv), 1), 4), dtype=np.uint32)
        n = lib().mfgpu_mesh_coarsen_leaves(dim, lv.ctypes.data if len(lv) else None, len(lv), out.ctypes.data)
        if n < 0:
            _check(int(n))
        return out[:n].copy()

    @staticmethod
    def refine_leaves(dim, leaves, flags, balance_vertices=False):
        lv = np.ascontiguousarray(leaves, dtype=np.uint32).reshape(-1, 4)
        fl = np.ascontiguousarray(np.asarray(flags) != 0, dtype=np.uint8).reshape(-1)
        if len(fl) != len(lv):
            raise MfgpuError("Mesh.refine_leaves: one flag per leaf")
        cap = max(len(lv), 1) * 2 ** dim
        out = np.zeros((cap, 4), dtype=np.uint32)
        n = lib().mfgpu_mesh_refine_leaves(dim, lv.ctypes.data if len(lv) else None, len(lv),
                                           fl.ctypes.data if len(fl) else None, int(bool(balance_vertices)),
                                           out.ctypes.data, cap)
        if n < 0:
            _check(int(n))
        return out[:n].copy()

    def refined(self, flags, degree=None, balance_vertices=False, number_type=None):
        leaves = self.cell_levels()
        if not len(leaves):
            raise MfgpuError("Mesh.refined: needs a leaf mesh (Mesh.adaptive, Mesh.adaptive_mg, Mesh.from_leaves)")
        dim = int(self.desc.dim)
        return Mesh.from_leaves(dim, int(self.desc.degree) if degree is None else int(degree),
# ... 135 lines not shown
            return None
        a = np.ascontiguousarray(a, dtype=dtype)
        keep.append(a)
        return a.ctypes.data

    d = Desc()
    d.dim, d.degree, d.number_type = dim, degree, number_type
    l2g = np.ascontiguousarray(loc2glob, dtype=np.uint32)
    d.n_dofs = int(n_dofs)
    d.n_cells = l2g.size // ((degree + 1) ** dim)
    uniform = np.asarray(inv_jac).size == d.n_cells
    assert uniform or np.asarray(inv_jac).size == l2g.size * dim * dim
    d.flags = ((UNIFORM_J0 if uniform else 0) | (HANGING_NODES if constraint_mask is not None else 0)
               | (COLORED_SCATTER if colored else 0))
    d.loc2glob = ptr(l2g, np.uint32)
    d.constraint_mask = ptr(constraint_mask, np.uint32)
    d.JxW = ptr(JxW, dt)
    d.inv_jac = ptr(inv_jac, dt)
    d.coefficient = ptr(coefficient, dt)
    d.quadrature_points = ptr(quadrature_points, dt)
    d.shape_values = ptr(shape_values, dt)
    d.shape_gradients = ptr(shape_gradients, dt)
    d.constraint_weights = ptr(constraint_weights, np.float64)
    c = np.ascontiguousarray(constrained, dtype=np.uint32)
    d.constrained_dofs = ptr(c, np.uint32)
    d.n_constrained = c.size
    d.max_cells_per_batch = max_cells_per_batch
    d.max_dofs_per_batch = max_dofs_per_batch
    d.kernel = kernel
    d.cell_loop_segments = cell_loop_segments
    d.max_workgroups = max_workgroups
    d.mass_coefficient = ptr(mass_coefficient, dt)
    return d, keep


class Plan:

    def __init__(self, desc: Desc, keep=None):
        self._keep = keep
        self.nd = (desc.degree + 1) ** desc.dim
        h = C.c_void_p()
        _check(lib().mfgpu_plan_create(C.byref(desc), C.byref(h)))
        self._h = h

    def __del__(self):
        if getattr(self, "_h", None) and _lib is not None:
            _lib.mfgpu_plan_destroy(self._h)
            self._h = None

    def _u32(self, what):
        p = C.c_void_p()
        cnt = lib().mfgpu_plan_array_u32(self._h, what, C.byref(p))
        if cnt < 0:
            _check(int(cnt))
        return _view(p.value, cnt, np.uint32).copy()

    batch_cell_off = property(lambda s: s._u32(0))
    batch_dof_off = property(lambda s: s._u32(1))
    color_batch_off = property(lambda s: s._u32(2))
    cell_order = property(lambda s: s._u32(3))
    bdofs = property(lambda s: s._u32(4) & np.uint32(0x7fffffff))
    bdofs_constrained = property(lambda s: (s._u32(4) >> np.uint32(31)).astype(bool))
    orphans = property(lambda s: s._u32(5))
    batch_nint = property(lambda s: s._u32(6))
    halo_off = property(lambda s: s._u32(7))
    sdofs = property(lambda s: s._u32(8))
    s_off = property(lambda s: s._u32(9))
    s_idx = property(lambda s: s._u32(10))
    chunks = property(lambda s: s._u32(11).reshape(-1, 4))
    gstarts = property(lambda s: s._u32(12))
    pr_dofs = property(lambda s: s._u32(13))
    pr_idx = property(lambda s: s._u32(14))
    pr_hn = property(lambda s: s._u32(15))
    pr_hn_slot = property(lambda s: s._u32(16))
    sh_dofs = property(lambda s: s._u32(17))
    sh_idx = property(lambda s: s._u32(18))
    sh_batch = property(lambda s: s._u32(19).reshape(-1, 4))
    shares_records = property(lambda s: bool(lib().mfgpu_plan_shares_records(s._h) & 1))
    sh_p2rec = property(lambda s: s._u32(20))
    sh_p2tab = property(lambda s: s._u32(21).reshape(-1, 2))
    shares_pass2_records = property(lambda s: bool(lib().mfgpu_plan_shares_records(s._h) & 2))

    @property
    def lmap(self):
        p = C.c_void_p()
        cnt = lib().mfgpu_plan_lmap(self._h, C.byref(p))
        return _view(p.value, cnt, np.uint16).reshape(-1, self.nd).copy()

    @property
    def bflags(self):
        p = C.c_void_p()
        cnt = lib().mfgpu_plan_bflags(self._h, C.byref(p))
        return _view(p.value, cnt, np.uint8).copy()


class DeviceVector:

    def __init__(self, n, number_type=F64):
        self.n, self.number_type = int(n), number_type
        p = C.c_void_p()
        _check(lib().mfgpu_vec_alloc(C.byref(p), self.n, number_type))
        self.ptr = p.value

    @classmethod
    def view(cls, ptr, n, number_type=F64):
        v = cls.__new__(cls)
        v.n, v.number_type, v.ptr, v._borrowed = int(n), number_type, int(ptr), True
        return v

    def __del__(self):
        if getattr(self, "ptr", None) and _lib is not None and not getattr(self, "_borrowed", False):
            _lib.mfgpu_vec_free(self.ptr)
            self.ptr = None

    def fill(self, value, stream=None):
        _check(lib().mfgpu_vec_fill(self.ptr, self.n, self.number_type, float(value), stream))

    def from_host(self, a):
        a = np.ascontiguousarray(a, dtype=np_dtype(self.number_type))
        assert a.size == self.n
        _check(lib().mfgpu_vec_from_host(self.ptr, a.ctypes.data, self.n, self.number_type))

    def to_host(self):
        a = np.empty(self.n, dtype=np_dtype(self.number_type))
        _check(lib().mfgpu_vec_to_host(a.ctypes.data, self.ptr, self.n, self.number_type))
        return a

    def swap(self, other):
        self.ptr, other.ptr = other.ptr, self.ptr
        self.n, other.n = other.n, self.n

    def _a(self, other=None):
        if other is not None:
            assert other.n == self.n and other.number_type == self.number_type
        return self.n, self.number_type

    def sadd(self, s, a, w, stream=None):
        _check(lib().mfgpu_vec_sadd(self.ptr, float(s), float(a), w.ptr, *self._a(w), stream))

    def add(self, a, w, stream=None):
        self.sadd(1.0, a, w, stream)

    def equ(self, a, w, stream=None):
        _check(lib().mfgpu_vec_equ(self.ptr, float(a), w.ptr, *self._a(w), stream))

    def scale(self, w, stream=None):
        _check(lib().mfgpu_vec_scale(self.ptr, w.ptr, *self._a(w), stream))

    def divide(self, w, stream=None):
        _check(lib().mfgpu_vec_divide(self.ptr, w.ptr, *self._a(w), stream))

    def invert(self, stream=None):
        _check(lib().mfgpu_vec_invert(self.ptr, *self._a(), stream))

    def mul(self, a, stream=None):
        _check(lib().mfgpu_vec_mul(self.ptr, float(a), *self._a(), stream))

    def dot(self, w, stream=None):
        r = C.c_double()
        _check(lib().mfgpu_vec_dot(self.ptr, w.ptr, *self._a(w), stream, C.byref(r)))
        return r.value

    def l2_norm(self, stream=None):
        r = C.c_double()
        _check(lib().mfgpu_vec_l2_norm(self.ptr, *self._a(), stream, C.byref(r)))
        return r.value

    def add_and_dot(self, a, x, w, stream=None):
        r = C.c_double()
        self._a(x)
        _check(lib().mfgpu_vec_add_and_dot(self.ptr, float(a), x.ptr, w.ptr, *self._a(w), stream, C.byref(r)))
        return r.value

    def all_zero(self, stream=None):
        r = C.c_int()
        _check(lib().mfgpu_vec_all_zero(self.ptr, *self._a(), stream, C.byref(r)))
        return bool(r.value)


class Operator:

    def __init__(self, desc: Desc, keep=None):
        self._keep = keep
        self.number_type = desc.number_type
        h = C.c_void_p()
        _check(lib().mfgpu_create(C.byref(desc), C.byref(h)))
        self._h = h

    def __del__(self):
        self.clear()

    def clear(self):
        if getattr(self, "_h", None) and _lib is not None:
            _lib.mfgpu_destroy(self._h)
            self._h = None

    def n(self):
        return int(lib().mfgpu_n_dofs(self._h))

    m = n

    def vmult(self, dst, src, stream=None):
        _check(lib().mfgpu_vmult(self._h, _ptr(dst), _ptr(src), stream))

    def vmult_add(self, dst, src, stream=None):
        _check(lib().mfgpu_vmult_add(self._h, _ptr(dst), _ptr(src), stream))

    def vmult_multi(self, dst, src, n_vectors, stride=None, add=False, mode=None, stream=None):
        flags = (MULTI_ADD if add else 0) | (mode or 0)
        _check(lib().mfgpu_vmult_multi(self._h, _ptr(dst), _ptr(src), int(n_vectors),
                                       self.n() if stride is None else int(stride), flags, stream))

    def multi_width(self):
        return int(lib().mfgpu_multi_width(self._h))

    def memory_consumption(self):
        return int(lib().mfgpu_memory_consumption(self._h))

    def plan_stats(self):
        s = (C.c_uint64 * 8)()
        _check(lib().mfgpu_plan_stats(self._h, s))
        keys = ["n_batches", "n_launches", "batch_dofs", "max_batch_dofs", "max_batch_cells", "n_orphans",
                "first_touch_or_shared_dofs", "rmw_adds_or_halo_slots"]
        out = dict(zip(keys, [int(v) for v in s]))
        r = (C.c_uint64 * 4)()
        _check(lib().mfgpu_record_stats(self._h, r))
        out.update(index_records="shared" if r[0] & 1 else "expanded",
                   pass2_records="shared" if r[0] & 2 else "expanded", distinct_dof_records=int(r[1]),
                   distinct_index_records=int(r[2]), index_record_bytes=int(r[3]))
        return out

    def kernel_name(self):
        return lib().mfgpu_kernel_name(self._h).decode()

    def compute_inverse_diagonal(self, inv_diag, stream=None):
        _check(lib().mfgpu_compute_inverse_diagonal(self._h, _ptr(inv_diag), stream))

    def set_constrained_values(self, vec, value, stream=None):
        _check(lib().mfgpu_set_constrained_values(self._h, _ptr(vec), float(value), stream))

    def update_coefficients(self, coef=None, mass=None, stream=None):
        _check(lib().mfgpu_update_coefficients(self._h, _optr(coef), _optr(mass), stream))

    def profile_enable(self, on=True):
        _check(lib().mfgpu_profile_enable(self._h, int(on)))

    def profile_read(self):
        ms, nv = C.c_double(), C.c_uint64()
        _check(lib().mfgpu_profile_read(self._h, C.byref(ms), C.byref(nv)))
        return ms.value, int(nv.value)

    def profile_read_pass2(self):
        ms = C.c_double()
        _check(lib().mfgpu_profile_read_pass2(self._h, C.byref(ms)))
        return ms.value


def cg_chebyshev_scalars(degree, lambda_max, smoothing_range):
    out = (C.c_double * max(2 * int(degree) - 1, 1))()
    _check(lib().mfgpu_cg_chebyshev_scalars(int(degree), float(lambda_max), float(smoothing_range), out))
    return np.array(out[:2 * int(degree) - 1], dtype=np.float64)


class CG:

    def __init__(self, op: "Operator", preconditioner=CG_NONE, inv_diag=None, degree=0, lambda_max=0.0,
                 smoothing_range=0.0, callback=None):
        self._op, self._inv_diag = op, inv_diag
        self._cb = self._cb_error = None
        self.n, self.number_type = op.n(), op.number_type
        h = C.c_void_p()
        _check(lib().mfgpu_cg_create(op._h, int(preconditioner), _optr(inv_diag), int(degree), float(lambda_max),
                                     float(smoothing_range), C.byref(h)))
        self._h = h
        if callback is not None:
            self.set_callback(callback)

    def set_callback(self, callback):
        def trampoline(_ctx, z, r, stream):
            try:
                rc = callback(DeviceVector.view(z, self.n, self.number_type),
                              DeviceVector.view(r, self.n, self.number_type), stream)
                return 0 if rc is None else int(rc)
            except Exception as e:
                self._cb_error = e
                return EINVAL

        cb = CG_CALLBACK_TYPE(trampoline)
        _check(lib().mfgpu_cg_set_callback(self._h, cb, None))
        self._cb = cb

    def _done(self, rc, check):
        e, self._cb_error = self._cb_error, None
        if e is not None:
            raise e
        return _check(rc) if check else rc

    def destroy(self):
        if getattr(self, "_h", None) and _lib is not None:
            _lib.mfgpu_cg_destroy(self._h)
            self._h = None

    __del__ = destroy

    def begin(self, x, b, tolerance, max_iterations, stream=None, check=True):
        return self._done(lib().mfgpu_cg_begin(self._h, _optr(x), _optr(b), float(tolerance), int(max_iterations), stream),
                          check)

    def begin_relative(self, x, b, relative_tolerance, max_iterations, stream=None, check=True):
        return self._done(lib().mfgpu_cg_begin_relative(self._h, _optr(x), _optr(b), float(relative_tolerance),
                                                        int(max_iterations), stream), check)

# ... 774 lines not shown
```

### include/mfgpu.h

```cpp
#ifndef MFGPU_H
#define MFGPU_H

#include <stddef.h>
#include <stdint.h>

#ifdef __cplusplus
extern "C" {
#endif

#define MFGPU_OK 0
#define MFGPU_EINVAL (-1)
#define MFGPU_EHIP (-2)
#define MFGPU_ENOMEM (-3)
#define MFGPU_EUNSUPPORTED (-4)

#define MFGPU_F64 0
#define MFGPU_F32 1

#define MFGPU_UNIFORM_J0 (1u << 0)
#define MFGPU_HANGING_NODES (1u << 1)

#define MFGPU_COLORED_SCATTER (1u << 8)

#define MFGPU_NO_SHARED_RECORDS (1u << 9)

#define MFGPU_UPDATABLE_COEFFICIENTS (1u << 10)

typedef struct mfgpu_handle mfgpu_handle;

typedef struct mfgpu_desc {
  int32_t dim;
  int32_t degree;
  int32_t number_type;
  uint32_t flags;
  uint32_t n_dofs;
  uint32_t n_cells;
  const uint32_t *loc2glob;
  const uint32_t *constraint_mask;
  const void *JxW;
  const void *inv_jac;
  const void *coefficient;
  const void *quadrature_points;
  const void *shape_values;
  const void *shape_gradients;
  const double *constraint_weights;
  const uint32_t *constrained_dofs;
  uint32_t n_constrained;
  uint32_t max_cells_per_batch;
  uint32_t max_dofs_per_batch;
  uint32_t kernel;
  uint32_t cell_loop_segments;
  uint32_t max_workgroups;
  const void *mass_coefficient;
} mfgpu_desc;

size_t mfgpu_desc_size(void);

#define MFGPU_KERNEL_AUTO 0
#define MFGPU_KERNEL_PENCILS 1
#define MFGPU_KERNEL_PENCILS_X 2
#define MFGPU_KERNEL_PLANES 3
#define MFGPU_KERNEL_PLANES_2W 4


int mfgpu_create(const mfgpu_desc *desc, mfgpu_handle **out);

int mfgpu_vmult(mfgpu_handle *h, void *dst_dev, const void *src_dev, void *stream);

int mfgpu_vmult_add(mfgpu_handle *h, void *dst_dev, const void *src_dev, void *stream);

#define MFGPU_MULTI_ADD   (1u << 0)
#define MFGPU_MULTI_LOOP  (1u << 1)
#define MFGPU_MULTI_FUSED (1u << 2)

int mfgpu_vmult_multi(mfgpu_handle *h, void *dst_dev, const void *src_dev, uint32_t n_vectors, size_t stride,
                      uint32_t flags, void *stream);
int mfgpu_multi_width(const mfgpu_handle *h);

int mfgpu_update_coefficients(mfgpu_handle *h, const void *coefficient_dev, const void *mass_coefficient_dev,
                              void *stream);

uint32_t mfgpu_n_dofs(const mfgpu_handle *h);

size_t mfgpu_memory_consumption(const mfgpu_handle *h);

void mfgpu_destroy(mfgpu_handle *h);

const char *mfgpu_last_error(void);

int mfgpu_plan_stats(const mfgpu_handle *h, uint64_t stats[8]);

int mfgpu_record_stats(const mfgpu_handle *h, uint64_t stats[4]);

const char *mfgpu_kernel_name(const mfgpu_handle *h);

int mfgpu_profile_enable(mfgpu_handle *h, int on);
int mfgpu_profile_read(mfgpu_handle *h, double *kernel_ms_total, uint64_t *n_vmults);
int mfgpu_profile_read_pass2(mfgpu_handle *h, double *pass2_ms_total);

typedef struct mfgpu_plan mfgpu_plan;
int mfgpu_plan_create(const mfgpu_desc *desc, mfgpu_plan **out);
void mfgpu_plan_destroy(mfgpu_plan *p);
int64_t mfgpu_plan_array_u32(const mfgpu_plan *p, int what, const uint32_t **ptr);
int mfgpu_plan_shares_records(const mfgpu_plan *p);
int mfgpu_plan_multi_groups(uint32_t n_vectors, const uint32_t *widths, uint32_t n_widths, uint32_t *groups,
                            uint32_t capacity);
int64_t mfgpu_plan_lmap(const mfgpu_plan *p, const uint16_t **ptr);
int64_t mfgpu_plan_bflags(const mfgpu_plan *p, const uint8_t **ptr);

int mfgpu_suggest_renumbering(const mfgpu_desc *desc, uint32_t *new_index );

int mfgpu_compute_inverse_diagonal(mfgpu_handle *h, void *inv_diag, void *stream);
int mfgpu_set_constrained_values(mfgpu_handle *h, void *vec, double value, void *stream);

int mfgpu_vec_sadd(void *v, double s, double a, const void *w, size_t n, int number_type, void *stream);
int mfgpu_vec_equ(void *v, double a, const void *w, size_t n, int number_type, void *stream);
int mfgpu_vec_scale(void *v, const void *w, size_t n, int number_type, void *stream);
int mfgpu_vec_divide(void *v, const void *w, size_t n, int number_type, void *stream);
int mfgpu_vec_invert(void *v, size_t n, int number_type, void *stream);
int mfgpu_vec_mul(void *v, double a, size_t n, int number_type, void *stream);
int mfgpu_vec_dot(const void *v, const void *w, size_t n, int number_type, void *stream, double *result);
int mfgpu_vec_l2_norm(const void *v, size_t n, int number_type, void *stream, double *result);
int mfgpu_vec_add_and_dot(void *v, double a, const void *x, const void *w, size_t n, int number_type,
                          void *stream, double *result);
int mfgpu_vec_all_zero(const void *v, size_t n, int number_type, void *stream, int *result);

int mfgpu_vec_alloc(void **dev, size_t n, int number_type);
int mfgpu_vec_free(void *dev);
int mfgpu_vec_fill(void *dev, size_t n, int number_type, double value, void *stream);
int mfgpu_vec_from_host(void *dev, const void *host, size_t n, int number_type);
int mfgpu_vec_to_host(void *host, const void *dev, size_t n, int number_type);
int mfgpu_device_synchronize(void);
int mfgpu_device_memory_info(size_t *free_bytes, size_t *total_bytes);

typedef struct mfgpu_dist mfgpu_dist;
int mfgpu_dist_unique_id(void *id128);
int mfgpu_dist_create(const void *id128, int rank, int world, const uint32_t *lower_ids, uint32_t n_lower,
                      const uint32_t *upper_ids, uint32_t n_upper, const uint32_t *constrained_dofs,
                      uint32_t n_constrained, uint32_t n_dofs, int number_type, mfgpu_dist **out);
int mfgpu_dist_connect_local(mfgpu_dist *lower_rank, mfgpu_dist *upper_rank);
int mfgpu_dist_attach(mfgpu_dist *d, mfgpu_handle *h);
int mfgpu_dist_schedule(const mfgpu_dist *d, uint32_t info[4]);
int mfgpu_vmult_dist_begin(mfgpu_handle *h, mfgpu_dist *d, void *dst_dev, const void *src_dev, void *stream);
int mfgpu_vmult_dist_end(mfgpu_handle *h, mfgpu_dist *d, void *dst_dev, void *stream);
int mfgpu_vmult_dist(mfgpu_handle *h, mfgpu_dist *d, void *dst_dev, const void *src_dev, void *stream);
void mfgpu_dist_destroy(mfgpu_dist *d);

typedef struct mfgpu_transfer mfgpu_transfer;
int mfgpu_transfer_create(int dim, int degree, int number_type, uint32_t n_coarse_cells,
                          const uint32_t *coarse_cell_dofs ,
                          const uint32_t *fine_patch_dofs  , uint32_t n_coarse_dofs,
                          uint32_t n_fine_dofs, const uint32_t *coarse_dirichlet, uint32_t n_coarse_dirichlet,
                          const double *prolongation_1d ,
                          mfgpu_transfer **out);
int mfgpu_transfer_prolongate(mfgpu_transfer *t, void *dst_fine_dev, const void *src_coarse_dev, void *stream);
int mfgpu_transfer_restrict_and_add(mfgpu_transfer *t, void *dst_coarse_dev, const void *src_fine_dev, void *stream);
int mfgpu_transfer_prolongate_add(mfgpu_transfer *t, void *dst_fine_dev, const void *src_coarse_dev, void *stream);
size_t mfgpu_transfer_memory_consumption(const mfgpu_transfer *t);
void mfgpu_transfer_destroy(mfgpu_transfer *t);

int mfgpu_transfer_create_p(int dim, int degree_coarse, int degree_fine, int number_type, uint32_t n_cells,
                            const uint32_t *coarse_cell_dofs ,
                            const uint32_t *fine_cell_dofs , uint32_t n_coarse_dofs,
                            uint32_t n_fine_dofs, const uint32_t *coarse_dirichlet, uint32_t n_coarse_dirichlet,
                            const double *prolongation_1d ,
                            mfgpu_transfer **out);
int mfgpu_transfer_p_prolongation_1d(int degree_coarse, int degree_fine, double *p1);
int mfgpu_transfer_create_p_hn(int dim, int degree_coarse, int degree_fine, int number_type, uint32_t n_cells,
                               const uint32_t *coarse_cell_dofs ,
                               const uint32_t *fine_cell_dofs , uint32_t n_coarse_dofs,
                               uint32_t n_fine_dofs, const uint32_t *coarse_dirichlet, uint32_t n_coarse_dirichlet,
                               const double *prolongation_1d ,
                               const uint32_t *constraint_mask ,
                               const double *coarse_constraint_weights , mfgpu_transfer **out);
int mfgpu_transfer_p_owner_list(int dim, int degree_fine, uint32_t n_cells, const uint32_t *fine_cell_dofs,
                                const uint32_t *constraint_mask , uint32_t n_fine_dofs,
                                uint32_t *out );
int mfgpu_transfer_create_h_hn(int dim, int degree, int number_type, uint32_t n_coarse_cells, uint32_t n_fine_cells,
                               const uint32_t *coarse_cell_dofs ,
                               const uint32_t *fine_cell_dofs ,
                               const uint32_t *parent , const uint32_t *child ,
                               uint32_t n_coarse_dofs, uint32_t n_fine_dofs, const uint32_t *coarse_dirichlet,
                               uint32_t n_coarse_dirichlet, const double *prolongation_1d ,
                               const uint32_t *coarse_mask ,
                               const uint32_t *fine_mask ,
                               const double *constraint_weights , mfgpu_transfer **out);

// ... 204 lines not shown
```

Measured before the change: 81.91 billion DoFs/s.

## Add paired-access plane records that gather and scatter adjacent DoFs as pairs

Adds a new record format for the planes3 f64 shared-record kernel in which consecutive global DoF indices are grouped into pairs. Each lane then loads and stores two values per access (16-byte pair loads and stores, aligned pair writes to the halo) and reads index words as uint4. The goal is to halve the number of gather and scatter instructions and index loads in the memory-bound vmult. The cost is extra host-side planning, a masked staging step for the pairs, and a fallback to the old path when a record cannot be fully paired.

```diff
diff --git a/dealii-cuda_amd/csrc/mfgpu_api.hip b/dealii-cuda_amd/csrc/mfgpu_api.hip
--- a/dealii-cuda_amd/csrc/mfgpu_api.hip
+++ b/dealii-cuda_amd/csrc/mfgpu_api.hip
@@ -64,6 +64,7 @@
   DeviceArray<uint32_t> d_bdofsp, d_idxp;
   DeviceArray<uint32_t> d_shtab;
   bool shared_records = false;
+  bool paired_access = false;
   size_t record_bytes = 0;
   DeviceArray<uint32_t> d_hnrec;
   DeviceArray<uint32_t> d_hn_slot;
@@ -124,13 +125,14 @@
 namespace {
 
 template <typename T>
-hipError_t bind_kernel(const mfgpu_handle *h, PlaneKernel pk, BatchKernel bk, bool hn, bool sh, CellKernel<T> *k) {
+hipError_t bind_kernel(const mfgpu_handle *h, PlaneKernel pk, BatchKernel bk, bool hn, bool sh, bool pa,
+                       CellKernel<T> *k) {
   const Plan &P = h->plan;
   const auto bind = pk == PlaneKernel::planes3 ? p_bind<T> : pk == PlaneKernel::planes4 ? q_bind<T>
                     : bk == BatchKernel::batches ? apply_bind<T> : bk == BatchKernel::x ? x_bind<T>
                     : bk == BatchKernel::g ? g_bind<T> : bk == BatchKernel::g2 ? g2_bind<T> : nullptr;
   if (!bind) return hipErrorInvalidValue;
-  return bind(P.dim, P.n, hn, h->twopass, sh, h->d_mass.get() != nullptr, P.max_batch_dofs, k);
+  return bind(P.dim, P.n, hn, h->twopass, sh, h->d_mass.get() != nullptr, pa, P.max_batch_dofs, k);
 }
 
 template <typename T, typename Args>
@@ -273,7 +275,9 @@
     }
     h->shared_records = P.sh_use && !(d.flags & MFGPU_NO_SHARED_RECORDS) &&
                         kernel_exists(h->planes, P.n, d.number_type, false, true, d.mass_coefficient != nullptr);
-    const std::vector<uint32_t> &rd = h->shared_records ? P.sh_dofs : P.pr_dofs;
+    h->paired_access = h->shared_records && P.pa_use && kPairedAccessDefault && !(d.flags & MFGPU_NO_PAIRED_ACCESS) &&
+                       kernel_exists(h->planes, P.n, d.number_type, false, true, d.mass_coefficient != nullptr, true);
+    const std::vector<uint32_t> &rd = h->paired_access ? P.pa_rec : h->shared_records ? P.sh_dofs : P.pr_dofs;
     const std::vector<uint32_t> &rx = h->shared_records ? P.sh_idx : P.pr_idx;
     if ((rc = up(h->d_bdofsp, rd.data(), rd.size()))) return rc;
     if ((rc = up(h->d_idxp, rx.data(), rx.size()))) return rc;
@@ -355,16 +359,16 @@
   h->max_workgroups = d.max_workgroups;
   if (h->planes != PlaneKernel::none) {
     CellKernel<T> &plain = h->kernel<T>(mfgpu_handle::kPlain), &masked = h->kernel<T>(mfgpu_handle::kMasked);
-    HIP_TRY(bind_kernel<T>(h, h->planes, BatchKernel::none, false, h->shared_records, &plain));
+    HIP_TRY(bind_kernel<T>(h, h->planes, BatchKernel::none, false, h->shared_records, h->paired_access, &plain));
     h->lds = plain.lds;
     if (P.n_plain_plane_batches < P.n_plane_batches) {
-      HIP_TRY(bind_kernel<T>(h, h->planes, BatchKernel::none, true, false, &masked));
+      HIP_TRY(bind_kernel<T>(h, h->planes, BatchKernel::none, true, false, false, &masked));
       h->lds = std::max(h->lds, masked.lds);
     }
   }
   if (h->batches == BatchKernel::none) return 0;
   CellKernel<T> &batch = h->kernel<T>(mfgpu_handle::kBatch);
-  const hipError_t bind_batch_family = bind_kernel<T>(h, PlaneKernel::none, h->batches, h->hn, false, &batch);
+  const hipError_t bind_batch_family = bind_kernel<T>(h, PlaneKernel::none, h->batches, h->hn, false, false, &batch);
   h->lds = batch.lds;
   if (h->lds > 160 * 1024) {
     set_error("batch needs more than 160 KiB of LDS; lower max_dofs_per_batch");
@@ -926,7 +930,7 @@
   const Plan &P = h->plan;
   const size_t n = (size_t)P.n, nb = (size_t)p_kgu((int)n) * 64, nx = ((n * n + 1) / 2) * (p_cells_per_wave((int)n) * n);
   const bool planes = h->planes != PlaneKernel::none;
-  s[0] = (h->shared_records ? 1 : 0) | (h->p2_shared ? 2 : 0);
+  s[0] = (h->shared_records ? 1 : 0) | (h->p2_shared ? 2 : 0) | (h->paired_access ? 4 : 0);
   s[1] = planes ? P.sh_dofs.size() / nb : 0;
   s[2] = planes ? P.sh_idx.size() / nx : 0;
   s[3] = h->record_bytes;
diff --git a/dealii-cuda_amd/csrc/mfgpu_internal.h b/dealii-cuda_amd/csrc/mfgpu_internal.h
--- a/dealii-cuda_amd/csrc/mfgpu_internal.h
+++ b/dealii-cuda_amd/csrc/mfgpu_internal.h
@@ -21,6 +21,12 @@
 constexpr int p_ji(int n) { return n == 3 ? 2 : n == 4 ? 5 : n == 5 ? 9 : n == 6 ? 14 : 23; }
 constexpr int p_hs(int n) { return n == 3 ? 3 : n == 4 ? 6 : n == 5 ? 9 : n == 6 ? 14 : 18; }
 constexpr int p_kgu(int n) { return p_ji(n) + p_hs(n); }
+constexpr int p_pa_gr(int n) { return (p_kgu(n) + 1) / 2; }
+constexpr int p_pa_sr(int n) { return (p_ji(n) + 1) / 2; }
+constexpr int p_pa_gq(int n) { return (p_pa_gr(n) + 3) / 4; }
+constexpr int p_pa_sq(int n) { return (2 * p_pa_sr(n) + 3) / 4; }
+constexpr int p_pa_quads(int n) { return 2 * p_pa_gq(n) + p_pa_sq(n); }
+constexpr size_t p_pa_word(int q0, int w, int lane) { return ((size_t)(q0 + w / 4) * 64 + lane) * 4 + w % 4; }
 constexpr int p_cell_stride(int n) {
   int s = n * n * n;
   while ((s & 31) != (n & 31)) ++s;
@@ -71,6 +77,8 @@
   std::vector<uint32_t> pr_dofs, pr_idx, pr_hn, pr_hn_slot;
   std::vector<uint32_t> sh_dofs, sh_idx, sh_batch;
   bool sh_use = false;
+  std::vector<uint32_t> pa_rec;
+  bool pa_use = false;
   std::vector<uint32_t> sh_p2rec, sh_p2tab;
   bool sh_p2_use = false;
   uint64_t n_first = 0, n_add = 0;
@@ -96,17 +104,19 @@
 int choose_kernel_and_plan(const mfgpu_desc &d, PlaneKernel &pk, BatchKernel &bk, Plan &plan);
 
 constexpr bool planes4_wide(int n) { return n >= 6; }
-constexpr bool kernel_exists(PlaneKernel k, int n, int number_type, bool hn, bool sh, bool mass) {
+constexpr bool kernel_exists(PlaneKernel k, int n, int number_type, bool hn, bool sh, bool mass, bool pa = false) {
   switch (k) {
-    case PlaneKernel::planes3: return n >= 3 && n <= 5 && !(sh && hn);
+    case PlaneKernel::planes3:
+      return n >= 3 && n <= 5 && !(sh && hn) && !(pa && !(sh && number_type == MFGPU_F64));
     case PlaneKernel::planes4:
-      return planes4_wide(n) ? n <= 7 && !hn && !sh && !mass
-                             : n >= 3 && !sh && !(mass && n == 5 && number_type == MFGPU_F64);
+      return planes4_wide(n) ? n <= 7 && !hn && !sh && !mass && !pa
+                             : n >= 3 && !sh && !pa && !(mass && n == 5 && number_type == MFGPU_F64);
     default: return false;
   }
 }
-constexpr bool kernel_exists(BatchKernel k, int n, int , bool , bool sh, bool ) {
-  return k != BatchKernel::none && n >= 2 && n <= 7 && !sh;
+constexpr bool kernel_exists(BatchKernel k, int n, int , bool , bool sh, bool ,
+                             bool pa = false) {
+  return k != BatchKernel::none && n >= 2 && n <= 7 && !sh && !pa;
 }
 constexpr int kFusedWidths[] = {3, 2};
 constexpr bool fused_kernel_exists(BatchKernel k, int n, int number_type, bool hn, bool , int nv) {
@@ -118,6 +128,8 @@
 constexpr int kShBatchWords = 4;
 constexpr double kShareMaxFraction = 0.5;
 void share_plane_records(Plan &plan);
+constexpr bool kPairedAccessDefault = true;
+void pair_plane_records(Plan &plan);
 constexpr int kP2Header = 16, kP2MaxK = 12, kP2SlotBits = 12;
 void share_pass2_records(Plan &plan);
 
diff --git a/dealii-cuda_amd/csrc/mfgpu_kernels.h b/dealii-cuda_amd/csrc/mfgpu_kernels.h
--- a/dealii-cuda_amd/csrc/mfgpu_kernels.h
+++ b/dealii-cuda_amd/csrc/mfgpu_kernels.h
@@ -122,7 +122,8 @@
 
 #define MFGPU_CELL_LOOP_FAMILY(F)                                                                              \
   template <typename T>                                                                                        \
-  hipError_t F##_bind(int dim, int n, bool hn, bool twopass, bool sh, bool mass, uint32_t nb_max, CellKernel<T> *k);
+  hipError_t F##_bind(int dim, int n, bool hn, bool twopass, bool sh, bool mass, bool pa, uint32_t nb_max,             \
+                      CellKernel<T> *k);
 MFGPU_CELL_LOOP_FAMILY(apply)
 MFGPU_CELL_LOOP_FAMILY(x)
 MFGPU_CELL_LOOP_FAMILY(g)
diff --git a/dealii-cuda_amd/csrc/mfgpu_kernels.hip b/dealii-cuda_amd/csrc/mfgpu_kernels.hip
--- a/dealii-cuda_amd/csrc/mfgpu_kernels.hip
+++ b/dealii-cuda_amd/csrc/mfgpu_kernels.hip
@@ -284,7 +284,8 @@
 }
 
 template <typename T>
-hipError_t apply_bind(int dim, int n, bool hn, bool twopass, bool sh, bool mass, uint32_t nb_max, CellKernel<T> *k) {
+hipError_t apply_bind(int dim, int n, bool hn, bool twopass, bool sh, bool mass, bool pa, uint32_t nb_max, CellKernel<T> *k) {
+  if (pa) return hipErrorInvalidValue;
   if (dim != 2 && dim != 3) return hipErrorInvalidValue;
   return dispatch_instantiation(n, [&](auto N, auto D3, auto HN, auto TP, auto SH, auto MASS) {
     constexpr int n_ = N, dim_ = D3 ? 3 : 2;
@@ -397,7 +398,7 @@
 }
 
 #define INST(T)                                                                                         \
-  template hipError_t apply_bind<T>(int, int, bool, bool, bool, bool, uint32_t, CellKernel<T> *);      \
+  template hipError_t apply_bind<T>(int, int, bool, bool, bool, bool, bool, uint32_t, CellKernel<T> *);      \
   template hipError_t orphan_launch<T>(T *, const T *, const uint32_t *, uint32_t, int, hipStream_t);   \
   template hipError_t coefficient_launch<T>(T *, const T *, size_t, int, hipStream_t);                  \
   template hipError_t fold_launch<T>(T *, const T *, const T *, const T *, const uint32_t *, uint32_t,  \
diff --git a/dealii-cuda_amd/csrc/mfgpu_kernels_g.hip b/dealii-cuda_amd/csrc/mfgpu_kernels_g.hip
--- a/dealii-cuda_amd/csrc/mfgpu_kernels_g.hip
+++ b/dealii-cuda_amd/csrc/mfgpu_kernels_g.hip
@@ -447,7 +447,8 @@
 }
 
 template <typename T>
-hipError_t g_bind(int, int n, bool hn, bool, bool sh, bool mass, uint32_t nb_max, CellKernel<T> *k) {
+hipError_t g_bind(int, int n, bool hn, bool, bool sh, bool mass, bool pa, uint32_t nb_max, CellKernel<T> *k) {
+  if (pa) return hipErrorInvalidValue;
   return g_bind_width(n, hn, sh, mass, 1, nb_max, k);
 }
 
@@ -461,7 +462,7 @@
 }
 
 #define INST(T)                                                                                                  \
-  template hipError_t g_bind<T>(int, int, bool, bool, bool, bool, uint32_t, CellKernel<T> *);                    \
+  template hipError_t g_bind<T>(int, int, bool, bool, bool, bool, bool, uint32_t, CellKernel<T> *);                    \
   template hipError_t g_bind_width<T>(int, bool, bool, bool, int, uint32_t, MultiKernel<T> *);                   \
   template hipError_t fold_general_launch<T>(T *, const T *, const T *, const T *, const uint32_t *, uint32_t, \
                                              uint32_t, hipStream_t);
diff --git a/dealii-cuda_amd/csrc/mfgpu_kernels_g2.hip b/dealii-cuda_amd/csrc/mfgpu_kernels_g2.hip
--- a/dealii-cuda_amd/csrc/mfgpu_kernels_g2.hip
+++ b/dealii-cuda_amd/csrc/mfgpu_kernels_g2.hip
@@ -173,7 +173,8 @@
 }
 
 template <typename T>
-hipError_t g2_bind(int, int n, bool hn, bool, bool sh, bool mass, uint32_t nb_max, CellKernel<T> *k) {
+hipError_t g2_bind(int, int n, bool hn, bool, bool sh, bool mass, bool pa, uint32_t nb_max, CellKernel<T> *k) {
+  if (pa) return hipErrorInvalidValue;
   return dispatch_instantiation(n, [&](auto N, auto HN, auto SH, auto MASS) {
     constexpr int n_ = N;
     if constexpr (kernel_exists(BatchKernel::g2, n_, number_type_of<T>, HN, SH, MASS)) {
@@ -183,8 +184,8 @@
       return hipErrorInvalidValue;
   }, hn, sh, mass);
 }
-template hipError_t g2_bind<double>(int, int, bool, bool, bool, bool, uint32_t, CellKernel<double> *);
-template hipError_t g2_bind<float>(int, int, bool, bool, bool, bool, uint32_t, CellKernel<float> *);
+template hipError_t g2_bind<double>(int, int, bool, bool, bool, bool, bool, uint32_t, CellKernel<double> *);
+template hipError_t g2_bind<float>(int, int, bool, bool, bool, bool, bool, uint32_t, CellKernel<float> *);
 
 template <typename T>
 hipError_t fold_general2_launch(T *M, const T *coef, const T *jxw, const T *jinv, const uint32_t *order,
diff --git a/dealii-cuda_amd/csrc/mfgpu_kernels_p.hip b/dealii-cuda_amd/csrc/mfgpu_kernels_p.hip
--- a/dealii-cuda_amd/csrc/mfgpu_kernels_p.hip
+++ b/dealii-cuda_amd/csrc/mfgpu_kernels_p.hip
@@ -8,7 +8,16 @@
 
 #define MFGPU_PIN_VMEM() __builtin_amdgcn_sched_barrier(0x380)
 
-template <int n, typename T, bool ADD, bool HN, bool SH = false, bool MASS = false>
+template <typename T>
+struct Pair {
+  T a, b;
+};
+template <typename T>
+struct alignas(2 * sizeof(T)) APair {
+  T a, b;
+};
+
+template <int n, typename T, bool ADD, bool HN, bool SH = false, bool MASS = false, bool PA = false>
 __global__ void __launch_bounds__(64) __attribute__((amdgpu_waves_per_eu(1, 1)))
 apply_planes3(const ApplyArgs<T> A, const TablesEO<T, n> tab) {
   constexpr int n2 = n * n;
@@ -17,6 +26,7 @@
   constexpr int KGU = p_kgu(n);
   constexpr int JI = p_ji(n);
   constexpr int HS = KGU - JI;
+  constexpr int GR = p_pa_gr(n), SR = p_pa_sr(n), GQ = p_pa_gq(n), HP = HS / 2, HT = HS & 1, NS = SR + HP + HT;
   constexpr int SA = p_cell_stride(n);
   constexpr int NIW = (n2 + 1) / 2;
   extern __shared__ __attribute__((aligned(16))) unsigned char smem_raw[];
@@ -58,7 +68,7 @@
     return l < bend ? (l >= hole0 ? l + hole_len : l) : x;
   };
   if (b >= hole0) b += hole_len;
-  static_assert(kernel_exists(PlaneKernel::planes3, n, number_type_of<T>, HN, SH, MASS), "no such instantiation");
+  static_assert(kernel_exists(PlaneKernel::planes3, n, number_type_of<T>, HN, SH, MASS, PA), "no such instantiation");
   struct Meta {
     uint32_t base, drec, irec;
   };
@@ -111,8 +121,59 @@
     }
   };
 
+  auto load_words = [&](uint32_t rec, int q0, auto &w) {
+    constexpr int NW = (int)(sizeof(w) / sizeof(w[0]));
+    const uint4 *p = reinterpret_cast<const uint4 *>(A.bdofsp) + ((size_t)rec * p_pa_quads(n) + q0) * 64 + lane;
+#pragma unroll
+    for (int q = 0; q < (NW + 3) / 4; ++q) {
+      const uint4 v = p[q * 64];
+      w[4 * q] = v.x;
+      if (4 * q + 1 < NW) w[4 * q + 1] = v.y;
+      if (4 * q + 2 < NW) w[4 * q + 2] = v.z;
+      if (4 * q + 3 < NW) w[4 * q + 3] = v.w;
+    }
+  };
+  auto src_pair = [&](uint32_t base, uint32_t g) -> const Pair<T> * {
+    return reinterpret_cast<const Pair<T> *>(reinterpret_cast<const char *>(A.src + base) +
+                                             (uint32_t)(g * (uint32_t)sizeof(T)));
+  };
+  auto dst_pair = [&](uint32_t base, uint32_t g) -> Pair<T> * {
+    return reinterpret_cast<Pair<T> *>(reinterpret_cast<char *>(A.dst + base) + (uint32_t)(g * (uint32_t)sizeof(T)));
+  };
+  auto ua_at = [&](uint32_t byte_off) -> double * {
+    return reinterpret_cast<double *>(reinterpret_cast<char *>(ua) + byte_off);
+  };
+  auto stage_src_pa = [&](const uint32_t (&ga)[PA ? GR : 1], const uint32_t (&gp)[PA ? GR : 1],
+                          const Pair<T> (&sv)[PA ? GR : 1]) {
+#pragma unroll
+    for (int j = 0; j < GR; ++j) {
+      const unsigned long long keep0 = (unsigned long long)(long long)~((int)(ga[j] << 1) >> 31);
+      const unsigned long long keep1 = (unsigned long long)(long long)~((int)ga[j] >> 31);
+      const double v0 = (double)sv[j].a, v1 = (double)sv[j].b;
+      *ua_at(gp[j] & 0xffffu) = __longlong_as_double((long long)((unsigned long long)__double_as_longlong(v0) & keep0));
+      *ua_at(gp[j] >> 16) = __longlong_as_double((long long)((unsigned long long)__double_as_longlong(v1) & keep1));
+    }
+    ua[KGU * 64 - 1] = 0.0;
+  };
+  auto scatter_pa = [&](int j, uint32_t bb, uint32_t base, const uint32_t (&sa)[PA ? SR : 1],
+                        const Pair<T> (&rs)[PA ? SR : 1], const Pair<T> (&od)[PA ? SR : 1],
+                        const APair<T> (&rh)[PA && HP ? HP : 1], T rt) {
+    T *const hp = A.halo + (size_t)bb * (HS * 64);
+    if (j < SR) {
+      *dst_pair(base, sa[j]) = ADD ? Pair<T>{od[j].a + rs[j].a, od[j].b + rs[j].b} : rs[j];
+    } else if (j < SR + HP) {
+      reinterpret_cast<APair<T> *>(hp + 128 * (j - SR))[lane] = rh[j - SR];
+    } else {
+      hp[128 * HP + lane] = rt;
+    }
+  };
+
   uint32_t b1 = next_of(b), b2 = next_of(b1);
   uint32_t Gp[KGU], Gc[KGU], Gn[KGU], Gnn[KGU];
+  uint32_t GAn[PA ? GR : 1], GAnn[PA ? GR : 1], GPn[PA ? GR : 1], SWc[PA ? 2 * SR : 1], SAp[PA ? SR : 1];
+  Pair<T> SV2[PA ? GR : 1], R2[PA ? SR : 1], old2[PA ? SR : 1];
+  APair<T> RH[PA && HP ? HP : 1];
+  T RT = T(0);
   uint32_t IXc[NIW], IXn[NIW];
   constexpr int CR = PRIV / 64, HROWS = HN ? p_hn_rows(n) : 1;
   uint32_t Hc[HROWS], Hn[HROWS];
@@ -138,8 +199,15 @@
     M2 = meta_of(meta_request(b2));
     Mp = Mc;
   }
-  load_dofs(SH ? Mc.drec : b, Gc);
-  load_dofs(SH ? M1.drec : b1, Gn);
+  if constexpr (PA) {
+    load_words(Mc.drec, 0, GAnn);
+    load_words(Mc.drec, GQ, GPn);
+    load_words(M1.drec, 0, GAn);
+    load_words(Mc.drec, 2 * GQ, SWc);
+  } else {
+    load_dofs(SH ? Mc.drec : b, Gc);
+    load_dofs(SH ? M1.drec : b1, Gn);
+  }
   load_ix(SH ? Mc.irec : b, IXc);
   if (HN) load_hn(b, Hc);
   constexpr uint32_t kDummyIx = 8u * (uint32_t)(KGU * 64 - 1) * 0x10001u;
@@ -155,14 +223,27 @@
 #pragma unroll
     for (int r = 0; r < n2; ++r) Mm[r] = nt_load(p + r * NT);
   }
-#pragma unroll
-  for (int j = 0; j < KGU; ++j) {
-    SVn[j] = src_at(Mc.base, Gc[j]);
-    Gp[j] = Gc[j];
-    R[j] = T(0);
-    old[j] = T(0);
-  }
-  stage_src(Gc, SVn);
+  if constexpr (PA) {
+#pragma unroll
+    for (int j = 0; j < GR; ++j) SV2[j] = *src_pair(Mc.base, GAnn[j]);
+#pragma unroll
+    for (int j = 0; j < SR; ++j) {
+      SAp[j] = SWc[j];
+      R2[j] = old2[j] = Pair<T>{T(0), T(0)};
+    }
+#pragma unroll
+    for (int j = 0; j < HP; ++j) RH[j] = APair<T>{T(0), T(0)};
+    stage_src_pa(GAnn, GPn, SV2);
+  } else {
+#pragma unroll
+    for (int j = 0; j < KGU; ++j) {
+      SVn[j] = src_at(Mc.base, Gc[j]);
+      Gp[j] = Gc[j];
+      R[j] = T(0);
+      old[j] = T(0);
+    }
+    stage_src(Gc, SVn);
+  }
   WaveSync::sync();
 
   const int pxy = lc * SA + n2 * k;
@@ -225,24 +306,44 @@
     STAMP(0);
     RSTAMP(8);
     WGSTAMP(10);
-    load_dofs(SH ? M2.drec : b2, Gnn);
+    if constexpr (PA) {
+      load_words(M2.drec, 0, GAnn);
+      load_words(M1.drec, GQ, GPn);
+      load_words(Mc.drec, 2 * GQ, SWc);
+    } else {
+      load_dofs(SH ? M2.drec : b2, Gnn);
+    }
     load_ix(SH ? M1.irec : b1, IXn);
     if (SH) Mv = meta_request(next_of(b2));
     if (HN) load_hn(b1, Hn);
     if (ADD) {
-#pragma unroll
-      for (int j = 0; j < JI; ++j) old[j] = *dst_at(Mp.base, Gp[j]);
+      if constexpr (PA) {
+#pragma unroll
+        for (int j = 0; j < SR; ++j) old2[j] = *dst_pair(Mp.base, SAp[j]);
+      } else {
+#pragma unroll
+        for (int j = 0; j < JI; ++j) old[j] = *dst_at(Mp.base, Gp[j]);
+      }
     }
     STAMP(1);
     auto hookA = [&](int) {};
     auto hookB = [&](int s) {
       MFGPU_PIN_VMEM();
-#pragma unroll
-      for (int j = (KGU * s) / (5 * n); j < (KGU * (s + 1)) / (5 * n); ++j)
-        scatter_slot(j, bp, Mp.base, Gp[j], R[j], old[j]);
-#pragma unroll
-      for (int j = (KGU * s) / (5 * n); j < (KGU * (s + 1)) / (5 * n); ++j)
-        SVn[j] = src_at(M1.base, Gn[j]);
+      if constexpr (PA) {
+#pragma unroll
+        for (int j = (NS * s) / (5 * n); j < (NS * (s + 1)) / (5 * n); ++j)
+          scatter_pa(j, bp, Mp.base, SAp, R2, old2, RH, RT);
+#pragma unroll
+        for (int j = (GR * s) / (5 * n); j < (GR * (s + 1)) / (5 * n); ++j)
+          SV2[j] = *src_pair(M1.base, GAn[j]);
+      } else {
+#pragma unroll
+        for (int j = (KGU * s) / (5 * n); j < (KGU * (s + 1)) / (5 * n); ++j)
+          scatter_slot(j, bp, Mp.base, Gp[j], R[j], old[j]);
+#pragma unroll
+        for (int j = (KGU * s) / (5 * n); j < (KGU * (s + 1)) / (5 * n); ++j)
+          SVn[j] = src_at(M1.base, Gn[j]);
+      }
       MFGPU_PIN_VMEM();
     };
     const T *const cnext = A.coefp + (size_t)b1 * (n2 * NT) + tk;
@@ -425,16 +526,33 @@
         if ((uint32_t)(r * 64 + lane) < hn_ncopy) lds_add(ua + (Hc[r] & 0xffffu), cv[r]);
       WaveSync::sync();
     }
-#pragma unroll
-    for (int j = 0; j < KGU; ++j) R[j] = (T)ua[lane + j * 64];
+    if constexpr (PA) {
+#pragma unroll
+      for (int j = 0; j < SR; ++j) R2[j] = Pair<T>{(T)ua_at(SWc[SR + j])[0], (T)ua_at(SWc[SR + j])[1]};
+#pragma unroll
+      for (int j = 0; j < HP; ++j) {
+        const APair<double> v = reinterpret_cast<const APair<double> *>(ua + JI * 64 + 128 * j)[lane];
+        RH[j] = APair<T>{(T)v.a, (T)v.b};
+      }
+      if (HT) RT = (T)ua[JI * 64 + 128 * HP + lane];
+    } else {
+#pragma unroll
+      for (int j = 0; j < KGU; ++j) R[j] = (T)ua[lane + j * 64];
+    }
     WaveSync::sync();
     STAMP(5);
-    stage_src(Gn, SVn);
+    if constexpr (PA) stage_src_pa(GAn, GPn, SV2);
+    else stage_src(Gn, SVn);
     STAMP(6);
     bp = b;
     if (SH) Mp = Mc;
-#pragma unroll
-    for (int j = 0; j < KGU; ++j) Gp[j] = Gc[j];
+    if constexpr (PA) {
+#pragma unroll
+      for (int j = 0; j < SR; ++j) SAp[j] = SWc[j];
+    } else {
+#pragma unroll
+      for (int j = 0; j < KGU; ++j) Gp[j] = Gc[j];
+    }
     STAMP(7);
     RSTAMP(9);
     if (!has_next) break;
@@ -447,10 +565,15 @@
       M1 = M2;
       M2 = meta_of(Mv);
     }
-#pragma unroll
-    for (int j = 0; j < KGU; ++j) {
-      Gc[j] = Gn[j];
-      Gn[j] = Gnn[j];
+    if constexpr (PA) {
+#pragma unroll
+      for (int j = 0; j < GR; ++j) GAn[j] = GAnn[j];
+    } else {
+#pragma unroll
+      for (int j = 0; j < KGU; ++j) {
+        Gc[j] = Gn[j];
+        Gn[j] = Gnn[j];
+      }
     }
 #pragma unroll
     for (int w = 0; w < NIW; ++w) IXc[w] = lane_on ? IXn[w] : kDummyIx;
@@ -459,12 +582,21 @@
       for (int w = 0; w < HROWS; ++w) Hc[w] = Hn[w];
     }
   }
-  if (ADD) {
-#pragma unroll
-    for (int j = 0; j < JI; ++j) old[j] = *dst_at(Mp.base, Gp[j]);
-  }
-#pragma unroll
-  for (int j = 0; j < KGU; ++j) scatter_slot(j, bp, Mp.base, Gp[j], R[j], old[j]);
+  if constexpr (PA) {
+    if (ADD) {
+#pragma unroll
+      for (int j = 0; j < SR; ++j) old2[j] = *dst_pair(Mp.base, SAp[j]);
+    }
+#pragma unroll
+    for (int j = 0; j < NS; ++j) scatter_pa(j, bp, Mp.base, SAp, R2, old2, RH, RT);
+  } else {
+    if (ADD) {
+#pragma unroll
+      for (int j = 0; j < JI; ++j) old[j] = *dst_at(Mp.base, Gp[j]);
+    }
+#pragma unroll
+    for (int j = 0; j < KGU; ++j) scatter_slot(j, bp, Mp.base, Gp[j], R[j], old[j]);
+  }
 }
 
 template <int n, typename T>
@@ -474,18 +606,19 @@
 }
 
 template <typename T>
-hipError_t p_bind(int, int n, bool hn, bool, bool sh, bool mass, uint32_t, CellKernel<T> *k) {
-  return dispatch_instantiation(n, [&](auto N, auto HN, auto SH, auto MASS) {
+hipError_t p_bind(int, int n, bool hn, bool, bool sh, bool mass, bool pa, uint32_t, CellKernel<T> *k) {
+  return dispatch_instantiation(n, [&](auto N, auto HN, auto SH, auto MASS, auto PA) {
     constexpr int n_ = N;
-    if constexpr (kernel_exists(PlaneKernel::planes3, n_, number_type_of<T>, HN, SH, MASS))
-      return bind_cell_kernel<T, 64, apply_planes3<n_, T, false, HN, SH, MASS>, apply_planes3<n_, T, true, HN, SH, MASS>,
-                              make_tables_eo<T, n_>>(p_lds_bytes<n_, T>(HN), k);
+    if constexpr (kernel_exists(PlaneKernel::planes3, n_, number_type_of<T>, HN, SH, MASS, PA))
+      return bind_cell_kernel<T, 64, apply_planes3<n_, T, false, HN, SH, MASS, PA>,
+                              apply_planes3<n_, T, true, HN, SH, MASS, PA>, make_tables_eo<T, n_>>(
+          p_lds_bytes<n_, T>(HN), k);
     else
       return hipErrorInvalidValue;
-  }, hn, sh, mass);
+  }, hn, sh, mass, pa);
 }
-template hipError_t p_bind<double>(int, int, bool, bool, bool, bool, uint32_t, CellKernel<double> *);
-template hipError_t p_bind<float>(int, int, bool, bool, bool, bool, uint32_t, CellKernel<float> *);
+template hipError_t p_bind<double>(int, int, bool, bool, bool, bool, bool, uint32_t, CellKernel<double> *);
+template hipError_t p_bind<float>(int, int, bool, bool, bool, bool, bool, uint32_t, CellKernel<float> *);
 
 template <typename T>
 __global__ void relayout_coef_kernel(T *out, const T *in, const uint32_t *cell_batch, const uint32_t *cell_pos,
diff --git a/dealii-cuda_amd/csrc/mfgpu_kernels_q.hip b/dealii-cuda_amd/csrc/mfgpu_kernels_q.hip
--- a/dealii-cuda_amd/csrc/mfgpu_kernels_q.hip
+++ b/dealii-cuda_amd/csrc/mfgpu_kernels_q.hip
@@ -412,7 +412,8 @@
 }
 
 template <typename T>
-hipError_t q_bind(int, int n, bool hn, bool, bool sh, bool mass, uint32_t, CellKernel<T> *k) {
+hipError_t q_bind(int, int n, bool hn, bool, bool sh, bool mass, bool pa, uint32_t, CellKernel<T> *k) {
+  if (pa) return hipErrorInvalidValue;
   return dispatch_instantiation(n, [&](auto N, auto HN, auto SH, auto MASS) {
     constexpr int n_ = N;
     if constexpr (!kernel_exists(PlaneKernel::planes4, n_, number_type_of<T>, HN, SH, MASS))
@@ -425,7 +426,7 @@
                               make_tables_eo<T, n_>>(q_lds_bytes<T>(n_, HN), k);
   }, hn, sh, mass);
 }
-template hipError_t q_bind<double>(int, int, bool, bool, bool, bool, uint32_t, CellKernel<double> *);
-template hipError_t q_bind<float>(int, int, bool, bool, bool, bool, uint32_t, CellKernel<float> *);
+template hipError_t q_bind<double>(int, int, bool, bool, bool, bool, bool, uint32_t, CellKernel<double> *);
+template hipError_t q_bind<float>(int, int, bool, bool, bool, bool, bool, uint32_t, CellKernel<float> *);
 
 }
diff --git a/dealii-cuda_amd/csrc/mfgpu_kernels_x.hip b/dealii-cuda_amd/csrc/mfgpu_kernels_x.hip
--- a/dealii-cuda_amd/csrc/mfgpu_kernels_x.hip
+++ b/dealii-cuda_amd/csrc/mfgpu_kernels_x.hip
@@ -394,7 +394,8 @@
 }
 
 template <typename T>
-hipError_t x_bind(int, int n, bool hn, bool, bool sh, bool mass, uint32_t nb_max, CellKernel<T> *k) {
+hipError_t x_bind(int, int n, bool hn, bool, bool sh, bool mass, bool pa, uint32_t nb_max, CellKernel<T> *k) {
+  if (pa) return hipErrorInvalidValue;
   return dispatch_instantiation(n, [&](auto N, auto HN, auto SH, auto MASS) {
     constexpr int n_ = N;
     if constexpr (kernel_exists(BatchKernel::x, n_, number_type_of<T>, HN, SH, MASS)) {
@@ -405,7 +406,7 @@
   }, hn, sh, mass);
 }
 
-#define INST(T) template hipError_t x_bind<T>(int, int, bool, bool, bool, bool, uint32_t, CellKernel<T> *);
+#define INST(T) template hipError_t x_bind<T>(int, int, bool, bool, bool, bool, bool, uint32_t, CellKernel<T> *);
 INST(double)
 INST(float)
 
diff --git a/dealii-cuda_amd/csrc/mfgpu_plan.cpp b/dealii-cuda_amd/csrc/mfgpu_plan.cpp
--- a/dealii-cuda_amd/csrc/mfgpu_plan.cpp
+++ b/dealii-cuda_amd/csrc/mfgpu_plan.cpp
@@ -836,6 +836,7 @@
     }
   }
   share_plane_records(P);
+  pair_plane_records(P);
   share_pass2_records(P);
   return 0;
 }
@@ -882,6 +883,75 @@
   const size_t shared = P.sh_dofs.size() + P.sh_idx.size() + P.sh_batch.size();
   const size_t expanded = P.pr_dofs.size() + P.pr_idx.size();
   P.sh_use = nbat > 0 && P.pr_hn.empty() && (double)shared <= kShareMaxFraction * (double)expanded;
+}
+
+namespace {
+struct Entry {
+  uint32_t dof, pos, flag;
+};
+
+bool pair_items(const std::vector<Entry> &e, std::vector<std::pair<Entry, Entry>> &items) {
+  items.clear();
+  for (size_t i = 0; i < e.size();) {
+    size_t j = i + 1;
+    while (j < e.size() && e[j].dof == e[j - 1].dof + 1) ++j;
+    const size_t len = j - i;
+    if (len < 2) return false;
+    for (size_t t = 0; t + 1 < len; t += 2) items.emplace_back(e[i + t], e[i + t + 1]);
+    if (len & 1) items.emplace_back(e[j - 2], e[j - 1]);
+    i = j;
+  }
+  return true;
+}
+}
+
+void pair_plane_records(Plan &P) {
+  P.pa_rec.clear();
+  P.pa_use = false;
+  const int n = P.n;
+  if (P.n_plane_batches == 0 || n < 3 || n > 5) return;
+  const size_t NB = (size_t)p_kgu(n) * 64, JI = (size_t)p_ji(n) * 64, nrec = P.sh_dofs.size() / NB;
+  const size_t GR = p_pa_gr(n), SR = p_pa_sr(n), WORDS = (size_t)p_pa_quads(n) * 256;
+  const int GQ = p_pa_gq(n);
+  if (!P.sh_use || nrec == 0) return;
+  std::vector<uint32_t> out(nrec * WORDS, 0u);
+  std::vector<Entry> all, interior;
+  std::vector<std::pair<Entry, Entry>> items;
+  for (size_t r = 0; r < nrec; ++r) {
+    const uint32_t *g = P.sh_dofs.data() + r * NB;
+    all.clear();
+    interior.clear();
+    for (size_t t = 0; t < JI && g[t] != g[JI]; ++t) interior.push_back(Entry{g[t] & 0x7fffffffu, (uint32_t)t, g[t] >> 31});
+    size_t last = JI;
+    while (g[last] != g[NB - 1]) ++last;
+    for (const Entry &e : interior) {
+      if (e.flag) return;
+      all.push_back(e);
+    }
+    for (size_t t = JI; t <= last; ++t) all.push_back(Entry{g[t] & 0x7fffffffu, (uint32_t)t, g[t] >> 31});
+    const auto by_dof = [](const Entry &a, const Entry &b) { return a.dof < b.dof; };
+    std::sort(all.begin(), all.end(), by_dof);
+    std::sort(interior.begin(), interior.end(), by_dof);
+    for (size_t i = 1; i < all.size(); ++i)
+      if (all[i].dof == all[i - 1].dof) return;
+    uint32_t *rec = out.data() + r * WORDS;
+    if (!pair_items(all, items) || items.empty() || items.size() > GR * 64) return;
+    for (size_t i = 0; i < GR * 64; ++i) {
+      const auto &it = items[i < items.size() ? i : 0];
+      rec[p_pa_word(0, (int)(i / 64), (int)(i % 64))] = it.first.dof | (it.first.flag << 30) | (it.second.flag << 31);
+      rec[p_pa_word(GQ, (int)(i / 64), (int)(i % 64))] = (it.first.pos * 8u) | ((it.second.pos * 8u) << 16);
+    }
+    if (!pair_items(interior, items) || items.empty() || items.size() > SR * 64) return;
+    for (const auto &it : items)
+      if (it.second.pos != it.first.pos + 1) return;
+    for (size_t i = 0; i < SR * 64; ++i) {
+      const auto &it = items[i < items.size() ? i : 0];
+      rec[p_pa_word(2 * GQ, (int)(i / 64), (int)(i % 64))] = it.first.dof;
+      rec[p_pa_word(2 * GQ, (int)(SR + i / 64), (int)(i % 64))] = it.first.pos * 8u;
+    }
+  }
+  P.pa_rec.swap(out);
+  P.pa_use = true;
 }
 
 void share_pass2_records(Plan &P) {
@@ -1188,6 +1258,20 @@
   return p ? (p->plan.sh_use ? 1 : 0) | (p->plan.sh_p2_use ? 2 : 0) : 0;
 }
 
+int64_t mfgpu_plan_pair_records(const mfgpu_plan *p, const uint32_t **ptr, uint32_t info[4]) {
+  if (!p || !ptr || !info) return MFGPU_EINVAL;
+  const mfgpu::Plan &P = p->plan;
+  const bool planes3 = P.n >= 3 && P.n <= 5;
+  info[0] = P.pa_use ? 1u : 0u;
+  info[1] = planes3 ? (uint32_t)mfgpu::p_pa_gr(P.n) : 0u;
+  info[2] = planes3 ? (uint32_t)mfgpu::p_pa_sr(P.n) : 0u;
+  info[3] = planes3 ? (uint32_t)(P.pa_rec.size() / ((size_t)mfgpu::p_pa_quads(P.n) * 256)) : 0u;
+  *ptr = P.pa_rec.data();
+  return (int64_t)P.pa_rec.size();
+}
+
+int mfgpu_paired_access_default(void) { return mfgpu::kPairedAccessDefault ? 1 : 0; }
+
 int64_t mfgpu_plan_lmap(const mfgpu_plan *p, const uint16_t **ptr) {
   if (!p || !ptr) return MFGPU_EINVAL;
   *ptr = p->plan.lmap.data();
diff --git a/dealii-cuda_amd/pymfgpu/__init__.py b/dealii-cuda_amd/pymfgpu/__init__.py
--- a/dealii-cuda_amd/pymfgpu/__init__.py
+++ b/dealii-cuda_amd/pymfgpu/__init__.py
@@ -13,6 +13,7 @@
 EUNSUPPORTED = -4
 MULTI_ADD, MULTI_LOOP, MULTI_FUSED = 1, 2, 4
 UNIFORM_J0, HANGING_NODES, COLORED_SCATTER, NO_SHARED_RECORDS = 1, 2, 1 << 8, 1 << 9
+NO_PAIRED_ACCESS = 1 << 11
 UPDATABLE_COEFFICIENTS = 1 << 10
 KERNEL_AUTO, KERNEL_PENCILS, KERNEL_PENCILS_X, KERNEL_PLANES, KERNEL_PLANES_2W = 0, 1, 2, 3, 4
 
@@ -84,7 +85,7 @@
     "mfgpu_vec_sadd", "mfgpu_vec_equ", "mfgpu_vec_scale", "mfgpu_vec_divide", "mfgpu_vec_invert", "mfgpu_vec_mul",
     "mfgpu_vec_dot", "mfgpu_vec_l2_norm", "mfgpu_vec_add_and_dot", "mfgpu_vec_all_zero", "mfgpu_profile_enable", "mfgpu_profile_read", "mfgpu_profile_read_pass2",
     "mfgpu_plan_create", "mfgpu_plan_destroy", "mfgpu_plan_array_u32", "mfgpu_plan_lmap", "mfgpu_plan_bflags",
-    "mfgpu_plan_shares_records", "mfgpu_record_stats",
+    "mfgpu_plan_shares_records", "mfgpu_plan_pair_records", "mfgpu_paired_access_default", "mfgpu_record_stats",
     "mfgpu_vec_alloc", "mfgpu_vec_free", "mfgpu_vec_fill", "mfgpu_vec_from_host", "mfgpu_vec_to_host",
     "mfgpu_device_synchronize", "mfgpu_device_memory_info", "mfgpu_mesh_create_uniform", "mfgpu_mesh_create_adaptive", "mfgpu_mesh_create_ball", "mfgpu_mesh_create_from_leaves",
     "mfgpu_mesh_cell_levels", "mfgpu_mesh_destroy",
@@ -178,6 +179,8 @@
         L.mfgpu_plan_bflags.argtypes = [C.c_void_p, C.POINTER(C.c_void_p)]
         L.mfgpu_plan_bflags.restype = C.c_int64
         L.mfgpu_plan_shares_records.argtypes = [C.c_void_p]
+        L.mfgpu_plan_pair_records.argtypes = [C.c_void_p, C.POINTER(C.c_void_p), C.POINTER(C.c_uint32)]
+        L.mfgpu_plan_pair_records.restype = C.c_int64
         L.mfgpu_record_stats.argtypes = [C.c_void_p, C.POINTER(C.c_uint64)]
         L.mfgpu_vec_alloc.argtypes = [C.POINTER(C.c_void_p), C.c_size_t, C.c_int]
         L.mfgpu_vec_free.argtypes = [C.c_void_p]
@@ -343,6 +346,10 @@
         raise err
 
 
+def paired_access_default():
+    return bool(lib().mfgpu_paired_access_default())
+
+
 def np_dtype(number_type):
     return np.float64 if number_type == F64 else np.float32
 
@@ -644,6 +651,24 @@
     shares_pass2_records = property(lambda s: bool(lib().mfgpu_plan_shares_records(s._h) & 2))
 
     @property
+    def pair_records(self):
+        p, info = C.c_void_p(), (C.c_uint32 * 4)()
+        cnt = lib().mfgpu_plan_pair_records(self._h, C.byref(p), info)
+        if cnt < 0:
+            _check(int(cnt))
+        use, gr, sr, nrec = (int(v) for v in info)
+        gq, sq = (gr + 3) // 4, (2 * sr + 3) // 4
+        raw = _view(p.value, cnt, np.uint32).copy().reshape(nrec, 2 * gq + sq, 64, 4)
+
+        def section(q0, nq, w0, nw):
+            sec = raw[:, q0:q0 + nq].transpose(0, 1, 3, 2).reshape(nrec, nq * 4, 64)
+            return sec[:, w0:w0 + nw].reshape(nrec, nw * 64)
+
+        return dict(paired_access=bool(use), gather_rounds=gr, store_rounds=sr, gather=section(0, gq, 0, gr),
+                    gather_pos=section(gq, gq, 0, gr), store=section(2 * gq, sq, 0, sr),
+                    store_pos=section(2 * gq, sq, sr, sr))
+
+    @property
     def lmap(self):
         p = C.c_void_p()
         cnt = lib().mfgpu_plan_lmap(self._h, C.byref(p))
@@ -789,7 +814,7 @@
         _check(lib().mfgpu_record_stats(self._h, r))
         out.update(index_records="shared" if r[0] & 1 else "expanded",
                    pass2_records="shared" if r[0] & 2 else "expanded", distinct_dof_records=int(r[1]),
-                   distinct_index_records=int(r[2]), index_record_bytes=int(r[3]))
+                   distinct_index_records=int(r[2]), index_record_bytes=int(r[3]), paired_access=bool(r[0] & 4))
         return out
 
     def kernel_name(self):
diff --git a/include/mfgpu.h b/include/mfgpu.h
--- a/include/mfgpu.h
+++ b/include/mfgpu.h
@@ -23,6 +23,8 @@
 #define MFGPU_COLORED_SCATTER (1u << 8)
 
 #define MFGPU_NO_SHARED_RECORDS (1u << 9)
+
+#define MFGPU_NO_PAIRED_ACCESS (1u << 11)
 
 #define MFGPU_UPDATABLE_COEFFICIENTS (1u << 10)
 
@@ -103,6 +105,8 @@
 void mfgpu_plan_destroy(mfgpu_plan *p);
 int64_t mfgpu_plan_array_u32(const mfgpu_plan *p, int what, const uint32_t **ptr);
 int mfgpu_plan_shares_records(const mfgpu_plan *p);
+int64_t mfgpu_plan_pair_records(const mfgpu_plan *p, const uint32_t **ptr, uint32_t info[4]);
+int mfgpu_paired_access_default(void);
 int mfgpu_plan_multi_groups(uint32_t n_vectors, const uint32_t *widths, uint32_t n_widths, uint32_t *groups,
                             uint32_t capacity);
 int64_t mfgpu_plan_lmap(const mfgpu_plan *p, const uint16_t **ptr);
```

Result: faster. 83.32 billion DoFs/s, median of 6 (+1.7%).
